# KrishnaswamyLab/MELD

Hardware: AMD Instinct MI355X
Metric: cells/sec through MELD.fit_transform (kNN+Chebyshev) (higher is better)
Workload: dtype f64

## Files before the change

### include/meld_hip.h

```cpp
#ifndef MELD_HIP_H
#define MELD_HIP_H

#include <stddef.h>
#include <stdint.h>

#ifdef __cplusplus
extern "C" {
#endif

#define MELD_OK 0
#define MELD_ERR_INVALID (-1)
#define MELD_ERR_UNSUPPORTED (-2)
#define MELD_ERR_HIP (-3)

typedef void* meld_stream_t;

int meld_abi_version(void);
const char* meld_last_error(void);
int meld_device_count(void);


int meld_knn_padded_dim(int d);
int meld_knn_tile_refs(void);
int meld_knn_block_queries(void);
// ... 45 lines not shown
                            int64_t tile_begin, int64_t tile_count, meld_stream_t stream);
int meld_knn16_sphere_layout(int64_t n_ref, int d, int64_t* rows, int64_t* row_bytes);
int meld_knn16_bounds_from_spheres(const double* X, int64_t N, int d, const double* mean, const float* scale_info,
                      const float* norm2_max, const void* Rt16, int64_t q_begin, int64_t q_count,
                      const float* thr_seed, const float* q_norm2 ,
                      int nprod, void* temp, void* lb2, meld_stream_t stream);
int meld_knn16_prepare_cross(const double* X, int64_t n_refs, int64_t n_total, int d, const double* mean, int64_t q_begin,
                             int64_t q_count, void* Rt16, void* Q16, float* Qn, float* norm2, float* norm2_max,
                             float* scale_info, meld_stream_t stream);
int meld_knn16_prepare_rows(const double* X, int64_t N, int d, const double* mean, const float* scale_info,
                            int64_t q_begin, const int32_t* rows, int64_t n_rows, void* Q16, float* Qn,
                            meld_stream_t stream);
int meld_knn16_research_thresholds(const int32_t* rows, int64_t n_rows, int64_t q_begin, const int32_t* cand_cnt,
                                   const float* cand_d2, int cap, int ksel, const float* norm2, const float* norm2_max,
                                   double err_coef, double err_lin, double err3, const float* scale_info, float* thr,
                                   meld_stream_t stream);
int meld_knn16_seed_thresholds_mfma(const void* Q16, const float* Qn, const void* Rt16, const float* scale_info,
                                    const float* norm2_max, int64_t n_ref, int d, int64_t q_begin, int64_t q_count,
                                    int knn, double radius_factor, int nprod, int side_tiles, float* thr_init,
                                    meld_stream_t stream);
int meld_knn16_topk(const void* Q16, const float* Qn, const void* Rt16, const float* scale_info,
                    int64_t n_ref, int d, int64_t q_count, int ksel, int nprod, int n_slices, const void* lb2,
                    const float* norm2_max, int64_t q_begin, const float* thr_init, int knn, double radius_factor,
                    int32_t* cand_idx, float* cand_d2, int32_t* cand_cnt, float* cand_thr,
                    uint64_t* tiles_done ,
                    const int32_t* block_order ,
                    meld_stream_t stream);
int meld_knn16_block_work(const void* lb2, const float* thr_seed, int64_t n_ref, int d, int64_t q_count, int nprod,
                          const float* norm2_max, const float* scale_info, int32_t* work, meld_stream_t stream);
int meld_knn16_step_lists(const void* lb2, const float* thr_seed, int64_t n_ref, int d, int64_t q_count, int nprod,
                          const float* norm2_max, const float* scale_info, int64_t q_begin, uint32_t* list,
                          int64_t list_stride, int32_t* cnt, meld_stream_t stream);
size_t meld_knn16_list_scratch_bytes(int64_t n_ref);
int meld_knn16_step_lists_direct(const double* X, int64_t N, int d, const double* mean, const float* scale_info, const float* norm2_max,
                                 const void* Rt16, const float* thr_seed, const float* q_norm2, int nprod, void* temp, void* scratch,
                                 uint32_t* list, int64_t list_stride, int32_t* cnt, meld_stream_t stream);
int meld_knn16_step_lists_direct_lead(const double* X, int64_t N, int d, const double* mean, const float* scale_info, const float* norm2_max,
                                 const void* Rt16, const float* thr_seed, const float* q_norm2, int nprod, void* temp, void* scratch,
                                 uint32_t* list, int64_t list_stride, int32_t* cnt, int lead_only, meld_stream_t stream);
int meld_knn16_step_lists_direct_spheres(const double* X, int64_t N, int d, const double* mean, const float* scale_info, const float* norm2_max,
                                 const void* Rt16, const float* thr_seed, const float* q_norm2, int nprod, void* temp, void* scratch,
                                 uint32_t* list, int64_t list_stride, int32_t* cnt, int lead_only, meld_stream_t stream);
int meld_knn16_topk_listed(const void* Q16, const float* Qn, const void* Rt16, const float* scale_info, int64_t n_ref, int d,
                           int64_t q_count, int ksel, const uint32_t* step_list, const int32_t* step_cnt, int64_t list_stride,
                           const float* norm2_max, int64_t q_begin, const float* thr_init, int knn, double radius_factor,
                           int32_t* cand_idx, float* cand_d2, int32_t* cand_cnt, float* cand_thr, uint64_t* tiles_done,
                           const int32_t* block_order, int n_slices , meld_stream_t stream);
int meld_knn16_topk_listed_partial(const void* Q16, const float* Qn, const void* Rt16, const float* scale_info, int64_t n_ref,
                                   int d, int64_t q_count, int ksel, const uint32_t* step_list, const int32_t* step_cnt,
                                   int64_t list_stride, const float* norm2_max, int64_t q_begin, const float* thr_init, int knn,
                                   double radius_factor, int32_t* cand_idx, float* cand_d2, int32_t* cand_cnt, float* cand_thr,
                                   uint64_t* tiles_done, const int32_t* block_order, int n_slices, int partial_test,
                                   meld_stream_t stream);
int meld_knn16_partial_filter(const void* Q16, const float* Qn, const void* Rt16, const float* scale_info, const float* norm2_max, int d,
                              int64_t q_count, const float* thr_init, uint32_t* step_list, const int32_t* step_cnt, int64_t list_stride,
                              int32_t* cnt_out, uint64_t* tested, const int32_t* block_order , meld_stream_t stream);
int meld_knn16_resident_blocks(int d, int nprod);
int meld_knn16_max_slices(int ksel);
int meld_knn16_merge_slices(const int32_t* s_idx, const float* s_d2, const int32_t* s_cnt, int64_t q_count,
                            int ksel, int n_slices, int32_t* out_idx, float* out_d2, int32_t* out_cnt,
                            meld_stream_t stream);


int meld_knn_refine(const double* X, int64_t N, int d, int64_t q_begin, int64_t q_count,
                    const int32_t* cand_idx, const float* cand_d2, const int32_t* cand_cnt,
                    const float* cand_thr ,
                    int ksel, int cap , int knn, double decay, double thresh,
                    const float* norm2_max, double err_coef,
                    const float* norm2 , double err_coef_lin, double* bw,
                    double* cand_val, int32_t* keep_cnt, int32_t* flag_rows, int32_t* n_flag,
                    const int32_t* rows, int out_cap, int32_t* cand_idx_out,
                    double bw_scale ,
                    const double* bw_fixed ,
                    int max_rank ,
                    meld_stream_t stream);

int meld_knn_radius_exact(const double* X, int64_t N, int d, int64_t q_begin, const int32_t* flag_rows,
                          int32_t n_flag, const double* bw, int knn, double decay, double thresh,
                          int mode, int32_t* fb_cnt, const int64_t* fb_off, int32_t* fb_cursor,
                          int32_t* fb_col, double* fb_val, int32_t* err_flag,
                          double bw_scale ,
                          meld_stream_t stream);
int meld_knn_pair_distances(const double* X, int d, const int64_t* rows, const int64_t* cand, int64_t n, int kk, double* out,
                            meld_stream_t stream);

#define MELD_METRIC_L1 1
#define MELD_METRIC_LINF 2
int meld_metric_tile_rows(void);
int meld_metric_tile_boxes(const double* X, int64_t N, int d, double* box_lo, double* box_hi, meld_stream_t stream);
int meld_metric_topk(const double* X, int64_t N, int d, int metric, int ksel, const double* box_lo, const double* box_hi, int prune,
                     double* heap_d, int32_t* heap_i, int32_t* cand_idx, double* cand_d, int32_t* cand_cnt,
                     unsigned long long* tiles_done, meld_stream_t stream);
int meld_metric_refine(const int32_t* cand_idx, const double* cand_d, const int32_t* cand_cnt, int64_t N, int ksel, int knn,
                       double decay, double thresh, double* bw, double* cand_val, int32_t* keep_cnt, int32_t* flag_rows,
                       int32_t* n_flag, meld_stream_t stream);
int meld_metric_radius(const double* X, int64_t N, int d, int metric, const int32_t* flag_rows, int32_t n_flag, const double* bw,
                       double decay, double thresh, int mode, int32_t* fb_cnt, const int64_t* fb_off, int32_t* fb_cursor,
                       int32_t* fb_col, double* fb_val, meld_stream_t stream);

int meld_metric_cross_slices(int64_t M, int64_t N, int n_slices);
int meld_metric_cross_seed(const double* Qt, int64_t M, const double* box_lo, const double* box_hi, int64_t N, int d, int metric,
                           unsigned long long* seed_key, meld_stream_t stream);
int meld_metric_cross_topk(const double* Qt, int64_t M, const double* X, int64_t N, int d, int metric, int ksel, const double* box_lo,
                           const double* box_hi, const int32_t* seed, int prune, int n_slices, double* heap_d, int32_t* heap_i,
                           int32_t* part_idx, double* part_d, int32_t* part_cnt, int32_t* cand_idx, double* cand_d, int32_t* cand_cnt,
                           unsigned long long* tiles_done, meld_stream_t stream);
int meld_metric_cross_refine(const int32_t* cand_idx, const double* cand_d, const int32_t* cand_cnt, int64_t M, int ksel, int knn,
                             double decay, double thresh, double bw_scale, double* bw, double* cand_val, int32_t* keep_cnt,
                             int32_t* flag_rows, int32_t* n_flag, meld_stream_t stream);
int meld_metric_cross_radius(const double* Q, int64_t M, const double* X, int64_t N, int d, int metric, const int32_t* flag_rows,
                             int32_t n_flag, const double* bw, double decay, double thresh, int mode, int32_t* fb_cnt,
                             const int64_t* fb_off, int32_t* fb_cursor, int32_t* fb_col, double* fb_val, meld_stream_t stream);


size_t meld_scan_temp_bytes(int64_t n);
int meld_exclusive_scan_i32_i64(const int32_t* in, int64_t* out, int64_t n, void* temp, size_t temp_bytes,
                                meld_stream_t stream);

int meld_coo_emit(int64_t q_begin, int64_t q_count, const int32_t* cand_idx, const double* cand_val,
                  const int32_t* cand_cnt, int ksel, int cap, const int64_t* keep_off, const int32_t* flag_rows,
                  int32_t n_flag, const int64_t* fb_off, const int32_t* fb_col, const double* fb_val,
                  int64_t fb_base, int64_t M, uint64_t* keys, double* vals, meld_stream_t stream);

size_t meld_sort_temp_bytes(int64_t n);
int meld_sort_pairs_u64_f64(const uint64_t* keys_in, uint64_t* keys_out, const double* vals_in,
                            double* vals_out, int64_t n, int end_bit, void* temp, size_t temp_bytes,
                            meld_stream_t stream);

size_t meld_merge_temp_bytes(int64_t n);
int meld_coo_merge(const uint64_t* keys_sorted, const double* vals_sorted, int64_t n, uint64_t* ukeys,
                   double* uvals, int64_t* n_unique, void* temp, size_t temp_bytes, meld_stream_t stream);

int meld_csr_from_keys(const uint64_t* ukeys, int64_t nnz, int64_t row_begin, int64_t n_rows,
                       int64_t* rowptr, int32_t* col, meld_stream_t stream);

int meld_coo_partition_remote(const uint64_t* keys, const double* vals, int64_t n, int64_t rows_per_rank, int world,
                              int self_rank, int64_t cap, int32_t* counts, int64_t* send, meld_stream_t stream);
int meld_coo_emit_scatter(int64_t q_count, const int32_t* cand_idx, const double* cand_val, int ksel, int cap,
                          const int32_t* keep_cnt, const int32_t* flag_rows, int32_t n_flag, const int64_t* fb_off,
                          const int32_t* fb_col, const double* fb_val, int64_t fb_total, int32_t* cursor, int32_t* tcol,
                          double* tval, meld_stream_t stream);
int meld_csr_bucket_slots(void);
int meld_coo_scatter_rows(const uint64_t* keys, const double* vals, int64_t n, int64_t row_begin, int64_t n_rows,
                          int32_t* cursor, int32_t* tcol, double* tval, meld_stream_t stream);
int meld_csr_rows_sort_merge(const int32_t* cursor, int64_t n_rows, int32_t* tcol, double* tval, int32_t* ucnt,
                             int32_t* flags,
                             int symm ,
                             double theta , meld_stream_t stream);
int meld_csr_rows_sort_merge_sums(const int32_t* cursor, int64_t n_rows, int32_t* tcol, double* tval, int32_t* ucnt, int32_t* flags,
                                  int symm, double theta, double diag, double* sums, meld_stream_t stream);
int meld_csr_compact_rows_anisotropy(const int64_t* rowptr, int64_t n_rows, const int32_t* tcol, const double* tval, int32_t* col,
                                     double* val, const double* ksum, double anisotropy, double* dw, meld_stream_t stream);
int meld_csr_compact_rows(const int64_t* rowptr, int64_t n_rows, const int32_t* tcol, const double* tval,
                          int32_t* col, double* val, meld_stream_t stream);
int meld_csr_compact_rows_sums(const int64_t* rowptr, int64_t n_rows, const int32_t* tcol, const double* tval, int32_t* col,
                               double* val, double diag, double* sums, meld_stream_t stream);

int meld_csr_row_sums(const int64_t* rowptr, const double* val, int64_t n_rows, double diag,
                      double* out, meld_stream_t stream);
int meld_csr_anisotropy(const int64_t* rowptr, const int32_t* col, double* val, int64_t n_rows,
                        const double* ksum_all, int64_t ksum_row_offset, double anisotropy,
                        meld_stream_t stream);
int meld_csr_anisotropy_degrees(const int64_t* rowptr, const int32_t* col, double* val, int64_t n_rows,
                                const double* ksum_all, int64_t ksum_row_offset, double anisotropy, double* dw,
                                meld_stream_t stream);


size_t meld_extend_rows_temp_bytes(int64_t n, int64_t n_rows);
int meld_extend_rows(const uint64_t* keys, const double* half_vals, int64_t n, int64_t row_begin, int64_t n_rows, int64_t n_cols,
                     int64_t* rowptr, int32_t* col, double* val, double* rowsum, void* temp, size_t temp_bytes,
                     meld_stream_t stream);
int meld_extend_apply(const int64_t* rowptr, const int32_t* col, const double* val, const double* rowsum, int64_t n_rows,
                      const double* F, int64_t n_f_rows, int p, const int64_t* colmap, double* out, meld_stream_t stream);


struct meld_pt_layout;
typedef struct meld_laplacian {
  const int64_t* rowptr; const int32_t* col; const double* val; const double* dw;
  int64_t n_rows, nnz;
  const struct meld_pt_layout* layout;
} meld_laplacian_t;

int meld_spmm_dot_slots(void);
int meld_cheby_step(const meld_laplacian_t* L, int p, const double* x_full, int64_t x_row_offset, const double* z, double* y,
                    double* r, double alpha, double beta, double gamma, double coef, double* dots, meld_stream_t stream);

int meld_cheby_step_wide(const meld_laplacian_t* L, int p, const double* x_full, int64_t x_row_offset, const double* z, double* y,
                         double alpha, double beta, double gamma, meld_stream_t stream);

int meld_block_max_blocks(void);
int meld_block_gram_f64(const double* A, int64_t lda, const double* B, int64_t ldb, int64_t n_rows, int m, double* part, int n_blocks,
                        double* C, meld_stream_t stream);
int meld_block_rotate_f64(const double* A, int64_t lda, const double* S, int64_t n_rows, int m, double* out, int64_t ldo,
                          meld_stream_t stream);
// ... 97 lines not shown
```

### meld_amd/_lib.py

```python
from __future__ import annotations

from ._options import is_set, opt

import ctypes as C
import os

_HERE = os.path.dirname(os.path.abspath(__file__))
LIB_NAME = "libmeld_hip.so"
LIB_PATH = os.path.join(_HERE, LIB_NAME)

_i32, _i64, _f64, _sz, _ptr = C.c_int, C.c_int64, C.c_double, C.c_size_t, C.c_void_p

SIGNATURES = {
    "meld_abi_version": (_i32, []),
    "meld_last_error": (C.c_char_p, []),
    "meld_device_count": (_i32, []),
    "meld_knn_padded_dim": (_i32, [_i32]),
    "meld_knn_tile_refs": (_i32, []),
    "meld_knn_block_queries": (_i32, []),
    "meld_knn_row_capacity": (_i32, [_i32]),
    "meld_col_sums_f64": (_i32, [_ptr, _i64, _i32, _ptr, _ptr]),
    "meld_col_stats_temp_bytes": (_sz, [_i32]),
    "meld_col_stats_f64": (_i32, [_ptr, _i64, _i32, _ptr, _ptr, _ptr, _ptr, _sz, _ptr]),
    "meld_knn_prepare_refs": (_i32, [_ptr, _i64, _i32, _ptr, _i32, _ptr, _ptr, _ptr, _ptr]),
    "meld_knn_prepare_queries": (_i32, [_ptr, _i64, _i32, _ptr, _i32, _i64, _i64, _ptr, _ptr]),
    "meld_knn_topk": (_i32, [_ptr, _ptr, _i64, _i32, _i64, _i32, _ptr, _ptr, _ptr, _ptr]),
    "meld_knn_refine": (
        _i32,
        [_ptr, _i64, _i32, _i64, _i64, _ptr, _ptr, _ptr, _ptr, _i32, _i32, _i32, _f64, _f64, _ptr, _f64, _ptr, _f64, _ptr, _ptr, _ptr,
         _ptr, _ptr, _ptr, _i32, _ptr, _f64, _ptr, _i32, _ptr],
    ),
    "meld_knn_error_coef": (_f64, [_i32]),
    "meld_knn16_kblocks": (_i32, [_i32]),
    "meld_knn16_tile_refs": (_i32, []),
    "meld_knn16_split_dims": (_i32, [_i32]),
    "meld_knn16_block_queries": (_i32, []),
    "meld_knn16_row_capacity": (_i32, [_i32]),
    "meld_knn16_error_coef": (_f64, [_i32, _i32]),
    "meld_knn16_error_coef_const": (_f64, [_i32, _i32]),
    "meld_knn16_error_coef_lin": (_f64, [_i32]),
    "meld_knn16_resident_blocks": (_i32, [_i32, _i32]),
    "meld_knn16_tile_bytes": (_sz, [_i32]),
    "meld_knn16_query_bytes": (_sz, [_i32]),
    "meld_knn16_prepare": (_i32, [_ptr, _i64, _i32, _ptr, _i64, _i64, _ptr, _ptr, _ptr, _ptr, _ptr, _ptr, _ptr]),
    "meld_knn16_prepare_scaled": (_i32, [_ptr, _i64, _i32, _ptr, _ptr, _ptr, _i64, _i64, _ptr, _ptr, _ptr, _ptr, _ptr, _ptr, _ptr]),
    "meld_knn16_prepare_cross": (_i32, [_ptr, _i64, _i64, _i32, _ptr, _i64, _i64, _ptr, _ptr, _ptr, _ptr, _ptr, _ptr, _ptr]),
    "meld_knn16_prepare_rows": (_i32, [_ptr, _i64, _i32, _ptr, _ptr, _i64, _ptr, _i64, _ptr, _ptr, _ptr]),
    "meld_knn16_research_thresholds": (_i32, [_ptr, _i64, _i64, _ptr, _ptr, _i32, _i32, _ptr, _ptr, _f64, _f64, _f64, _ptr, _ptr, _ptr]),
    "meld_knn16_bounds_bytes": (_sz, [_i64, _i64]),
    "meld_knn16_bounds_temp_bytes": (_sz, [_i64, _i32, _i64]),
    "meld_knn16_bounds": (_i32, [_ptr, _i64, _i32, _ptr, _ptr, _ptr, _ptr, _i64, _i64, _ptr, _ptr, _i32, _ptr, _ptr, _ptr]),
    "meld_knn16_bounds_from_spheres": (_i32, [_ptr, _i64, _i32, _ptr, _ptr, _ptr, _ptr, _i64, _i64, _ptr, _ptr, _i32, _ptr, _ptr, _ptr]),
    "meld_knn16_tile_spheres": (_i32, [_ptr, _i64, _i32, _ptr, _ptr, _ptr, _i64, _i64, _ptr]),
    "meld_knn16_sphere_layout": (_i32, [_i64, _i32, _ptr, _ptr]),
    "meld_knn16_topk": (_i32, [_ptr, _ptr, _ptr, _ptr, _i64, _i32, _i64, _i32, _i32, _i32, _ptr, _ptr, _i64, _ptr, _i32, _f64, _ptr, _ptr, _ptr, _ptr, _ptr, _ptr, _ptr]),
    "meld_knn16_block_work": (_i32, [_ptr, _ptr, _i64, _i32, _i64, _i32, _ptr, _ptr, _ptr, _ptr]),
    "meld_knn16_step_lists": (_i32, [_ptr, _ptr, _i64, _i32, _i64, _i32, _ptr, _ptr, _i64, _ptr, _i64, _ptr, _ptr]),
    "meld_knn16_list_scratch_bytes": (_sz, [_i64]),
    "meld_knn16_step_lists_direct": (_i32, [_ptr, _i64, _i32, _ptr, _ptr, _ptr, _ptr, _ptr, _ptr, _i32, _ptr, _ptr, _ptr, _i64, _ptr, _ptr]),
    "meld_knn16_prepare_fused": (_i32, [_ptr, _i64, _i32, _ptr, _ptr, _ptr, _ptr, _ptr, _ptr, _ptr, _ptr, _ptr, _ptr, _ptr]),
    "meld_knn16_step_lists_direct_spheres": (_i32, [_ptr, _i64, _i32, _ptr, _ptr, _ptr, _ptr, _ptr, _ptr, _i32, _ptr, _ptr, _ptr, _i64, _ptr, _i32, _ptr]),
    "meld_knn16_step_lists_direct_lead": (_i32, [_ptr, _i64, _i32, _ptr, _ptr, _ptr, _ptr, _ptr, _ptr, _i32, _ptr, _ptr, _ptr, _i64, _ptr, _i32, _ptr]),
    "meld_knn16_topk_listed": (_i32, [_ptr, _ptr, _ptr, _ptr, _i64, _i32, _i64, _i32, _ptr, _ptr, _i64, _ptr, _i64, _ptr, _i32, _f64, _ptr, _ptr, _ptr, _ptr, _ptr, _ptr, _i32, _ptr]),
    "meld_knn16_topk_listed_partial": (_i32, [_ptr, _ptr, _ptr, _ptr, _i64, _i32, _i64, _i32, _ptr, _ptr, _i64, _ptr, _i64, _ptr, _i32, _f64, _ptr, _ptr, _ptr, _ptr, _ptr, _ptr, _i32, _i32, _ptr]),
    "meld_knn16_partial_filter": (_i32, [_ptr, _ptr, _ptr, _ptr, _ptr, _i32, _i64, _ptr, _ptr, _ptr, _i64, _ptr, _ptr, _ptr, _ptr]),
    "meld_knn16_seed_thresholds_mfma": (_i32, [_ptr, _ptr, _ptr, _ptr, _ptr, _i64, _i32, _i64, _i64, _i32, _f64, _i32, _i32, _ptr, _ptr]),
    "meld_knn16_max_slices": (_i32, [_i32]),
    "meld_knn16_merge_slices": (_i32, [_ptr, _ptr, _ptr, _i64, _i32, _i32, _ptr, _ptr, _ptr, _ptr]),
    "meld_knn_radius_exact": (
        _i32,
        [_ptr, _i64, _i32, _i64, _ptr, _i32, _ptr, _i32, _f64, _f64, _i32, _ptr, _ptr, _ptr, _ptr, _ptr, _ptr, _f64, _ptr],
    ),
    "meld_knn_pair_distances": (_i32, [_ptr, _i32, _ptr, _ptr, _i64, _i32, _ptr, _ptr]),
    "meld_metric_tile_rows": (_i32, []),
    "meld_metric_tile_boxes": (_i32, [_ptr, _i64, _i32, _ptr, _ptr, _ptr]),
    "meld_metric_topk": (_i32, [_ptr, _i64, _i32, _i32, _i32, _ptr, _ptr, _i32, _ptr, _ptr, _ptr, _ptr, _ptr, _ptr, _ptr]),
    "meld_metric_refine": (_i32, [_ptr, _ptr, _ptr, _i64, _i32, _i32, _f64, _f64, _ptr, _ptr, _ptr, _ptr, _ptr, _ptr]),
    "meld_metric_radius": (_i32, [_ptr, _i64, _i32, _i32, _ptr, _i32, _ptr, _f64, _f64, _i32, _ptr, _ptr, _ptr, _ptr, _ptr, _ptr]),
    "meld_metric_cross_slices": (_i32, [_i64, _i64, _i32]),
    "meld_metric_cross_seed": (_i32, [_ptr, _i64, _ptr, _ptr, _i64, _i32, _i32, _ptr, _ptr]),
    "meld_metric_cross_topk": (_i32, [_ptr, _i64, _ptr, _i64, _i32, _i32, _i32, _ptr, _ptr, _ptr, _i32, _i32, _ptr, _ptr, _ptr, _ptr, _ptr, _ptr,
                                      _ptr, _ptr, _ptr, _ptr]),
    "meld_metric_cross_refine": (_i32, [_ptr, _ptr, _ptr, _i64, _i32, _i32, _f64, _f64, _f64, _ptr, _ptr, _ptr, _ptr, _ptr, _ptr]),
    "meld_metric_cross_radius": (_i32, [_ptr, _i64, _ptr, _i64, _i32, _i32, _ptr, _i32, _ptr, _f64, _f64, _i32, _ptr, _ptr, _ptr, _ptr, _ptr, _ptr]),
    "meld_scan_temp_bytes": (_sz, [_i64]),
    "meld_exclusive_scan_i32_i64": (_i32, [_ptr, _ptr, _i64, _ptr, _sz, _ptr]),
    "meld_coo_emit": (
        _i32,
        [_i64, _i64, _ptr, _ptr, _ptr, _i32, _i32, _ptr, _ptr, _i32, _ptr, _ptr, _ptr, _i64, _i64, _ptr, _ptr, _ptr],
    ),
    "meld_sort_temp_bytes": (_sz, [_i64]),
    "meld_sort_pairs_u64_f64": (_i32, [_ptr, _ptr, _ptr, _ptr, _i64, _i32, _ptr, _sz, _ptr]),
    "meld_merge_temp_bytes": (_sz, [_i64]),
    "meld_coo_merge": (_i32, [_ptr, _ptr, _i64, _ptr, _ptr, _ptr, _ptr, _sz, _ptr]),
    "meld_csr_from_keys": (_i32, [_ptr, _i64, _i64, _i64, _ptr, _ptr, _ptr]),
    "meld_csr_seg_length": (_i32, []),
    "meld_csr_spmm_f64": (_i32, [_ptr, _ptr, _ptr, _i32, _i64, _ptr, _ptr, _i64, _ptr, _ptr, _i64, _ptr, _ptr, _i64, _i32, _ptr, _i64, _ptr]),
    "meld_csr_transpose_keys": (_i32, [_ptr, _ptr, _ptr, _i32, _i64, _ptr, _ptr, _ptr]),
    "meld_csr_rows_to_dense_f64": (_i32, [_ptr, _ptr, _ptr, _i32, _i64, _i64, _i64, _ptr, _i64, _ptr]),
    "meld_csr_bucket_slots": (_i32, []),
    "meld_coo_scatter_rows": (_i32, [_ptr, _ptr, _i64, _i64, _i64, _ptr, _ptr, _ptr, _ptr]),
    "meld_coo_emit_scatter": (_i32, [_i64, _ptr, _ptr, _i32, _i32, _ptr, _ptr, _i32, _ptr, _ptr, _ptr, _i64, _ptr, _ptr, _ptr, _ptr]),
    "meld_coo_partition_remote": (_i32, [_ptr, _ptr, _i64, _i64, _i32, _i32, _i64, _ptr, _ptr, _ptr]),
    "meld_csr_rows_sort_merge": (_i32, [_ptr, _i64, _ptr, _ptr, _ptr, _ptr, _i32, _f64, _ptr]),
    "meld_csr_compact_rows": (_i32, [_ptr, _i64, _ptr, _ptr, _ptr, _ptr, _ptr]),
    "meld_csr_rows_sort_merge_sums": (_i32, [_ptr, _i64, _ptr, _ptr, _ptr, _ptr, _i32, _f64, _f64, _ptr, _ptr]),
    "meld_csr_compact_rows_anisotropy": (_i32, [_ptr, _i64, _ptr, _ptr, _ptr, _ptr, _ptr, _f64, _ptr, _ptr]),
    "meld_csr_compact_rows_sums": (_i32, [_ptr, _i64, _ptr, _ptr, _ptr, _ptr, _f64, _ptr, _ptr]),
    "meld_csr_row_sums": (_i32, [_ptr, _ptr, _i64, _f64, _ptr, _ptr]),
    "meld_csr_anisotropy": (_i32, [_ptr, _ptr, _ptr, _i64, _ptr, _i64, _f64, _ptr]),
    "meld_csr_anisotropy_degrees": (_i32, [_ptr, _ptr, _ptr, _i64, _ptr, _i64, _f64, _ptr, _ptr]),
    "meld_extend_rows_temp_bytes": (_sz, [_i64, _i64]),
    "meld_extend_rows": (_i32, [_ptr, _ptr, _i64, _i64, _i64, _i64, _ptr, _ptr, _ptr, _ptr, _ptr, _sz, _ptr]),
    "meld_extend_apply": (_i32, [_ptr, _ptr, _ptr, _ptr, _i64, _ptr, _i64, _i32, _ptr, _ptr, _ptr]),
    "meld_spmm_dot_slots": (_i32, []),
    "meld_cheby_step": (_i32, [_ptr, _i32, _ptr, _i64, _ptr, _ptr, _ptr, _f64, _f64, _f64, _f64, _ptr, _ptr]),
    "meld_lanczos_steps": (_i32, [_ptr, _ptr, _ptr, _ptr, _ptr, _ptr, _ptr, _i32, _i32, _ptr, _ptr, _ptr]),
    "meld_lanczos_spmv": (_i32, [_ptr, _ptr, _i64, _ptr, _ptr, _ptr, _ptr, _ptr]),
    "meld_lanczos_alpha": (_i32, [_ptr, _ptr, _ptr, _ptr, _i32, _ptr]),
    "meld_lanczos_axpy": (_i32, [_ptr, _ptr, _i64, _ptr, _ptr, _ptr]),
    "meld_lanczos_beta": (_i32, [_ptr, _ptr, _ptr, _ptr, _i32, _ptr]),
    "meld_lanczos_fold": (_i32, [_ptr, _ptr, _ptr, _ptr, _i32, _ptr]),
    "meld_lanczos_axpy3": (_i32, [_ptr, _ptr, _ptr, _i64, _ptr, _ptr, _ptr]),
    "meld_pt_geometry": (_i32, [_ptr, _ptr, _ptr, _ptr]),
    "meld_pt_num_blocks": (_i32, [_i64]),
    "meld_pt_seg_len": (_i64, [_i32]),
    "meld_pt_stream_len": (_i64, [_i64, _i32]),
    "meld_pt_desc_len": (_i64, [_i32]),
    "meld_pt_build": (_i32, [_ptr, _ptr, _ptr, _i64, _i64, _i64, _i32, _ptr, _ptr, _ptr, _ptr]),
    "meld_cheby_step_wide": (_i32, [_ptr, _i32, _ptr, _i64, _ptr, _ptr, _f64, _f64, _f64, _ptr]),
    "meld_block_max_blocks": (_i32, []),
    "meld_block_gram_f64": (_i32, [_ptr, _i64, _ptr, _i64, _i64, _i32, _ptr, _i32, _ptr, _ptr]),
    "meld_block_rotate_f64": (_i32, [_ptr, _i64, _ptr, _i64, _i32, _ptr, _i64, _ptr]),
    "meld_block_residuals_f64": (_i32, [_ptr, _ptr, _i64, _ptr, _i64, _i32, _ptr, _i32, _ptr, _ptr]),
    "meld_kmeans_max_blocks": (_i32, []),
    "meld_kmeans_assign": (_i32, [_ptr, _i64, _i32, _ptr, _i32, _ptr, _ptr, _ptr, _ptr, _i32, _ptr]),
    "meld_scale_f64": (_i32, [_ptr, _f64, _ptr, _i64, _ptr]),
    "meld_axpby_f64": (_i32, [_f64, _ptr, _f64, _ptr, _i64, _ptr, _ptr]),
    "meld_normalize_rows_l1": (_i32, [_ptr, _ptr, _i64, _i32, _ptr]),
    "meld_assign_nearest": (_i32, [_ptr, _i64, _i32, _ptr, _i32, _ptr, _ptr, _ptr, _ptr]),
    "meld_chain_order": (_i32, [_ptr, _i64, _i32, _i32, _ptr, _ptr]),
    "meld_gather_rows_f64": (_i32, [_ptr, _ptr, _i64, _i32, _ptr, _ptr]),
    "meld_frame_max_dims": (_i32, []),
    "meld_cov_sample_f64": (_i32, [_ptr, _i64, _i32, _ptr, _i64, _ptr, _ptr]),
    "meld_rotate_rows_f64": (_i32, [_ptr, _i64, _i32, _ptr, _ptr, _ptr, _ptr]),
    "meld_argsort_u32_temp_bytes": (_sz, [_i64]),
    "meld_argsort_u32": (_i32, [_ptr, _i64, _i32, _ptr, _ptr, _ptr, _sz, _ptr]),
    "meld_order_starts": (_i32, [_ptr, _i64, _i32, _ptr, _ptr]),
    "meld_order_pick_centroids": (_i32, [_ptr, _i64, _i32, _ptr, _ptr, _i32, _i32, _ptr, _ptr]),
    "meld_order_update_keys": (_i32, [_ptr, _ptr, _ptr, _i64, _i32, _ptr]),
    "meld_rccl_available": (_i32, []),
    "meld_rccl_unique_id": (_i32, [_ptr]),
    "meld_rccl_comm_create": (_i32, [_ptr, _i32, _i32, _ptr]),
    "meld_rccl_comm_destroy": (_i32, [_ptr]),
    "meld_rccl_all_gather": (_i32, [_ptr, _ptr, _ptr, _sz, _ptr]),
# ... 61 lines not shown
```

### meld_amd/build.py

```python
from __future__ import annotations

from ._options import is_set, opt

import os
import shutil
import subprocess
import sys

_HERE = os.path.dirname(os.path.abspath(__file__))
CSRC = os.path.join(_HERE, "csrc")
SOURCES = ["api.hip", "knn.hip", "knn16.hip", "refine.hip", "assemble.hip", "spmm.hip", "spmm_tiled.hip", "reorder.hip", "kmeans.hip", "labels.hip", "sharded.hip", "frame.hip", "csr_dense.hip", "metric_knn.hip", "extend.hip", "subspace.hip"]
OUT = os.path.join(_HERE, "libmeld_hip.so")
FLAGS = ["--offload-arch=gfx950", "-O3", "-std=c++17", "-fPIC", "-Wno-unused-result"]
FILE_FLAGS = {"knn16.hip": ["-fno-honor-nans"]}


def _hipcc():
    exe = shutil.which("hipcc") or "/opt/rocm/bin/hipcc"
    if not os.path.exists(exe):
        raise RuntimeError("hipcc not found (ROCm toolchain required to build meld_amd)")
    return exe


def _stale(out, deps):
# ... 29 lines not shown
                    label = lines[max(i for i in starts if i <= wi)]
                    m2 = re.search(r"Header=(BB\d+_\d+)", label) or (re.match(r"^\.L(BB\d+_\d+):", label) if "Loop Header" in label else None)
                    if m2:
                        votes[m2.group(1)] = votes.get(m2.group(1), 0) + 1
                header = max(votes, key=votes.get)
                assert votes[header] >= 7, votes
                checked = 0
                for bi, i0 in enumerate(starts):
                    i1 = starts[bi + 1] if bi + 1 < len(starts) else len(lines)
                    label = lines[i0]
                    in_loop = re.search(r"(Header=|Loop |^\.L)" + header + r"\b", label) is not None
                    if not in_loop and not any(i in wait_set for i in range(i0, i1)):
                        continue
                    inside = False
                    for l in lines[i0 + 1 : i1]:
                        if "#ASMSTART" in l:
                            inside = True
                        elif "#ASMEND" in l:
                            inside = False
                        elif not inside and not l.lstrip().startswith(";"):
                            assert not slot.search(l.split(";")[0]), (fn, l)
                            checked += 1
                assert checked > 200, (fn, checked)
                kernels += 1
            fn, lines = (m.group(1) if m else None), []
        elif fn:
            lines.append(line)
    assert kernels == 3, kernels
    return kernels


def gate_stream_slots(hipcc=None, verbose=True):
    hipcc = hipcc or _hipcc()
    src = os.path.join(CSRC, "spmm_tiled.hip")
    cmd = [hipcc] + FLAGS + ["--cuda-device-only", "-S", src, "-o", "-"]
    if verbose:
        print("[meld_amd.build] gate:", " ".join(cmd), flush=True)
    run = subprocess.run(cmd, stdout=subprocess.PIPE, stderr=subprocess.PIPE, text=True)
    if run.returncode != 0 or not run.stdout:
        raise RuntimeError("meld_amd.build: `hipcc -S` of spmm_tiled.hip failed (status {}), the register-slot guard of pt_step_kernel "
                           "could not run -- not linking:\n{}".format(run.returncode, run.stderr[-2000:]))
    asm = run.stdout
    try:
        return check_stream_slots(asm)
    except (AssertionError, ValueError, StopIteration) as e:
        raise RuntimeError("meld_amd.build: the register-slot guard of pt_step_kernel failed ({}); the tiled recurrence kernel "
                           "cannot be trusted with this toolchain -- not linking".format(e))


def build(force=False, verbose=True):
    hipcc = _hipcc()
    objdir = os.path.join(_HERE, "build")
    os.makedirs(objdir, exist_ok=True)
    headers = [os.path.join(CSRC, "common.hpp"), os.path.join(_HERE, "..", "include", "meld_hip.h")]
    procs = []
    objs = []
    for src in SOURCES:
        s = os.path.join(CSRC, src)
        o = os.path.join(objdir, src.replace(".hip", ".o"))
        objs.append(o)
        if force or _stale(o, [s] + headers):
            cmd = [hipcc] + FLAGS + FILE_FLAGS.get(src, []) + ["-c", s, "-o", o]
            if verbose:
                print("[meld_amd.build]", " ".join(cmd), flush=True)
            procs.append((src, subprocess.Popen(cmd, stdout=subprocess.PIPE, stderr=subprocess.STDOUT)))
    rebuilt = [src for src, _ in procs]
    for src, p in procs:
        out, _ = p.communicate()
        if p.returncode != 0:
            sys.stderr.write(out.decode(errors="replace"))
            raise RuntimeError("hipcc failed on {}".format(src))
    if "spmm_tiled.hip" in rebuilt or (force and opt("MELD_BUILD_SKIP_GATE") != "1"):
        if opt("MELD_BUILD_SKIP_GATE") != "1":
            gate_stream_slots(hipcc, verbose)
    if force or procs or _stale(OUT, objs):
        cmd = [hipcc, "--offload-arch=gfx950", "-shared", "-fPIC"] + objs + ["-ldl", "-o", OUT]
        if verbose:
            print("[meld_amd.build]", " ".join(cmd), flush=True)
        subprocess.check_call(cmd)
    return OUT


if __name__ == "__main__":
    build(force="--force" in sys.argv)
    print(OUT)
```

### meld_amd/csrc/assemble.hip

```cpp
#include "common.hpp"

#include <rocprim/rocprim.hpp>

namespace meld {

__global__ __launch_bounds__(256) void coo_emit_rows_kernel(int64_t q_begin, int64_t q_count,
                                                            const int* __restrict__ cand_idx,
                                                            const double* __restrict__ cand_val, int ksel, int cap,
                                                            const int64_t* __restrict__ keep_off, int64_t M,
                                                            unsigned long long* __restrict__ keys,
                                                            double* __restrict__ vals) {
  const int lane = threadIdx.x & 63;
  const int64_t q = (int64_t)blockIdx.x * 4 + (threadIdx.x >> 6);
  if (q >= q_count) return;
  const int64_t base = keep_off[q];
  if (keep_off[q + 1] == base) return;
  const unsigned long long gi = (unsigned long long)(q_begin + q);
  int written = 0;
  for (int c0 = 0; c0 < ksel; c0 += 64) {
    const int c = c0 + lane;
    double v = 0.0;
    int j = 0;
    if (c < ksel) {
      v = cand_val[(size_t)q * ksel + c];
// ... 196 lines not shown

extern "C" size_t meld_merge_temp_bytes(int64_t n) {
  size_t bytes = 0;
  uint64_t* k = nullptr;
  double* v = nullptr;
  int64_t* c = nullptr;
  (void)rocprim::reduce_by_key(nullptr, bytes, k, v, (size_t)n, k, v, c, rocprim::plus<double>(),
                               rocprim::equal_to<uint64_t>());
  return bytes + 256;
}

extern "C" int meld_coo_merge(const uint64_t* keys_sorted, const double* vals_sorted, int64_t n, uint64_t* ukeys,
                              double* uvals, int64_t* n_unique, void* temp, size_t temp_bytes,
                              meld_stream_t stream) {
  MELD_CHECK_ARG(keys_sorted && vals_sorted && ukeys && uvals && n_unique && temp && n >= 0,
                 "meld_coo_merge: bad arguments");
  if (n == 0) {
    MELD_HIP_CALL(hipMemsetAsync(n_unique, 0, sizeof(int64_t), S(stream)));
    return MELD_OK;
  }
  size_t bytes = temp_bytes;
  MELD_HIP_CALL(rocprim::reduce_by_key(temp, bytes, keys_sorted, vals_sorted, (size_t)n, ukeys, uvals, n_unique,
                                       rocprim::plus<double>(), rocprim::equal_to<uint64_t>(), S(stream)));
  return MELD_OK;
}

extern "C" int meld_csr_from_keys(const uint64_t* ukeys, int64_t nnz, int64_t row_begin, int64_t n_rows,
                                  int64_t* rowptr, int32_t* col, meld_stream_t stream) {
  MELD_CHECK_ARG(rowptr && n_rows > 0 && nnz >= 0 && (nnz == 0 || (ukeys && col)), "meld_csr_from_keys: bad arguments");
  hipLaunchKernelGGL(csr_rowptr_kernel, dim3((unsigned)ceil_div(n_rows + 1, 256)), dim3(256), 0, S(stream),
                     reinterpret_cast<const unsigned long long*>(ukeys), nnz, row_begin, n_rows, rowptr);
  MELD_LAUNCH_CHECK("csr_rowptr_kernel");
  if (nnz > 0) {
    hipLaunchKernelGGL(csr_cols_kernel, dim3((unsigned)ceil_div(nnz, 256)), dim3(256), 0, S(stream),
                       reinterpret_cast<const unsigned long long*>(ukeys), nnz, col);
    MELD_LAUNCH_CHECK("csr_cols_kernel");
  }
  return MELD_OK;
}

__device__ __forceinline__ void coo_row_run(int64_t r, int lane, bool* leader, int* rank, int* run_len) {
  const int64_t prev = __shfl_up(r, 1, 64);
  const bool head = lane == 0 || prev != r;
  const unsigned long long hb = __ballot(head);
  const unsigned long long below = hb & ((2ull << lane) - 1ull);
  const int lead = 63 - __clzll((long long)below);
  const unsigned long long above = lane == 63 ? 0ull : (hb >> (lane + 1));
  const int next = above ? lane + 1 + (__ffsll((long long)above) - 1) : 64;
  *leader = head;
  *rank = lane - lead;
  *run_len = next - lane;
}

constexpr int CSR_BUCKET = 256;

__global__ __launch_bounds__(256) void coo_scatter_rows_kernel(const unsigned long long* __restrict__ keys,
                                                               const double* __restrict__ vals, int64_t n, int64_t row_begin,
                                                               int64_t n_rows, int* __restrict__ cursor, int* __restrict__ tcol,
                                                               double* __restrict__ tval) {
  const int64_t e = (int64_t)blockIdx.x * blockDim.x + threadIdx.x;
  const int lane = threadIdx.x & 63;
  int64_t r = -1 - lane;
  unsigned long long k = 0;
  if (e < n) {
    k = keys[e];
    const int64_t rr = (int64_t)(k >> 32) - row_begin;
    if (rr >= 0 && rr < n_rows) r = rr;
  }
  bool leader;
  int rank, run_len;
  coo_row_run(r, lane, &leader, &rank, &run_len);
  int first = 0;
  if (leader && r >= 0) first = atomicAdd(cursor + r, run_len);
  const int slot = __shfl(first, lane - rank, 64) + rank;
  if (r >= 0 && slot < CSR_BUCKET) {
    tcol[r * CSR_BUCKET + slot] = (int)(unsigned)k;
    tval[r * CSR_BUCKET + slot] = vals[e];
  }
}

constexpr int PR_PER = 16;
constexpr int PR_WORLD_MAX = 64;
__global__ __launch_bounds__(256) void coo_partition_remote_kernel(const unsigned long long* __restrict__ keys,
                                                                   const double* __restrict__ vals, int64_t n,
                                                                   int64_t rows_per_rank, int world, int self_rank, int64_t cap,
                                                                   int* __restrict__ counts, long long* __restrict__ send) {
  __shared__ int s_cnt[PR_WORLD_MAX];
  __shared__ int s_base[PR_WORLD_MAX];
  if (threadIdx.x < PR_WORLD_MAX) s_cnt[threadIdx.x] = 0;
  __syncthreads();
  const int64_t e0 = (int64_t)blockIdx.x * (256 * PR_PER) + threadIdx.x;
  unsigned long long k[PR_PER];
  int pos[PR_PER];
#pragma unroll
  for (int u = 0; u < PR_PER; ++u) {
    const int64_t e = e0 + (int64_t)u * 256;
    pos[u] = -1;
    k[u] = 0;
    if (e < n) {
      k[u] = keys[e];
      const int o = (int)min((int64_t)(k[u] >> 32) / rows_per_rank, (int64_t)world - 1);
      if (o != self_rank) pos[u] = (o << 24) | atomicAdd(&s_cnt[o], 1);
    }
  }
  __syncthreads();
  if (threadIdx.x < world && s_cnt[threadIdx.x] > 0) s_base[threadIdx.x] = atomicAdd(counts + threadIdx.x, s_cnt[threadIdx.x]);
  __syncthreads();
#pragma unroll
  for (int u = 0; u < PR_PER; ++u) {
    if (pos[u] >= 0) {
      const int o = pos[u] >> 24;
      const int64_t slot = (int64_t)s_base[o] + (pos[u] & 0xFFFFFF);
      if (slot < cap) {
        send[((int64_t)o * 2 + 0) * cap + slot] = (long long)k[u];
        send[((int64_t)o * 2 + 1) * cap + slot] = __double_as_longlong(vals[e0 + (int64_t)u * 256]);
      }
    }
  }
}

__global__ __launch_bounds__(256) void coo_emit_scatter_rows_kernel(int64_t q_count, const int* __restrict__ cand_idx,
                                                                    const double* __restrict__ cand_val, int ksel, int cap,
                                                                    const int* __restrict__ keep_cnt, int* __restrict__ cursor,
                                                                    int* __restrict__ tcol, double* __restrict__ tval) {
  const int lane = threadIdx.x & 63;
  const int64_t q = (int64_t)blockIdx.x * 4 + (threadIdx.x >> 6);
  if (q >= q_count) return;
  if (keep_cnt[q] == 0) return;
  int written = 0;
  for (int c0 = 0; c0 < ksel; c0 += 64) {
    const int c = c0 + lane;
    double v = 0.0;
    int j = 0;
    if (c < ksel) {
      v = cand_val[(size_t)q * ksel + c];
      j = cand_idx[(size_t)q * cap + c];
    }
    const bool keep = v > 0.0;
    const unsigned long long b = __ballot(keep);
    if (keep) {
      const int pos = written + __popcll(b & ((1ull << lane) - 1ull));
      const double hv = 0.5 * v;
      tcol[q * CSR_BUCKET + pos] = j;
      tval[q * CSR_BUCKET + pos] = hv;
      const int slot = atomicAdd(cursor + j, 1);
      if (slot < CSR_BUCKET) {
        tcol[(int64_t)j * CSR_BUCKET + slot] = (int)q;
        tval[(int64_t)j * CSR_BUCKET + slot] = hv;
      }
    }
    written += __popcll(b);
  }
}
__global__ __launch_bounds__(256) void coo_emit_scatter_fallback_kernel(const int* __restrict__ flag_rows, int n_flag,
                                                                        const int64_t* __restrict__ fb_off,
                                                                        const int* __restrict__ fb_col,
                                                                        const double* __restrict__ fb_val, int64_t fb_total,
                                                                        int* __restrict__ cursor, int* __restrict__ tcol,
                                                                        double* __restrict__ tval) {
  const int64_t e = (int64_t)blockIdx.x * blockDim.x + threadIdx.x;
  if (e >= fb_total) return;
  int lo = 0, hi = n_flag - 1;
  while (lo < hi) {
    const int mid = (lo + hi + 1) >> 1;
    if (fb_off[mid] <= e) lo = mid; else hi = mid - 1;
  }
  const int64_t q = flag_rows[lo];
  const int64_t pos = e - fb_off[lo];
  const int j = fb_col[e];
  const double hv = 0.5 * fb_val[e];
  if (pos < CSR_BUCKET) {
    tcol[q * CSR_BUCKET + pos] = j;
    tval[q * CSR_BUCKET + pos] = hv;
  }
  const int slot = atomicAdd(cursor + j, 1);
  if (slot < CSR_BUCKET) {
    tcol[(int64_t)j * CSR_BUCKET + slot] = (int)q;
    tval[(int64_t)j * CSR_BUCKET + slot] = hv;
  }
}

template <int SL, typename K>
__device__ __forceinline__ void csr_bitonic_sort(K (&key)[SL], int lane) {
  constexpr int NE = 64 * SL;
#pragma unroll
  for (int k = 2; k <= NE; k <<= 1) {
#pragma unroll
    for (int j = k >> 1; j > 0; j >>= 1) {
      if (j >= 64) {
        const int je = j >> 6;
#pragma unroll
        for (int e = 0; e < SL; ++e) {
          if ((e & je) == 0) {
            const bool asc = ((64 * e + lane) & k) == 0;
            const K a = key[e], b = key[e | je];
            const bool sw = asc ? (b < a) : (a < b);
            key[e] = sw ? b : a;
            key[e | je] = sw ? a : b;
          }
        }
      } else {
#pragma unroll
        for (int e = 0; e < SL; ++e) {
          const int i = 64 * e + lane;
          const K o = __shfl_xor(key[e], j, 64);
          const bool keep_min = ((i & j) == 0) == ((i & k) == 0);
          key[e] = keep_min ? (o < key[e] ? o : key[e]) : (o < key[e] ? key[e] : o);
        }
      }
    }
  }
}

template <int SL>
__device__ __forceinline__ int csr_row_merge(int* __restrict__ tcol, double* __restrict__ tval, int64_t base, int n, int lane,
                                             bool* bad, int symm, double theta, double* srow) {
  static_assert(CSR_BUCKET <= 256, "the slot shares a 32-bit key with a 24-bit column");
  unsigned cin[SL];
  bool wide = false;
#pragma unroll
  for (int e = 0; e < SL; ++e) {
// ... 200 lines not shown
        if (k < len) {
          const double dd = di * kj[u];
          const double w = (anisotropy == 0.0) ? v[u] : (anisotropy == 1.0) ? v[u] / dd : v[u] / pow(dd, anisotropy);
          col[dst + k] = c[u];
          val[dst + k] = w;
          s += w;
        }
      }
    }
  }
  s += __shfl_xor(s, 1, 64);
  s += __shfl_xor(s, 2, 64);
  s += __shfl_xor(s, 4, 64);
  if (r < n_rows && g == 0) dw[r] = 0.0 + s;
}

extern "C" int meld_csr_bucket_slots(void) { return CSR_BUCKET; }

extern "C" int meld_coo_scatter_rows(const uint64_t* keys, const double* vals, int64_t n, int64_t row_begin, int64_t n_rows,
                                     int32_t* cursor, int32_t* tcol, double* tval, meld_stream_t stream) {
  MELD_CHECK_ARG(cursor && n_rows > 0 && n >= 0 && (n == 0 || (keys && vals && tcol && tval)),
                 "meld_coo_scatter_rows: bad arguments");
  MELD_HIP_CALL(hipMemsetAsync(cursor, 0, sizeof(int32_t) * (size_t)n_rows, S(stream)));
  if (n == 0) return MELD_OK;
  hipLaunchKernelGGL(coo_scatter_rows_kernel, dim3((unsigned)ceil_div(n, 256)), dim3(256), 0, S(stream),
                     reinterpret_cast<const unsigned long long*>(keys), vals, n, row_begin, n_rows, cursor, tcol, tval);
  MELD_LAUNCH_CHECK("coo_scatter_rows_kernel");
  return MELD_OK;
}

extern "C" int meld_coo_partition_remote(const uint64_t* keys, const double* vals, int64_t n, int64_t rows_per_rank, int world,
                                         int self_rank, int64_t cap, int32_t* counts, int64_t* send, meld_stream_t stream) {
  MELD_CHECK_ARG(counts && send && n >= 0 && (n == 0 || (keys && vals)) && rows_per_rank > 0 && world >= 1 && self_rank >= 0 &&
                     self_rank < world && cap >= 0,
                 "meld_coo_partition_remote: bad arguments");
  MELD_HIP_CALL(hipMemsetAsync(counts, 0, sizeof(int32_t) * (size_t)world, S(stream)));
  if (cap > 0) MELD_HIP_CALL(hipMemsetAsync(send, 0xFF, sizeof(int64_t) * 2 * (size_t)world * (size_t)cap, S(stream)));
  if (n == 0) return MELD_OK;
  MELD_CHECK_ARG(world <= PR_WORLD_MAX, "meld_coo_partition_remote: %d ranks (at most %d)", world, PR_WORLD_MAX);
  hipLaunchKernelGGL(coo_partition_remote_kernel, dim3((unsigned)ceil_div(n, 256 * PR_PER)), dim3(256), 0, S(stream),
                     reinterpret_cast<const unsigned long long*>(keys), vals, n, rows_per_rank, world, self_rank, cap, counts,
                     reinterpret_cast<long long*>(send));
  MELD_LAUNCH_CHECK("coo_partition_remote_kernel");
  return MELD_OK;
}

extern "C" int meld_coo_emit_scatter(int64_t q_count, const int32_t* cand_idx, const double* cand_val, int ksel, int cap,
                                     const int32_t* keep_cnt, const int32_t* flag_rows, int32_t n_flag, const int64_t* fb_off,
                                     const int32_t* fb_col, const double* fb_val, int64_t fb_total, int32_t* cursor, int32_t* tcol,
                                     double* tval, meld_stream_t stream) {
  MELD_CHECK_ARG(cand_idx && cand_val && keep_cnt && cursor && tcol && tval && q_count > 0, "meld_coo_emit_scatter: bad arguments");
  MELD_CHECK_ARG(cap >= ksel && ksel <= CSR_BUCKET, "meld_coo_emit_scatter: ksel=%d must fit a row bucket (%d) and the row stride cap=%d",
                 ksel, CSR_BUCKET, cap);
  hipLaunchKernelGGL(coo_emit_scatter_rows_kernel, dim3((unsigned)ceil_div(q_count, 4)), dim3(256), 0, S(stream), q_count, cand_idx,
                     cand_val, ksel, cap, keep_cnt, cursor, tcol, tval);
  MELD_LAUNCH_CHECK("coo_emit_scatter_rows_kernel");
  if (n_flag > 0 && fb_total > 0) {
    MELD_CHECK_ARG(flag_rows && fb_off && fb_col && fb_val, "meld_coo_emit_scatter: missing fallback arrays");
    hipLaunchKernelGGL(coo_emit_scatter_fallback_kernel, dim3((unsigned)ceil_div(fb_total, 256)), dim3(256), 0, S(stream), flag_rows,
                       n_flag, fb_off, fb_col, fb_val, fb_total, cursor, tcol, tval);
    MELD_LAUNCH_CHECK("coo_emit_scatter_fallback_kernel");
  }
  return MELD_OK;
}

extern "C" int meld_csr_rows_sort_merge(const int32_t* cursor, int64_t n_rows, int32_t* tcol, double* tval, int32_t* ucnt,
                                        int32_t* flags, int symm, double theta, meld_stream_t stream) {
  MELD_CHECK_ARG(cursor && tcol && tval && ucnt && flags && n_rows > 0, "meld_csr_rows_sort_merge: bad arguments");
  MELD_CHECK_ARG(symm >= 0 && symm <= 2 && (symm != 2 || (theta >= 0.0 && theta <= 1.0)),
                 "meld_csr_rows_sort_merge: symm must be 0 (+), 1 (*) or 2 (mnn, theta in [0, 1])");
  MELD_HIP_CALL(hipMemsetAsync(flags, 0, sizeof(int32_t), S(stream)));
  hipLaunchKernelGGL(csr_rows_sort_merge_kernel, dim3((unsigned)ceil_div(n_rows, 4)), dim3(256), 0, S(stream), cursor, n_rows,
                     tcol, tval, ucnt, flags, symm, theta, 0.0, (double*)nullptr);
  MELD_LAUNCH_CHECK("csr_rows_sort_merge_kernel");
  return MELD_OK;
}

extern "C" int meld_csr_rows_sort_merge_sums(const int32_t* cursor, int64_t n_rows, int32_t* tcol, double* tval, int32_t* ucnt,
                                             int32_t* flags, int symm, double theta, double diag, double* sums, meld_stream_t stream) {
  MELD_CHECK_ARG(cursor && tcol && tval && ucnt && flags && sums && n_rows > 0, "meld_csr_rows_sort_merge_sums: bad arguments");
  MELD_CHECK_ARG(symm >= 0 && symm <= 2 && (symm != 2 || (theta >= 0.0 && theta <= 1.0)),
                 "meld_csr_rows_sort_merge_sums: symm must be 0 (+), 1 (*) or 2 (mnn, theta in [0, 1])");
  MELD_HIP_CALL(hipMemsetAsync(flags, 0, sizeof(int32_t), S(stream)));
  hipLaunchKernelGGL(csr_rows_sort_merge_kernel, dim3((unsigned)ceil_div(n_rows, 4)), dim3(256), 0, S(stream), cursor, n_rows,
                     tcol, tval, ucnt, flags, symm, theta, diag, sums);
  MELD_LAUNCH_CHECK("csr_rows_sort_merge_kernel");
  return MELD_OK;
}

extern "C" int meld_csr_compact_rows_anisotropy(const int64_t* rowptr, int64_t n_rows, const int32_t* tcol, const double* tval,
                                                int32_t* col, double* val, const double* ksum, double anisotropy, double* dw,
                                                meld_stream_t stream) {
  MELD_CHECK_ARG(rowptr && n_rows > 0 && tcol && tval && col && val && ksum && dw, "meld_csr_compact_rows_anisotropy: bad arguments");
  hipLaunchKernelGGL(csr_compact_rows_anisotropy_kernel, dim3((unsigned)ceil_div(n_rows * 8, 256)), dim3(256), 0, S(stream), rowptr, n_rows,
                     tcol, tval, col, val, ksum, anisotropy, dw);
  MELD_LAUNCH_CHECK("csr_compact_rows_anisotropy_kernel");
  return MELD_OK;
}

extern "C" int meld_csr_compact_rows(const int64_t* rowptr, int64_t n_rows, const int32_t* tcol, const double* tval,
                                     int32_t* col, double* val, meld_stream_t stream) {
  MELD_CHECK_ARG(rowptr && n_rows > 0 && tcol && tval && col && val, "meld_csr_compact_rows: bad arguments");
  hipLaunchKernelGGL(csr_compact_rows_kernel, dim3((unsigned)ceil_div(n_rows * 16, 256)), dim3(256), 0, S(stream), rowptr,
                     n_rows, tcol, tval, col, val);
  MELD_LAUNCH_CHECK("csr_compact_rows_kernel");
  return MELD_OK;
}

extern "C" int meld_csr_compact_rows_sums(const int64_t* rowptr, int64_t n_rows, const int32_t* tcol, const double* tval, int32_t* col,
                                          double* val, double diag, double* sums, meld_stream_t stream) {
  MELD_CHECK_ARG(rowptr && n_rows > 0 && tcol && tval && col && val && sums, "meld_csr_compact_rows_sums: bad arguments");
  hipLaunchKernelGGL(csr_compact_rows_sums_kernel, dim3((unsigned)ceil_div(n_rows * 8, 256)), dim3(256), 0, S(stream), rowptr, n_rows, tcol,
                     tval, col, val, diag, sums);
  MELD_LAUNCH_CHECK("csr_compact_rows_sums_kernel");
// ... 34 lines not shown
```

### meld_amd/csrc/common.hpp

```cpp
#pragma once
#include <hip/hip_runtime.h>
#include <stdint.h>
#include <stdio.h>
#include <stdlib.h>
#include <string.h>

#include "../../include/meld_hip.h"

namespace meld {

char* err_buf();
void set_err(const char* fmt, ...);

static inline hipStream_t S(meld_stream_t s) { return reinterpret_cast<hipStream_t>(s); }

constexpr int WAVE = 64;

#define MELD_CHECK_ARG(cond, ...)        \
  do {                                   \
    if (!(cond)) {                       \
      meld::set_err(__VA_ARGS__);        \
      return MELD_ERR_INVALID;           \
    }                                    \
  } while (0)

#define MELD_LAUNCH_CHECK(name)                                               \
  do {                                                                        \
    hipError_t e__ = hipGetLastError();                                       \
    if (e__ != hipSuccess) {                                                  \
      meld::set_err("%s: launch failed: %s", name, hipGetErrorString(e__));   \
      return MELD_ERR_HIP;                                                    \
    }                                                                         \
  } while (0)

#define MELD_HIP_CALL(expr)                                                   \
  do {                                                                        \
    hipError_t e__ = (expr);                                                  \
    if (e__ != hipSuccess) {                                                  \
      meld::set_err("%s failed: %s", #expr, hipGetErrorString(e__));          \
      return MELD_ERR_HIP;                                                    \
    }                                                                         \
  } while (0)

__device__ __forceinline__ double wave_sum(double v) {
#pragma unroll
  for (int off = 32; off > 0; off >>= 1) v += __shfl_xor(v, off, 64);
  return v;
}

__device__ __forceinline__ int lane_id() { return threadIdx.x & 63; }

static inline int64_t ceil_div(int64_t a, int64_t b) { return (a + b - 1) / b; }

static inline const char* meld_dev_getenv(const char* name) {
  const char* dev = getenv("MELD_DEV");
  return (dev && dev[0] == '1' && dev[1] == 0) ? getenv(name) : nullptr;
}

struct PtLanczos {
  const double* nrm2_prev;
  double* nrm2_zero;
  const double* state_prev;
  double* state_cur;
  double* betas;
  int it;
  const int* stop;
};

static inline bool laplacian_ok(const meld_laplacian_t* L) {
  if (!L || !L->rowptr || !L->dw) return false;
  if (const meld_pt_layout_t* t = L->layout)
    return t->blk_row && t->blk_ntile && t->blk_ndist && t->seg && t->list_cols && t->pval && t->pidx;
  return L->nnz == 0 || (L->col && L->val);
}

int pt_step(const meld_pt_layout_t* L, const int64_t* rowptr, const double* dw, int p, const double* x_full,
            int64_t x_row_offset, const double* z, double* y, double* r, double alpha, double beta, double gamma,
            double coef, double* dots, const double* coef_dev, hipStream_t st, double coef_x = 0.0, const PtLanczos* lz = nullptr);

}
```

### meld_amd/csrc/knn16.hip

```cpp
#include "common.hpp"

#include <hip/hip_fp16.h>

#include <algorithm>

namespace meld {

constexpr int K16_TS = 64;
constexpr int K16_BQ = 256;
constexpr int K16_THREADS = 256;
constexpr int K16_NWAVE = K16_THREADS / 64;
constexpr int K16_SLACK = 128;
constexpr int K16_CAPMAX = 256;
constexpr int K16_BOUNDS_THREADS = 1024;
constexpr int K16_SLOTS = K16_CAPMAX / 64;
constexpr int K16_DMAX = 16 * 9 - 3;

constexpr int K16_SPLIT_DA = 13;
__host__ __device__ inline void k16_slot(int c, int d, int dA, int* coord, int* piece) {
  *coord = -1;
  *piece = -1;
  if (dA == 0) {
    if (c < d) *coord = c;
    else if (c < d + 3) *piece = 3 + (c - d);
    return;
  }
  const int nb = d - dA;
  if (c < dA) *coord = c;
  else if (c < dA + 3) *piece = c - dA;
  else if (c < 16) return;
  else if (c < 16 + nb) *coord = dA + (c - 16);
  else if (c < 16 + nb + 3) *piece = 3 + (c - 16 - nb);
}

typedef float f32x16 __attribute__((ext_vector_type(16)));
typedef _Float16 f16x8 __attribute__((ext_vector_type(8)));

__device__ __forceinline__ float min3f(float a, float b, float c) { return __builtin_fminf(__builtin_fminf(a, b), c); }
__device__ __forceinline__ float min16(const f32x16& v) {
  const float a = min3f(v[0], v[1], v[2]);
  const float b = min3f(v[3], v[4], v[5]);
  const float c = min3f(v[6], v[7], v[8]);
  const float d = min3f(v[9], v[10], v[11]);
  const float e = min3f(v[12], v[13], v[14]);
  return __builtin_fminf(min3f(a, b, v[15]), min3f(c, d, e));
}

__device__ __forceinline__ unsigned ordered_bits(float f) {
  const unsigned b = __float_as_uint(f);
  return (b & 0x80000000u) ? ~b : (b | 0x80000000u);
}

__device__ __forceinline__ float ld_sc1_f(const float* p) {
  return __hip_atomic_load(p, __ATOMIC_RELAXED, __HIP_MEMORY_SCOPE_AGENT);
}
__device__ __forceinline__ int ld_sc1_i(const int* p) {
  return __hip_atomic_load(p, __ATOMIC_RELAXED, __HIP_MEMORY_SCOPE_AGENT);
}

#define K16_COLD_REGION_END() __builtin_amdgcn_s_waitcnt(0x0F70)

__device__ __forceinline__ bool knn16_row_slot(int p, int n0, int n1, int half, int* q) {
  if (p < half) {
    *q = p;
    return p < n0;
  }
  *q = n0 + (p - half);
  return (p - half) < n1;
}
__device__ __forceinline__ int knn16_split_pos(int pos, int m0, int half) { return pos < m0 ? pos : half + (pos - m0); }

__device__ __forceinline__ float from_ordered_bits(unsigned k) {
  return __uint_as_float((k & 0x80000000u) ? (k & 0x7fffffffu) : ~k);
}

__device__ float knn16_squeeze_row(int n0, int n1, int half, int ksel, int knn1, float rf2, float err, float nq_row,
                                   float* __restrict__ d2row, int* __restrict__ idxrow, int lane, int* n0_out,
                                   int* n1_out, float* r_out) {
  asm volatile("s_waitcnt vmcnt(0)" ::: "memory");
  float d[K16_SLOTS];
  int ix[K16_SLOTS];
  unsigned key[K16_SLOTS];
  bool valid[K16_SLOTS];
#pragma unroll
  for (int e = 0; e < K16_SLOTS; ++e) {
    const int p = lane + 64 * e;
    int q;
    valid[e] = p < 2 * half && knn16_row_slot(p, n0, n1, half, &q);
    if (valid[e]) {
      d[e] = ld_sc1_f(d2row + p);
      ix[e] = ld_sc1_i(idxrow + p);
      key[e] = ordered_bits(d[e]);
    } else {
      d[e] = INFINITY;
      ix[e] = 0x7fffffff;
      key[e] = 0xffffffffu;
    }
  }
  unsigned T = 0;
#pragma unroll 1
  for (int bit = 31; bit >= 0; --bit) {
    const unsigned trial = T | (1u << bit);
    int c = 0;
#pragma unroll
    for (int e = 0; e < K16_SLOTS; ++e) c += __popcll(__ballot(key[e] < trial));
    if (c < ksel) T = trial;
  }
  float R = INFINITY;
  if (knn1 > 0 && n0 + n1 >= knn1) {
    unsigned A = 0;
#pragma unroll 1
    for (int bit = 31; bit >= 0; --bit) {
      const unsigned trial = A | (1u << bit);
      int c = 0;
#pragma unroll
      for (int e = 0; e < K16_SLOTS; ++e) c += __popcll(__ballot(key[e] < trial));
      if (c < knn1) A = trial;
    }
    R = (rf2 * ((from_ordered_bits(A) + nq_row) + err) + err) * 1.00001f + 1e-30f - nq_row;
  }
  *r_out = R;
  const unsigned Tc = min(T, ordered_bits(R));
  int total = 0;
#pragma unroll
  for (int e = 0; e < K16_SLOTS; ++e) total += __popcll(__ballot(valid[e] && key[e] <= Tc));
  const int m0 = (total + 1) >> 1;
  int base = 0;
// ... 798 lines not shown
  auto emit = [&](unsigned ev, int par) __attribute__((always_inline)) {
    unsigned nm = 0u;
#pragma unroll
    for (int w = 0; w < 4; ++w) nm |= ((wmask[par][w] >> lane) & 1u) << w;
    nm &= (ev >> 24);
    const bool keep = nm != 0u;
    const unsigned long long b = __ballot(keep);
    if (keep) my_list_w[out_n + __popcll(b & ((1ull << lane) - 1ull))] = (ev & 0xFFFFFFu) | (nm << 24);
    out_n += __popcll(b);
  };
  unsigned ev_prev = 0u, ev_cur = load_entries(0), ev_nxt = load_entries(1);
  if (n_steps > 0) stage(ev_cur, 0);
  __builtin_amdgcn_s_waitcnt(0x0F70);
  asm volatile("s_waitcnt lgkmcnt(0)\n\ts_barrier" ::: "memory");
  for (int s = 0; s < n_steps; ++s) {
    const int buf = s & 1;
    const unsigned ev_nn = load_entries(s + 2);
    if (s + 1 < n_steps) stage(ev_nxt, buf ^ 1);
    if (wave == 0 && s > 0) emit(ev_prev, buf ^ 1);
    unsigned mybits = 0u;
#pragma unroll
    for (int j = 0; j < TPS; ++j) {
      const unsigned e = (unsigned)__builtin_amdgcn_readlane((int)ev_cur, j);
      if ((e >> (24 + wave)) & 1u) {
        const f16x8* a8 = reinterpret_cast<const f16x8*>(&ring[buf][j][0]) + jq;
        const f16x8 aA = a8[h * K16_TS], aB = a8[h * K16_TS + 32];
        f32x16 c00, c01, c10, c11;
#pragma unroll
        for (int r = 0; r < 16; ++r) c00[r] = c01[r] = c10[r] = c11[r] = 0.0f;
        c00 = __builtin_amdgcn_mfma_f32_32x32x16_f16(aA, b0[0], c00, 0, 0, 0);
        c01 = __builtin_amdgcn_mfma_f32_32x32x16_f16(aA, b0[1], c01, 0, 0, 0);
        c10 = __builtin_amdgcn_mfma_f32_32x32x16_f16(aB, b0[0], c10, 0, 0, 0);
        c11 = __builtin_amdgcn_mfma_f32_32x32x16_f16(aB, b0[1], c11, 0, 0, 0);
        const bool hit = __builtin_fminf(min16(c00), min16(c10)) < tA[0] || __builtin_fminf(min16(c01), min16(c11)) < tA[1];
        if (__any(hit)) mybits |= 1u << j;
        ++n_tested;
      }
    }
    if (lane == 0) wmask[buf][wave] = mybits;
    __builtin_amdgcn_s_waitcnt(0x0F70);
    asm volatile("s_waitcnt lgkmcnt(0)\n\ts_barrier" ::: "memory");
    ev_prev = ev_cur;
    ev_cur = ev_nxt;
    ev_nxt = ev_nn;
  }
  if (wave == 0) {
    if (n_steps > 0) emit(ev_prev, (n_steps - 1) & 1);
    if (lane == 0) cnt_out[bx] = out_n;
  }
  if (tested && lane == 0) atomicAdd(tested, n_tested);
}

template <int SL>
__device__ __forceinline__ void k16_bitonic_sort(unsigned long long (&key)[SL], int lane) {
  constexpr int NE = 64 * SL;
#pragma unroll
  for (int k = 2; k <= NE; k <<= 1) {
#pragma unroll
    for (int j = k >> 1; j > 0; j >>= 1) {
      if (j >= 64) {
        const int je = j >> 6;
#pragma unroll
        for (int e = 0; e < SL; ++e) {
          if ((e & je) == 0) {
            const int i = 64 * e + lane;
            const bool asc = (i & k) == 0;
            const unsigned long long a = key[e], b = key[e | je];
            const bool sw = asc ? (b < a) : (a < b);
            key[e] = sw ? b : a;
            key[e | je] = sw ? a : b;
          }
        }
      } else {
#pragma unroll
        for (int e = 0; e < SL; ++e) {
          const int i = 64 * e + lane;
          const unsigned long long o = __shfl_xor(key[e], j, 64);
          const bool keep_min = ((i & j) == 0) == ((i & k) == 0);
          key[e] = keep_min ? (o < key[e] ? o : key[e]) : (o < key[e] ? key[e] : o);
        }
      }
    }
  }
}
template <int SL>
__device__ __forceinline__ void k16_finish_row(float* __restrict__ drow, int* __restrict__ irow, int n0, int half, int n_all, int n,
                                               float add, float out_scale, int lane) {
  unsigned long long key[SL];
#pragma unroll
  for (int e = 0; e < SL; ++e) {
    const int i = lane + 64 * e;
    const int p = i < n0 ? i : half + (i - n0);
    key[e] = ~0ull;
    if (i < n_all) key[e] = ((unsigned long long)ordered_bits(drow[p] + 0.0f) << 32) | (unsigned)irow[p];
  }
  k16_bitonic_sort<SL>(key, lane);
#pragma unroll
  for (int e = 0; e < SL; ++e) {
    const int i = 64 * e + lane;
    if (i < n) {
      drow[i] = (from_ordered_bits((unsigned)(key[e] >> 32)) + add) * out_scale;
      irow[i] = (int)(unsigned)key[e];
    }
  }
}
__global__ __launch_bounds__(256) void knn16_finish_rows_kernel(float* __restrict__ d2, int* __restrict__ idx,
                                                                int* __restrict__ cnt, const float* __restrict__ Qn,
                                                                const float* __restrict__ scale_info, int64_t n_rows,
                                                                int64_t q_pad, int cap, int ksel) {
  const int lane = threadIdx.x & 63;
  const int64_t row = (int64_t)blockIdx.x * 4 + (threadIdx.x >> 6);
  if (row >= n_rows) return;
  const int packed = cnt[row];
  const int n0 = packed & 0xffff, n1 = (packed >> 16) & 0xffff, half = cap >> 1;
  float* drow = d2 + (size_t)row * cap;
  int* irow = idx + (size_t)row * cap;
  const int n_all = n0 + n1, n = min(n_all, ksel);
  const float add = Qn[row % q_pad], out_scale = scale_info[1];
  if (n_all <= 64)
    k16_finish_row<1>(drow, irow, n0, half, n_all, n, add, out_scale, lane);
  else if (n_all <= 128)
    k16_finish_row<2>(drow, irow, n0, half, n_all, n, add, out_scale, lane);
  else
    k16_finish_row<K16_SLOTS>(drow, irow, n0, half, n_all, n, add, out_scale, lane);
  if (lane == 0) cnt[row] = n;
}

constexpr int K16_MERGE_MAX = 4096;
constexpr int K16_MERGE_SLOTS = K16_MERGE_MAX / 64;

__global__ __launch_bounds__(64) void knn16_merge_slices_kernel(const int* __restrict__ s_idx,
                                                                const float* __restrict__ s_d2,
                                                                const int* __restrict__ s_cnt, int q_count, int q_pad,
                                                                int ksel, int cap, int n_slices,
                                                                int* __restrict__ out_idx, float* __restrict__ out_d2,
                                                                int* __restrict__ out_cnt) {
  extern __shared__ __attribute__((aligned(16))) unsigned char merge_lds[];
  float* sd = reinterpret_cast<float*>(merge_lds);
// ... 1315 lines not shown
                     dim3(64 * SEED_WAVES), 0, st, reinterpret_cast<const _Float16*>(Q16), Qn,                            \
                     reinterpret_cast<const _Float16*>(Rt16), scale_info, norm2_max, n_tiles, (int)(q_begin / K16_TS),   \
                     side, n_b * K16_NWAVE, knn + 1, rf2, ec, el, thr_init)
#define K16_SEEDM_CASE(KBV)          \
  case KBV:                          \
    if (knn + 1 <= 16)               \
      K16_SEEDM_LAUNCH(KBV, 16);     \
    else                             \
      K16_SEEDM_LAUNCH(KBV, 64);     \
    break;
  switch (KB) {
    K16_SEEDM_CASE(1)
    K16_SEEDM_CASE(2)
    K16_SEEDM_CASE(3)
    K16_SEEDM_CASE(4)
    K16_SEEDM_CASE(5)
    K16_SEEDM_CASE(6)
    K16_SEEDM_CASE(7)
    K16_SEEDM_CASE(8)
    K16_SEEDM_CASE(9)
    default:
      set_err("meld_knn16_seed_thresholds_mfma: no kernel for %d K blocks", KB);
      return MELD_ERR_UNSUPPORTED;
  }
#undef K16_SEEDM_CASE
#undef K16_SEEDM_LAUNCH
  MELD_LAUNCH_CHECK("knn16_seed_mfma_kernel");
  return MELD_OK;
}

template <int KB, int STATS>
static void k16_launch_topk(dim3 grid, hipStream_t st, const K16Args& ka, bool listed, bool ee, int nprod) {
  if (listed) {
    if constexpr (KB >= 2 && KB <= 7) {
      if (ee) {
        hipLaunchKernelGGL((knn16_topk_kernel<KB, STATS, 1, true, true>), grid, dim3(K16_THREADS), 0, st, ka);
        return;
      }
    }
    hipLaunchKernelGGL((knn16_topk_kernel<KB, STATS, 1, true>), grid, dim3(K16_THREADS), 0, st, ka);
  } else if (nprod == 1) {
    hipLaunchKernelGGL((knn16_topk_kernel<KB, STATS, 1>), grid, dim3(K16_THREADS), 0, st, ka);
  } else {
    hipLaunchKernelGGL((knn16_topk_kernel<KB, STATS, 3>), grid, dim3(K16_THREADS), 0, st, ka);
  }
}

static int k16_topk_impl(const void* Q16, const float* Qn, const void* Rt16, const float* scale_info,
                         int64_t n_ref, int d,
                         int64_t q_count, int ksel, int nprod, int n_slices, const void* lb2,
                         const float* norm2_max, int64_t q_begin, const float* thr_init, int knn,
                         double radius_factor, int32_t* cand_idx, float* cand_d2, int32_t* cand_cnt,
                         float* cand_thr, uint64_t* tiles_done, const int32_t* block_order, const uint32_t* step_list,
                         const int32_t* step_cnt, int64_t list_stride, meld_stream_t stream, int partial_test = 0, int two_counters = 0) {
  MELD_CHECK_ARG(nprod == 1 || nprod == 3, "meld_knn16_topk: nprod must be 1 or 3");
  MELD_CHECK_ARG(step_list == nullptr || (step_cnt != nullptr && nprod == 1 && lb2 == nullptr && thr_init != nullptr),
                 "meld_knn16_topk_listed: step lists go with the hi-only pass, start thresholds and no table");
  MELD_CHECK_ARG(n_slices >= 1 && n_slices * ksel <= K16_MERGE_MAX, "meld_knn16_topk: n_slices=%d must satisfy n_slices * ksel <= %d",
                 n_slices, K16_MERGE_MAX);
  MELD_CHECK_ARG(Q16 && Qn && Rt16 && scale_info && cand_idx && cand_d2 && cand_cnt, "meld_knn16_topk: null pointer");
  MELD_CHECK_ARG(lb2 == nullptr || norm2_max != nullptr, "meld_knn16_topk: pruning needs norm2_max");
  MELD_CHECK_ARG(cand_thr == nullptr || (norm2_max != nullptr && knn >= 0 && knn < ksel && radius_factor >= 1.0),
                 "meld_knn16_topk: the radius cut needs norm2_max, 0 <= knn < ksel, radius_factor >= 1");
  const int knn1 = (cand_thr && knn >= 1) ? knn + 1 : 0;
  const float rf2 = knn1 > 0 ? (float)(radius_factor * radius_factor * (1.0 + 1e-6)) : 0.0f;
  const float err_c = (float)meld_knn16_error_coef_const(nprod, d), err_l = (float)meld_knn16_error_coef_lin(nprod);
  MELD_CHECK_ARG(n_ref > 0 && n_ref < (int64_t)1 << 31 && q_count > 0, "meld_knn16_topk: bad sizes");
  const int cap = meld_knn16_row_capacity(ksel);
  if (cap < 0) return cap;
  const int KB = meld_knn16_kblocks(d);
  if (KB < 0) return KB;
  const int n_tiles = (int)ceil_div(n_ref, K16_TS);
  const dim3 grid((unsigned)n_slices, (unsigned)ceil_div(q_count, K16_BQ));
  MELD_CHECK_ARG(grid.y <= 65535u, "meld_knn16_topk: more than 65535 query blocks in one launch");
  MELD_CHECK_ARG(n_slices <= ceil_div(n_ref, K16_TS), "meld_knn16_topk: more slices than reference tiles");
  const int tile_origin = (int)((q_begin / K16_TS) % n_tiles);
  const _Float16* q = reinterpret_cast<const _Float16*>(Q16);
  const _Float16* r = reinterpret_cast<const _Float16*>(Rt16);
  unsigned long long* stats = nullptr;
  if (meld_dev_getenv("MELD_KNN16_STATS")) {
    static unsigned long long* counters[64] = {nullptr};
    int dev = 0;
    MELD_HIP_CALL(hipGetDevice(&dev));
    MELD_CHECK_ARG(dev >= 0 && dev < 64, "meld_knn16_topk: device index out of range");
    if (counters[dev] == nullptr) MELD_HIP_CALL(hipMalloc(reinterpret_cast<void**>(&counters[dev]), 256));
    MELD_HIP_CALL(hipMemsetAsync(counters[dev], 0, 256, S(stream)));
    stats = counters[dev];
  }
  K16Args ka;
  ka.Q16 = q;
  ka.Qn = Qn;
  ka.Rt16 = r;
  ka.scale_info = scale_info;
  ka.n_ref = (int)n_ref;
  ka.n_tiles = n_tiles;
  ka.ksel = ksel;
  ka.cap = cap;
  ka.lb2 = reinterpret_cast<const __half*>(lb2);
  ka.norm2_max = norm2_max;
  ka.err_coef = (float)meld_knn16_error_coef(nprod, d);
  ka.tile_origin = tile_origin;
  ka.batch_every = 64;
  ka.batch_slack = 64;
  ka.two_sided = 1;
  ka.stats = stats;
  ka.thr_init = thr_init;
  ka.knn1 = knn1;
  ka.rf2 = rf2;
  ka.err_c = err_c;
  ka.err_l = err_l;
  ka.cand_idx = cand_idx;
  ka.cand_d2 = cand_d2;
  ka.cand_cnt = cand_cnt;
  ka.cand_thr = cand_thr;
  ka.tiles_done = reinterpret_cast<unsigned long long*>(tiles_done);
  ka.block_order = block_order;
  ka.step_list = step_list;
  ka.step_cnt = step_cnt;
  ka.list_stride = (long long)list_stride;
  const int dA = k16_dA(d, KB);
  const bool ee = step_list != nullptr && dA > 0 && KB >= 2 && KB <= 7 && partial_test != 0;
  ka.ee_hi = 16 + d - dA;
  ka.count_go = two_counters;
  ka.planes_used = ((dA > 0 ? 16 + (d - dA) + 3 : d + 3) + 7) / 8;
#define K16_CASE(KBV)                                                                                                      \
  case KBV:                                                                                                                \
    (stats ? k16_launch_topk<KBV, 1> : k16_launch_topk<KBV, 0>)(grid, S(stream), ka, step_list != nullptr, ee, nprod); \
    break;
  switch (KB) {
    K16_CASE(1)
    K16_CASE(2)
    K16_CASE(3)
    K16_CASE(4)
    K16_CASE(5)
    K16_CASE(6)
    K16_CASE(7)
    K16_CASE(8)
    K16_CASE(9)
    default:
      set_err("meld_knn16_topk: KB=%d is not an instantiated size", KB);
      return MELD_ERR_UNSUPPORTED;
  }
#undef K16_CASE
  MELD_LAUNCH_CHECK("knn16_topk_kernel");
  const int64_t n_rows = (int64_t)grid.x * K16_BQ * grid.y;
  hipLaunchKernelGGL(knn16_finish_rows_kernel, dim3((unsigned)ceil_div(n_rows, 4)), dim3(256), 0, S(stream), cand_d2, cand_idx, cand_cnt, Qn,
                     scale_info, n_rows, (int64_t)grid.y * K16_BQ, cap, ksel);
  MELD_LAUNCH_CHECK("knn16_finish_rows_kernel");
  if (stats) {
    unsigned long long st[13] = {0, 0, 0, 0, 0, 0, 0, 0, 0, 0, 0, 0, 0};
    MELD_HIP_CALL(hipStreamSynchronize(S(stream)));
    MELD_HIP_CALL(hipMemcpy(st, stats, sizeof(st), hipMemcpyDeviceToHost));
    fprintf(stderr, "[knn16 stats] wave-blocks %llu  slow-path entries %llu (%.1f %%)  appends %llu (%.1f per query)  compactions %llu  tiles staged %llu (%.1f %% of workgroups x tiles)\n",
            st[0], st[1], st[0] ? 100.0 * (double)st[1] / (double)st[0] : 0.0, st[2], (double)st[2] / (double)q_count, st[3], st[4],
            100.0 * (double)st[4] / ((double)grid.y * (double)n_tiles));
    if (ee)
      fprintf(stderr, "[knn16 stats] blocks of 32 references that went on past K block 0: %llu of %llu (%.1f %%)\n", st[12], st[0],
              st[0] ? 100.0 * (double)st[12] / (double)st[0] : 0.0);
    {
      const double tot = (double)(st[5] + st[6] + st[7] + st[8] + st[9] + st[10]);
      fprintf(stderr, "[knn16 stats] wave cycles (s_memtime units, summed over waves; %% of the scan loop): MFMA segments of live steps %.1f  slow path %.1f  "
                      "control tail %.1f  tile wait %.1f  barrier %.1f  steps sat out %.1f   -- per wave and staged tile: %.0f units; live wave-steps %.1f %%\n",
              100.0 * st[5] / tot, 100.0 * st[6] / tot, 100.0 * st[7] / tot, 100.0 * st[8] / tot, 100.0 * st[9] / tot, 100.0 * st[10] / tot,
              tot / (double)st[11], st[11] ? 50.0 * (double)st[0] / (double)st[11] : 0.0);
    }
  }
  return MELD_OK;
}

extern "C" int meld_knn16_topk(const void* Q16, const float* Qn, const void* Rt16, const float* scale_info,
                               int64_t n_ref, int d,
                               int64_t q_count, int ksel, int nprod, int n_slices, const void* lb2,
                               const float* norm2_max, int64_t q_begin, const float* thr_init, int knn,
                               double radius_factor, int32_t* cand_idx, float* cand_d2, int32_t* cand_cnt,
                               float* cand_thr, uint64_t* tiles_done, const int32_t* block_order, meld_stream_t stream) {
  return k16_topk_impl(Q16, Qn, Rt16, scale_info, n_ref, d, q_count, ksel, nprod, n_slices, lb2, norm2_max, q_begin, thr_init, knn,
                       radius_factor, cand_idx, cand_d2, cand_cnt, cand_thr, tiles_done, block_order, nullptr, nullptr, 0, stream);
}

extern "C" int meld_knn16_topk_listed(const void* Q16, const float* Qn, const void* Rt16, const float* scale_info, int64_t n_ref,
                                      int d, int64_t q_count, int ksel, const uint32_t* step_list, const int32_t* step_cnt,
                                      int64_t list_stride, const float* norm2_max, int64_t q_begin, const float* thr_init, int knn,
                                      double radius_factor, int32_t* cand_idx, float* cand_d2, int32_t* cand_cnt, float* cand_thr,
                                      uint64_t* tiles_done, const int32_t* block_order, int n_slices, meld_stream_t stream) {
  MELD_CHECK_ARG(step_list && step_cnt && list_stride > 0, "meld_knn16_topk_listed: null step lists");
  return k16_topk_impl(Q16, Qn, Rt16, scale_info, n_ref, d, q_count, ksel, 1, n_slices, nullptr, norm2_max, q_begin, thr_init, knn,
                       radius_factor, cand_idx, cand_d2, cand_cnt, cand_thr, tiles_done, block_order, step_list, step_cnt, list_stride,
                       stream);
}

extern "C" int meld_knn16_topk_listed_partial(const void* Q16, const float* Qn, const void* Rt16, const float* scale_info, int64_t n_ref,
                                              int d, int64_t q_count, int ksel, const uint32_t* step_list, const int32_t* step_cnt,
                                              int64_t list_stride, const float* norm2_max, int64_t q_begin, const float* thr_init, int knn,
                                              double radius_factor, int32_t* cand_idx, float* cand_d2, int32_t* cand_cnt, float* cand_thr,
                                              uint64_t* tiles_done, const int32_t* block_order, int n_slices, int partial_test,
                                              meld_stream_t stream) {
  MELD_CHECK_ARG(step_list && step_cnt && list_stride > 0, "meld_knn16_topk_listed_partial: null step lists");
  return k16_topk_impl(Q16, Qn, Rt16, scale_info, n_ref, d, q_count, ksel, 1, n_slices, nullptr, norm2_max, q_begin, thr_init, knn,
                       radius_factor, cand_idx, cand_d2, cand_cnt, cand_thr, tiles_done, block_order, step_list, step_cnt, list_stride,
                       stream, partial_test, 1);
}

extern "C" int meld_knn16_partial_filter(const void* Q16, const float* Qn, const void* Rt16, const float* scale_info, const float* norm2_max,
                                         int d, int64_t q_count, const float* thr_init, uint32_t* step_list, const int32_t* step_cnt,
                                         int64_t list_stride, int32_t* cnt_out, uint64_t* tested, const int32_t* block_order,
                                         meld_stream_t stream) {
  MELD_CHECK_ARG(Q16 && Qn && Rt16 && scale_info && norm2_max && thr_init && step_list && step_cnt && cnt_out && list_stride > 0 && q_count > 0,
                 "meld_knn16_partial_filter: null pointer or bad sizes");
  const int KB = meld_knn16_kblocks(d);
  if (KB < 0) return KB;
  const int dA = k16_dA(d, KB);
  MELD_CHECK_ARG(dA > 0 && KB >= 2, "meld_knn16_partial_filter: d = %d has no split operand layout", d);
  const unsigned n_blocks = (unsigned)ceil_div(q_count, K16_BQ);
  hipLaunchKernelGGL((knn16_partial_filter_kernel<8, 4>), dim3(n_blocks), dim3(256), 0, S(stream), reinterpret_cast<const _Float16*>(Q16), Qn,
                     reinterpret_cast<const _Float16*>(Rt16), scale_info, norm2_max, thr_init, step_list, step_cnt, (long long)list_stride, cnt_out,
                     reinterpret_cast<unsigned long long*>(tested), block_order, KB, 16 + d - dA);
  MELD_LAUNCH_CHECK("knn16_partial_filter_kernel");
  return MELD_OK;
}

extern "C" int meld_knn16_resident_blocks(int d, int nprod) {
  MELD_CHECK_ARG(nprod == 1 || nprod == 3, "meld_knn16_resident_blocks: nprod must be 1 or 3");
  const int KB = meld_knn16_kblocks(d);
  if (KB < 0) return KB;
  int per_cu = 0;
#define K16_OCC(KBV)                                                                                              \
  case KBV:                                                                                                       \
    if (nprod == 1) {                                                                                             \
      MELD_HIP_CALL(hipOccupancyMaxActiveBlocksPerMultiprocessor(&per_cu, knn16_topk_kernel<KBV, 0, 1>, K16_THREADS, 0)); \
    } else {                                                                                                      \
      MELD_HIP_CALL(hipOccupancyMaxActiveBlocksPerMultiprocessor(&per_cu, knn16_topk_kernel<KBV, 0, 3>, K16_THREADS, 0)); \
    }                                                                                                             \
    break;
  switch (KB) {
    K16_OCC(1)
    K16_OCC(2)
    K16_OCC(3)
    K16_OCC(4)
    K16_OCC(5)
    K16_OCC(6)
    K16_OCC(7)
    K16_OCC(8)
    K16_OCC(9)
    default:
      return MELD_ERR_UNSUPPORTED;
  }
#undef K16_OCC
  int dev = 0, cus = 0;
  MELD_HIP_CALL(hipGetDevice(&dev));
  MELD_HIP_CALL(hipDeviceGetAttribute(&cus, hipDeviceAttributeMultiprocessorCount, dev));
  return per_cu * cus;
}

// ... 16 lines not shown
```

### meld_amd/csrc/refine.hip

```cpp
#include "common.hpp"

#include <algorithm>
#include <cfloat>

namespace meld {

constexpr int RB_FALL = 8;
#ifndef RF_U
#define RF_UC 7
#define RF_U 5
#endif

constexpr int RF_DMAX = 256;
__host__ __device__ __forceinline__ bool rf_four_chains(int d) { return (d & 1) == 0 && d <= RF_DMAX; }

__device__ __forceinline__ double dist2_four_chains(const double* __restrict__ xa, const double* __restrict__ xb, int d) {
  const double2* a2 = reinterpret_cast<const double2*>(xa);
  const double2* b2 = reinterpret_cast<const double2*>(xb);
  const int nk = d >> 1;
  double s[4] = {0.0, 0.0, 0.0, 0.0}, s1[4] = {0.0, 0.0, 0.0, 0.0};
  int kk = 0;
  for (; kk + 4 <= nk; kk += 4) {
#pragma unroll
    for (int j = 0; j < 4; ++j) {
      const double2 a = a2[kk + j], b = b2[kk + j];
      const double t0 = a.x - b.x, t1 = a.y - b.y;
      s[j] = fma(t0, t0, s[j]);
      s1[j] = fma(t1, t1, s1[j]);
    }
  }
#pragma unroll
  for (int j = 0; j < 3; ++j) {
    if (kk + j < nk) {
      const double2 a = a2[kk + j], b = b2[kk + j];
      const double t0 = a.x - b.x, t1 = a.y - b.y;
      s[j] = fma(t0, t0, s[j]);
      s1[j] = fma(t1, t1, s1[j]);
    }
  }
  return ((s[0] + s1[0]) + (s[1] + s1[1])) + ((s[2] + s1[2]) + (s[3] + s1[3]));
}

__device__ __forceinline__ double decay_kernel(double dist, double bw, double decay) {
  if (isinf(decay)) return dist <= bw ? 1.0 : 0.0;
  double v = exp(-pow(dist / bw, decay));
  if (v != v) v = 1.0;
  return v;
}

template <bool COOP>
__global__ __launch_bounds__(256) void refine_kernel(
    const double* __restrict__ X, int d, int64_t q_begin, int64_t q_count, const int* __restrict__ cand_idx,
    const float* __restrict__ cand_d2, const int* __restrict__ cand_cnt, const float* __restrict__ cand_thr, int ksel,
    int cap, int knn, double decay, double thresh, double radius_factor, const float* __restrict__ norm2_max, double err_coef,
    const float* __restrict__ norm2, double err_coef_lin, double bw_scale, const double* __restrict__ bw_fixed, int max_rank,
    double* __restrict__ bw_out, double* __restrict__ cand_val, int* __restrict__ keep_cnt,
    int* __restrict__ flag_rows, int* __restrict__ n_flag, const int* __restrict__ rows, int out_cap,
    int* __restrict__ cand_idx_out) {
  const int lane = threadIdx.x & 63;
  const int64_t q = (int64_t)blockIdx.x * 4 + (threadIdx.x >> 6);
  if (q >= q_count) return;
  const int64_t orow = rows ? (int64_t)rows[q] : q;
  const int64_t gi = q_begin + orow;
  const double* xi = X + gi * d;
  const size_t ro = (size_t)q * cap;
  int idx_raw[2] = {0, 0};
  float d2_raw[2] = {0.0f, 0.0f}, d2_knn = 0.0f;
  if constexpr (COOP) {
#pragma unroll
    for (int e = 0; e < 2; ++e) {
      const int cc = min(lane + 64 * e, cap - 1);
      idx_raw[e] = cand_idx[ro + cc];
      d2_raw[e] = cand_d2[ro + cc];
    }
    d2_knn = cand_d2[ro + min(knn, cap - 1)];
  }
  const int n = min(cand_cnt[q], ksel);

  double E = err_coef * (double)norm2_max[0];
  if (norm2 != nullptr && err_coef_lin > 0.0) E += err_coef_lin * sqrt((double)norm2[gi] * (double)norm2_max[0]);
  double skip_above = INFINITY;
  const double skip_factor = fmax(radius_factor * bw_scale, 1.0);
  if (bw_fixed != nullptr) {
    const double rfix = fmax(bw_fixed[gi] * bw_scale, DBL_EPSILON) * radius_factor;
    skip_above = rfix * rfix * (1.0 + 1e-12) + E;
  } else if (n > knn) {
    skip_above = skip_factor * skip_factor * ((double)(COOP ? d2_knn : cand_d2[ro + knn]) + E) + E;
  }

  double dist[2];
  int idx[2];
  if constexpr (COOP) {
    __shared__ __attribute__((aligned(16))) double xis[4][RF_DMAX];
    __shared__ double dls[4][128];
    const int w = threadIdx.x >> 6;
    for (int k = lane; k < d; k += 64) xis[w][k] = xi[k];
    bool gth[2];
#pragma unroll
    for (int e = 0; e < 2; ++e) {
      const int c = lane + 64 * e;
      idx[e] = c < n ? idx_raw[e] : 0x7fffffff;
      gth[e] = c < n && (double)d2_raw[e] <= skip_above;
    }
    const int n_g = __popcll(__ballot(gth[0])) + __popcll(__ballot(gth[1]));
    const int grp = lane >> 2, j = lane & 3, nk = d >> 1;
    const double2* X2 = reinterpret_cast<const double2*>(X);
    const double2* xi2 = reinterpret_cast<const double2*>(&xis[w][0]);
    for (int c0 = 0; c0 < n_g; c0 += 16) {
      const int c = c0 + grp;
      const int i_lo = __shfl(idx[0], c & 63, 64), i_hi = __shfl(idx[1], c & 63, 64);
      const bool ok = c < n_g;
      const double2* xj2 = X2 + (int64_t)(ok ? (c < 64 ? i_lo : i_hi) : 0) * nk;
      double s = 0.0, s1 = 0.0;
      for (int k0 = 0; k0 < nk; k0 += 4 * RF_UC) {
        double2 b[RF_UC];
#pragma unroll
        for (int u = 0; u < RF_UC; ++u) {
          const int k = k0 + 4 * u + j;
          if (ok && k < nk) b[u] = xj2[k];
        }
#pragma unroll
        for (int u = 0; u < RF_UC; ++u) {
          const int k = k0 + 4 * u + j;
          if (ok && k < nk) {
            const double2 a = xi2[k];
            const double t0 = a.x - b[u].x, t1 = a.y - b[u].y;
            s = fma(t0, t0, s);
            s1 = fma(t1, t1, s1);
          }
        }
// ... 49 lines not shown
        s = fma(t, t, s);
        s += s1;
      }
      dist[e] = sqrt(s);
    } else {
      if (c >= n) idx[e] = 0x7fffffff;
      dist[e] = INFINITY;
    }
  }
  }

  const unsigned long long g0 = __ballot(dist[0] < INFINITY), g1 = __ballot(dist[1] < INFINITY);
  const int n_fin = g1 ? 64 + (64 - __clzll((long long)g1)) : (g0 ? 64 - __clzll((long long)g0) : 0);
  int rk[2] = {0, 0};
  const int ne = (n_fin > 64) ? 2 : 1;
  bool ranked = false;
  if (ne == 1 && n <= 64) {
    int r0 = 0;
    for (int l2 = 0; l2 < n_fin; ++l2) {
      const double de = __hiloint2double(__builtin_amdgcn_readlane(__double2hiint(dist[0]), l2), __builtin_amdgcn_readlane(__double2loint(dist[0]), l2));
      r0 += (de < dist[0]) ? 1 : 0;
    }
    int sum = dist[0] < INFINITY ? r0 : 0;
#pragma unroll
    for (int o = 32; o > 0; o >>= 1) sum += __shfl_xor(sum, o, 64);
    if (sum == n_fin * (n_fin - 1) / 2) {
      rk[0] = r0;
      ranked = true;
    }
  }
  for (int e2 = 0; e2 < (ranked ? 0 : ne); ++e2) {
    const int lim = min(64, n_fin - 64 * e2);
    for (int l2 = 0; l2 < lim; ++l2) {
      const double de = __hiloint2double(__builtin_amdgcn_readlane(__double2hiint(dist[e2]), l2), __builtin_amdgcn_readlane(__double2loint(dist[e2]), l2));
      const int ie = __builtin_amdgcn_readlane(idx[e2], l2);
      rk[0] += (de < dist[0] || (de == dist[0] && ie < idx[0])) ? 1 : 0;
      if (n > 64) rk[1] += (de < dist[1] || (de == dist[1] && ie < idx[1])) ? 1 : 0;
    }
  }
  double bw = 0.0;
#pragma unroll
  for (int e = 0; e < 2; ++e) {
    const unsigned long long b = __ballot((lane + 64 * e) < n && rk[e] == knn);
    if (b) bw = __shfl(dist[e], __ffsll((long long)b) - 1, 64);
  }
  if (bw_fixed != nullptr) bw = bw_fixed[gi];
  bw = fmax(bw, DBL_EPSILON);
  const double bw_raw = bw;
  bw = fmax(bw * bw_scale, DBL_EPSILON);

  const double radius = bw * radius_factor;
  const double reach = bw_fixed != nullptr ? radius : fmax(radius, bw_raw);
  double tau = INFINITY;
  if (cand_cnt[q] >= ksel) tau = (double)cand_d2[ro + ksel - 1];
  if (cand_thr != nullptr) tau = fmin(tau, (double)cand_thr[q]);
  bool complete = (reach * reach + E <= tau);
  if (max_rank > 0) {
    double d_m = INFINITY;
#pragma unroll
    for (int e = 0; e < 2; ++e) {
      const unsigned long long b = __ballot((lane + 64 * e) < n && rk[e] == max_rank - 1 && dist[e] < INFINITY);
      if (b) d_m = __shfl(dist[e], __ffsll((long long)b) - 1, 64);
    }
    if (d_m < INFINITY && d_m * d_m + E <= tau && d_m >= bw_raw) complete = true;
  }
  if (bw_fixed == nullptr && n <= knn) complete = false;

  int kept = 0;
#pragma unroll
  for (int e = 0; e < 2; ++e) {
    const int c = lane + 64 * e;
    double v = 0.0;
    if (c < n && complete) {
      v = decay_kernel(dist[e], bw, decay);
      if (v < thresh || (int64_t)idx[e] == gi) v = 0.0;
      if (max_rank > 0 && rk[e] >= max_rank) v = 0.0;
    }
    if (c < ksel) {
      cand_val[(size_t)orow * ksel + c] = v;
      if (cand_idx_out) cand_idx_out[(size_t)orow * out_cap + c] = (c < n) ? idx[e] : 0;
    }
    kept += __popcll(__ballot(v > 0.0));
  }
  if (lane == 0) {
    bw_out[orow] = bw_raw;
    keep_cnt[orow] = complete ? kept : 0;
    if (!complete) {
      const int pos = atomicAdd(n_flag, 1);
      flag_rows[pos] = (int)orow;
    }
  }
}

__global__ __launch_bounds__(256) void radius_exact_kernel(
    const double* __restrict__ X, int64_t N, int d, int64_t q_begin, const int* __restrict__ flag_rows,
    int n_flag, const double* __restrict__ bw_all, int knn, double decay, double thresh, int mode,
    int* __restrict__ fb_cnt, const int64_t* __restrict__ fb_off, int* __restrict__ fb_cursor,
    int* __restrict__ fb_col, double* __restrict__ fb_val, int* __restrict__ err_flag, int64_t ref_chunk,
    double radius_factor, double bw_scale) {
  extern __shared__ __attribute__((aligned(16))) double xq[];
  __shared__ int s_cnt[RB_FALL];
  __shared__ int s_lt[RB_FALL];
  const int f0 = blockIdx.x * RB_FALL;
  const int nf = min(RB_FALL, n_flag - f0);
  const int64_t ref_lo = (int64_t)blockIdx.y * ref_chunk;
  const int64_t ref_hi = min(N, ref_lo + ref_chunk);
  int64_t gi[RB_FALL];
  double bw[RB_FALL], rad[RB_FALL], bw_chk[RB_FALL];
#pragma unroll
  for (int f = 0; f < RB_FALL; ++f) {
    const int q = flag_rows[f0 + (f < nf ? f : 0)];
    gi[f] = q_begin + q;
    bw_chk[f] = bw_all[q];
    bw[f] = fmax(bw_all[q] * bw_scale, DBL_EPSILON);
    rad[f] = bw[f] * radius_factor * (1.0 + 1e-9);
  }
  for (int u = threadIdx.x; u < RB_FALL * d; u += blockDim.x) {
    const int f = u / d, k = u % d;
    xq[u] = X[gi[f] * d + k];
  }
  if (threadIdx.x < RB_FALL) {
    s_cnt[threadIdx.x] = 0;
    s_lt[threadIdx.x] = 0;
  }
  __syncthreads();

  int cnt[RB_FALL], lt[RB_FALL];
#pragma unroll
  for (int f = 0; f < RB_FALL; ++f) cnt[f] = lt[f] = 0;

  const bool four = rf_four_chains(d);
  const int tpr = four ? 4 : 1;
  const int jq = four ? (threadIdx.x & 3) : 0;
  const int nk = d >> 1;
  const double2* xq2 = reinterpret_cast<const double2*>(xq);
// ... 84 lines not shown
                                    int* __restrict__ fb_cnt) {
  const int f = blockIdx.x * blockDim.x + threadIdx.x;
  if (f >= n_flag) return;
  if (lt_then_cursor[f] > knn && bw_all[flag_rows[f]] > DBL_EPSILON) {
    atomicOr(err_flag, 1);
    fb_cnt[f] = -1;
  }
  lt_then_cursor[f] = 0;
}

__global__ __launch_bounds__(256) void pair_distances_kernel(const double* __restrict__ X, int d, const int64_t* __restrict__ rows,
                                                             const int64_t* __restrict__ cand, int64_t n, int kk,
                                                             double* __restrict__ out) {
  const int64_t e = (int64_t)blockIdx.x * blockDim.x + threadIdx.x;
  if (e >= n * kk) return;
  const double* xq = X + rows[e / kk] * d;
  const double* xr = X + cand[e] * d;
  if (rf_four_chains(d)) {
    out[e] = sqrt(dist2_four_chains(xq, xr, d));
    return;
  }
  double s = 0.0, s1 = 0.0;
  for (int k = 0; k < d; ++k) {
    const double t = xq[k] - xr[k];
    if ((k & 1) == 0) s = fma(t, t, s); else s1 = fma(t, t, s1);
  }
  out[e] = sqrt(s + s1);
}

}

using namespace meld;

extern "C" int meld_knn_refine(const double* X, int64_t N, int d, int64_t q_begin, int64_t q_count,
                               const int32_t* cand_idx, const float* cand_d2, const int32_t* cand_cnt,
                               const float* cand_thr, int ksel,
                               int cap, int knn, double decay, double thresh, const float* norm2_max, double err_coef,
                               const float* norm2, double err_coef_lin, double* bw,
                               double* cand_val, int32_t* keep_cnt, int32_t* flag_rows, int32_t* n_flag,
                               const int32_t* rows, int out_cap, int32_t* cand_idx_out, double bw_scale, const double* bw_fixed,
                               int max_rank, meld_stream_t stream) {
  MELD_CHECK_ARG(X && cand_idx && cand_d2 && cand_cnt && norm2_max && bw && cand_val && keep_cnt && flag_rows && n_flag,
                 "meld_knn_refine: null pointer");
  MELD_CHECK_ARG(q_count > 0 && q_begin >= 0 && d > 0 && (rows != nullptr || q_begin + q_count <= N),
                 "meld_knn_refine: bad sizes");
  MELD_CHECK_ARG(rows == nullptr || (cand_idx_out != nullptr && out_cap >= ksel),
                 "meld_knn_refine: a row list needs cand_idx_out with row stride >= ksel");
  MELD_CHECK_ARG(ksel >= 1 && ksel <= 128, "meld_knn_refine: ksel=%d outside [1,128]", ksel);
  MELD_CHECK_ARG(knn >= 0 && decay > 0 && thresh > 0 && thresh <= 1, "meld_knn_refine: bad kernel parameters");
  MELD_CHECK_ARG(cap >= ksel, "meld_knn_refine: row stride cap=%d smaller than ksel=%d", cap, ksel);
  MELD_CHECK_ARG(err_coef >= 0 && err_coef_lin >= 0, "meld_knn_refine: error coefficients must be non-negative");
  MELD_CHECK_ARG(bw_scale > 0 && bw_scale < INFINITY, "meld_knn_refine: bandwidth_scale must be positive and finite");
  MELD_CHECK_ARG(max_rank == 0 || max_rank > knn, "meld_knn_refine: max_rank=%d must exceed knn=%d (or be 0)", max_rank, knn);
  const double radius_factor = pow(-log(thresh), 1.0 / decay);
#define RF_LAUNCH(COOPV)                                                                                                          \
  hipLaunchKernelGGL(refine_kernel<COOPV>, dim3((unsigned)ceil_div(q_count, 4)), dim3(256), 0, S(stream), X, d, q_begin, q_count,  \
                     cand_idx, cand_d2, cand_cnt, cand_thr, ksel, cap, knn, decay, thresh, radius_factor, norm2_max, err_coef,     \
                     norm2, err_coef_lin, bw_scale, bw_fixed, max_rank, bw, cand_val, keep_cnt, flag_rows, n_flag, rows, out_cap, \
                     cand_idx_out)
  if (rf_four_chains(d))
    RF_LAUNCH(true);
  else
    RF_LAUNCH(false);
#undef RF_LAUNCH
  MELD_LAUNCH_CHECK("refine_kernel");
  return MELD_OK;
}

extern "C" int meld_knn_radius_exact(const double* X, int64_t N, int d, int64_t q_begin, const int32_t* flag_rows,
                                     int32_t n_flag, const double* bw, int knn, double decay, double thresh, int mode,
                                     int32_t* fb_cnt, const int64_t* fb_off, int32_t* fb_cursor, int32_t* fb_col,
                                     double* fb_val, int32_t* err_flag, double bw_scale, meld_stream_t stream) {
  if (n_flag == 0) return MELD_OK;
  MELD_CHECK_ARG(bw_scale > 0 && bw_scale < INFINITY, "meld_knn_radius_exact: bandwidth_scale must be positive and finite");
  MELD_CHECK_ARG(X && flag_rows && bw && n_flag > 0 && N > 0 && d > 0, "meld_knn_radius_exact: bad arguments");
  MELD_CHECK_ARG(mode == 0 ? (fb_cnt && err_flag && fb_cursor) : (fb_off && fb_cursor && fb_col && fb_val),
                 "meld_knn_radius_exact: missing output for mode %d", mode);
  const size_t lds = sizeof(double) * RB_FALL * (size_t)d;
  constexpr size_t lds_default = 64 * 1024 - 2 * RB_FALL * sizeof(int), lds_max = 160 * 1024 - 2 * RB_FALL * sizeof(int);
  MELD_CHECK_ARG(lds <= lds_max, "meld_knn_radius_exact: d=%d needs %zu bytes of LDS for the %d rows of a workgroup, more than the %zu it has",
                 d, lds, RB_FALL, lds_max);
  if (lds > lds_default) {
    static bool configured[64] = {};
    int dev = 0;
    if (hipGetDevice(&dev) != hipSuccess || dev < 0 || dev >= 64) dev = 0;
    if (!configured[dev]) {
      MELD_HIP_CALL(hipFuncSetAttribute(reinterpret_cast<const void*>(&radius_exact_kernel), hipFuncAttributeMaxDynamicSharedMemorySize,
                                        (int)lds_max));
      configured[dev] = true;
    }
  }
  const int64_t n_groups = ceil_div(n_flag, RB_FALL);
  const int64_t want_chunks = std::max<int64_t>(1, 1024 / n_groups);
  const int64_t ref_chunk = std::max<int64_t>(1024, ceil_div(ceil_div(N, want_chunks), 256) * 256);
  const int64_t n_chunks = ceil_div(N, ref_chunk);
  hipStream_t st = S(stream);
  if (mode == 0) {
    MELD_HIP_CALL(hipMemsetAsync(fb_cnt, 0, sizeof(int32_t) * n_flag, st));
    MELD_HIP_CALL(hipMemsetAsync(fb_cursor, 0, sizeof(int32_t) * n_flag, st));
  }
  hipLaunchKernelGGL(radius_exact_kernel, dim3((unsigned)n_groups, (unsigned)n_chunks), dim3(256), lds, st, X, N, d, q_begin,
                     flag_rows, n_flag, bw, knn, decay, thresh, mode, fb_cnt, fb_off, fb_cursor, fb_col, fb_val, err_flag,
                     ref_chunk, pow(-log(thresh), 1.0 / decay), bw_scale);
  if (mode == 0)
    hipLaunchKernelGGL(radius_check_kernel, dim3((unsigned)ceil_div(n_flag, 256)), dim3(256), 0, st, fb_cursor, n_flag, knn,
                       err_flag, flag_rows, bw, fb_cnt);
  MELD_LAUNCH_CHECK("radius_exact_kernel");
  return MELD_OK;
}

extern "C" int meld_knn_pair_distances(const double* X, int d, const int64_t* rows, const int64_t* cand, int64_t n, int kk, double* out,
                                       meld_stream_t stream) {
  MELD_CHECK_ARG(X && rows && cand && out && d > 0 && n >= 0 && kk > 0, "meld_knn_pair_distances: bad arguments");
  if (n == 0) return MELD_OK;
  hipLaunchKernelGGL(pair_distances_kernel, dim3((unsigned)ceil_div(n * kk, 256)), dim3(256), 0, S(stream), X, d, rows, cand, n, kk, out);
  MELD_LAUNCH_CHECK("pair_distances_kernel");
  return MELD_OK;
}
```

### meld_amd/graph.py

```python
from __future__ import annotations

from ._options import opt

import math
import time

from types import SimpleNamespace

import numpy as np
import torch

from ._lib import check, get_lib, ptr
from .knn_plan import SearchOptions, plan_knn_search, search_nprod, sphere_layout

__all__ = ["DeviceGraph", "build_knn_graph", "default_ksel", "EVENTS", "record_events"]

EVENTS = {"enabled": False, "pairs": []}


def record_events(enabled=True):
    EVENTS["enabled"] = bool(enabled)
    EVENTS["pairs"] = []


class _EventSpan:
    def __init__(self, name, **meta):
        self.name, self.meta = name, meta

    def __enter__(self):
        if EVENTS["enabled"]:
            self.a = torch.cuda.Event(enable_timing=True)
            self.b = torch.cuda.Event(enable_timing=True)
            self.a.record()
        return self

    def __exit__(self, *exc):
        if EVENTS["enabled"]:
            self.b.record()
            EVENTS["pairs"].append((self.name, self.a, self.b, self.meta))
        return False


def event_times_ms():
    out = {}
    for name, a, b, meta in EVENTS["pairs"]:
        out.setdefault(name, []).append(a.elapsed_time(b))
    return out


def _stream():
    return torch.cuda.current_stream().cuda_stream


def default_ksel(knn):
    k = 4 * (knn + 1)
    k = ((k + 31) // 32) * 32
    return int(min(128, max(32, k)))


class _Timer:

    def __init__(self, enabled):
        self.enabled = enabled
        self.t = {}
        self._t0 = None

# ... 412 lines not shown
                return False
            At = np.zeros((d, int(lib.meld_frame_max_dims())))
            At[:, :d] = evecs[:, ::-1].T
            return torch.from_numpy(At).to(X.device, non_blocking=True)

        return finish

    def principal_frame(self, X, mean, lead, comm=None, axes=None):
        lib, st = self.lib, _stream()
        N, d = int(X.shape[0]), int(X.shape[1])
        if axes is not None and (comm is None or getattr(comm, "world", 1) == 1):
            At = axes(lead)
            if At is False:
                return None
            out = torch.empty_like(X)
            check(lib.meld_rotate_rows_f64(ptr(X), N, d, ptr(mean), ptr(At), ptr(out), st), "meld_rotate_rows_f64")
            return out
        wide = d > int(lib.meld_frame_max_dims())
        stride = max(1, N // 32768)
        if wide:
            Xs = X[::stride] - mean
            cov = torch.triu(Xs.T @ Xs)
            del Xs
        else:
            cov = torch.zeros(d, d, dtype=torch.float64, device=X.device)
            check(lib.meld_cov_sample_f64(ptr(X), N, d, ptr(mean), stride, ptr(cov), st), "meld_cov_sample_f64")
        if comm is not None and getattr(comm, "world", 1) > 1:
            if comm.rank != 0:
                cov.zero_()
            comm.all_reduce_sum(cov)
        evals, evecs = _eigh_one_thread(cov.cpu().numpy())
        tot = float(evals.sum())
        if not np.isfinite(tot) or tot <= 0.0 or float(evals[-lead:].sum()) < 0.5 * tot:
            return None
        if wide:
            V = torch.from_numpy(np.ascontiguousarray(evecs[:, ::-1])).to(X.device)
            return torch.addmm(-(mean @ V), X, V)
        At = np.zeros((d, int(lib.meld_frame_max_dims())))
        At[:, :d] = evecs[:, ::-1].T
        At = torch.from_numpy(At).to(X.device)
        out = torch.empty_like(X)
        check(lib.meld_rotate_rows_f64(ptr(X), N, d, ptr(mean), ptr(At), ptr(out), st), "meld_rotate_rows_f64")
        return out

    def directed_kernel_coo(self, X, q_begin, q_count, knn, decay, thresh, ksel, tm=None, force_fallback=False, n_refs=None, assemble=False, comm=None,
                            bw_scale=1.0, bw_fixed=None, col_stats=None, knn_max=None, symm=(0, 0.0), count_rows_ge=None, frame_axes=None,
                            anisotropy=None):
        N = int(X.shape[0])
        NR = int(n_refs) if n_refs is not None else N
        if n_refs is not None and not (0 < NR <= q_begin and q_begin + q_count <= N):
            raise ValueError("cross search: the queries must lie behind the n_refs references")
        a = SimpleNamespace(X=X, N=N, d=int(X.shape[1]), NR=NR, cross=n_refs is not None, q_begin=q_begin, q_count=q_count, knn=knn, decay=decay,
                            thresh=thresh, bw_scale=bw_scale, bw_fixed=bw_fixed, knn_max=knn_max, force_fallback=force_fallback,
                            col_stats=col_stats, frame_axes=frame_axes, tm=tm or _Timer(False))
        r = self._search_and_refine(a, ksel, comm)
        retry_from = None
        if r.n_flag > max(1024, q_count // 100) and ksel < 128 and r.plan.search == "f16x3" and not force_fallback:
            retry_from, ksel = (ksel, r.n_flag), 128
            r = self._search_and_refine(a, ksel, None)
        s = self._exact_sweep(a, r, count_rows_ge)
        keys, vals, assembled = self._emit(a, r, s, ksel, assemble, symm, anisotropy)
        p, c = r.plan, r.cands
        info = dict(ksel=int(ksel), KP=int(c.KP), search=p.search, nprod=p.nprod, n_flagged_rows=r.n_flag,
                    prune=p.prune, radius_cut=p.radius_cut, seed=p.seed != "none", seeded_bounds=p.seeded_bounds, block_order=p.block_order != "none",
                    step_lists=p.lists != "none", principal_frame=p.frame, two_phase=p.two_pass, n_rows_bandwidth_recomputed=s.n_rebandwidth,
                    n_researched_rows=r.n_flag_stage1 if p.stage2 else 0, nnz_directed=r.m_main + s.fb_total,
                    wave_tiles_done=r.tiles_done_h, blocks_past_partial_test=r.blocks_on_h, pairs_past_filter=r.pairs_kept_h)
        if s.rows_at_least is not None:
            info["rows_with_at_least"] = s.rows_at_least
        if assembled is not None:
            info["assembled"] = assembled
        if retry_from is not None:
            info["ksel_retry_from"], info["n_flagged_rows_first_try"] = int(retry_from[0]), int(retry_from[1])
        return keys, vals, r.bw, info

    def _search_and_refine(self, a, ksel, comm):
        lib, dev = self.lib, a.X.device
        nprod = search_nprod(self.nprod, a.d)
        resident = lib.meld_knn16_resident_blocks(a.d, nprod) if lib.meld_knn16_kblocks(a.d) > 0 and nprod in (1, 3) else 0
        plan = plan_knn_search(lib, a.N, a.d, a.q_begin, a.q_count, a.knn, ksel, options=self, cross=a.cross, bandwidth=a.bw_fixed is not None,
                               world=getattr(comm, "world", 1) if comm is not None else 1, resident=resident)
        a.tm.start()
        col_min = col_max = None
        if a.col_stats is not None:
            sums, col_min, col_max = a.col_stats
            mean = sums / a.N
        elif a.d <= 256:
            sums, col_min, col_max = self.col_stats(a.X)
            mean = sums / a.N
        else:
            mean = a.X.mean(dim=0)
        norm2 = torch.empty(a.N, dtype=torch.float32, device=dev)
        nmax = torch.zeros(1, dtype=torch.float32, device=dev)
        if plan.search == "wide":
            c = self._candidates_wide(a, plan, ksel, mean, norm2, nmax)
        elif plan.search == "f32":
            c = self._candidates_f32(a, plan, ksel, mean, norm2, nmax)
        else:
            c = self._candidates_f16x3(a, plan, ksel, comm, mean, col_min, col_max, norm2, nmax)
        a.tm.stop("knn_topk")
        return self._refine(a, c, ksel)

    def _candidates_wide(self, a, plan, ksel, mean, norm2, nmax):
        dev, N, q_begin, q_count = a.X.device, a.N, a.q_begin, a.q_count
        cap = int(ksel)
        Xc = a.X - mean
        n2 = (Xc * Xc).sum(dim=1)
        norm2.copy_(n2.to(torch.float32))
        nmax.copy_(n2.max().to(torch.float32).reshape(1))
        a.tm.stop("prepare")
        kk = min(int(ksel), N)
        cand_idx = torch.zeros(q_count * cap, dtype=torch.int32, device=dev)
        cand_d2 = torch.full((q_count * cap,), float("inf"), dtype=torch.float32, device=dev)
        cand_cnt = torch.full((q_count,), kk, dtype=torch.int32, device=dev)
        QC, RC = 4096, 32768
        with _EventSpan("knn_topk", N=N, d=a.d, q=q_count):
            for q0 in range(0, q_count, QC):
                q1 = min(q_count, q0 + QC)
                Xq = Xc[q_begin + q0 : q_begin + q1]
                nq = n2[q_begin + q0 : q_begin + q1]
                best_d = torch.full((q1 - q0, 0), 0.0, dtype=torch.float64, device=dev)
                best_i = torch.zeros((q1 - q0, 0), dtype=torch.int64, device=dev)
                for r0 in range(0, N, RC):
                    r1 = min(N, r0 + RC)
                    D = nq[:, None] + n2[None, r0:r1] - 2.0 * (Xq @ Xc[r0:r1].T)
                    ids = torch.arange(r0, r1, device=dev, dtype=torch.int64)[None, :].expand(q1 - q0, -1)
                    D = torch.cat([best_d, D], dim=1)
                    ids = torch.cat([best_i, ids], dim=1)
                    best_d, sel = torch.topk(D, min(kk, D.shape[1]), dim=1, largest=False, sorted=True)
                    best_i = torch.gather(ids, 1, sel)
                rows = torch.arange(q0, q1, device=dev, dtype=torch.int64)[:, None] * cap + torch.arange(kk, device=dev)[None, :]
                cand_d2[rows.reshape(-1)] = best_d.clamp_(min=0.0).to(torch.float32).reshape(-1)
                cand_idx[rows.reshape(-1)] = best_i.to(torch.int32).reshape(-1)
        return SimpleNamespace(plan=plan, idx=cand_idx, d2=cand_d2, cnt=cand_cnt, thr=None, cap=cap, err_coef=1e-6, err_lin=0.0, KP=a.d,
# ... 108 lines not shown
            check(lib.meld_knn16_tile_spheres(ptr(X_s), N, d, ptr(mean_s), ptr(o.scale_info), ptr(tmpb), t0s, max(t1s - t0s, 0), st), "meld_knn16_tile_spheres")
            parts = (tmpb[: rows_c * row_b], tmpb[rows_c * row_b : rows_c * (row_b + 4)], tmpb[rows_c * (row_b + 4) : rows_c * (row_b + 8)])
            for arr, width in zip(parts, (row_b, 4, 4)):
                mine = arr[comm.rank * per * width : (comm.rank + 1) * per * width].clone()
                comm.all_gather_rows(arr, mine)
        lb2 = step_list = step_cnt = None
        if plan.lists == "direct":
            step_list = torch.empty(n_blocks * n_tiles, dtype=torch.int32, device=dev)
            step_cnt = torch.empty(n_blocks, dtype=torch.int32, device=dev)
            scratch = torch.empty(lib.meld_knn16_list_scratch_bytes(N), dtype=torch.uint8, device=dev)
            check((lib.meld_knn16_step_lists_direct_spheres if spheres_ready else lib.meld_knn16_step_lists_direct_lead)(ptr(X_s), N, d, ptr(mean_s), ptr(o.scale_info), ptr(nmax), ptr(o.Rt), ptr(seeds), ptr(o.Qn), plan.nprod,
                ptr(tmpb), ptr(scratch), ptr(step_list), n_tiles, ptr(step_cnt), int(plan.lead_bounds), st),
                  "meld_knn16_step_lists_direct")
            del scratch
        else:
            sb = plan.seeded_bounds
            lb2 = torch.empty(lib.meld_knn16_bounds_bytes(N, a.q_count), dtype=torch.uint8, device=dev)
            check((lib.meld_knn16_bounds_from_spheres if plan.bounds == "bounds_from_spheres" or spheres_ready else lib.meld_knn16_bounds)(
                ptr(X_s), N, d, ptr(mean_s), ptr(o.scale_info), ptr(nmax), ptr(o.Rt), a.q_begin, a.q_count, ptr(seeds) if sb else None,
                ptr(o.Qn) if sb else None, plan.nprod, ptr(tmpb), ptr(lb2), st), "meld_knn16_bounds")
            if plan.lists == "table":
                step_list = torch.empty(n_blocks * n_tiles, dtype=torch.int32, device=dev)
                step_cnt = torch.empty(n_blocks, dtype=torch.int32, device=dev)
                check(lib.meld_knn16_step_lists(ptr(lb2), ptr(seeds), N, d, a.q_count, plan.nprod, ptr(nmax), ptr(o.scale_info), a.q_begin,
                                                ptr(step_list), n_tiles, ptr(step_cnt), st), "meld_knn16_step_lists")
        work = step_cnt
        if plan.block_order == "work":
            work = torch.empty(n_blocks, dtype=torch.int32, device=dev)
            check(lib.meld_knn16_block_work(ptr(lb2), ptr(seeds), N, d, a.q_count, plan.nprod, ptr(nmax), ptr(o.scale_info), ptr(work), st), "meld_knn16_block_work")
        block_order = torch.argsort(work, descending=True, stable=True).to(torch.int32) if plan.block_order != "none" else None
        a.tm.stop("bounds")
        return lb2, step_list, step_cnt, block_order

    def _search16(self, a, plan, o, c, ksel, seeds, rfac, lists):
        lib, st, dev, d, q_count, q_pad, cap = self.lib, _stream(), a.X.device, a.d, a.q_count, o.q_pad, c.cap
        lb2, step_list, step_cnt, block_order = lists
        q0 = 0 if a.cross else a.q_begin
        tiles_b = c.tiles_done
        if plan.two_pass:
            with _EventSpan("knn_filter", N=a.N, d=d, q=q_count):
                check(lib.meld_knn16_partial_filter(ptr(o.Q), ptr(o.Qn), ptr(o.Rt), ptr(o.scale_info), ptr(c.nmax), d, q_count, ptr(seeds), ptr(step_list),
                                                    ptr(step_cnt), o.n_tiles, ptr(step_cnt), ptr(c.tiles_done), ptr(block_order), st), "meld_knn16_partial_filter")
                if block_order is not None:
                    block_order = torch.argsort(step_cnt, descending=True, stable=True).to(torch.int32)
            tiles_b = c.tiles_done[1:]
            a.tm.stop("knn_filter")
        S = plan.main_slices
        with _EventSpan("knn_topk", N=a.N, d=d, q=q_count):
            if S > 1:
                out = (torch.empty(S * q_pad * cap, dtype=torch.int32, device=dev), torch.empty(S * q_pad * cap, dtype=torch.float32, device=dev),
                       torch.empty(S * q_pad, dtype=torch.int32, device=dev), torch.full((S, q_pad), float("inf"), dtype=torch.float32, device=dev))
            else:
                out = (c.idx, c.d2, c.cnt, c.thr)
            if step_list is not None:
                check(lib.meld_knn16_topk_listed_partial(ptr(o.Q), ptr(o.Qn), ptr(o.Rt), ptr(o.scale_info), a.NR, d, q_count, ksel, ptr(step_list), ptr(step_cnt),
                                                         o.n_tiles, ptr(c.nmax), q0, ptr(seeds), plan.knn_cut, rfac, *map(ptr, out), ptr(tiles_b), ptr(block_order),
                                                         S, int(plan.partial_in_search), st), "meld_knn16_topk_listed")
            else:
                check(lib.meld_knn16_topk(ptr(o.Q), ptr(o.Qn), ptr(o.Rt), ptr(o.scale_info), a.NR, d, q_count, ksel, plan.nprod, S, ptr(lb2), ptr(c.nmax), q0,
                                          ptr(seeds), plan.knn_cut, rfac, *map(ptr, out), ptr(c.tiles_done), ptr(block_order), st), "meld_knn16_topk")
            if S > 1:
                check(lib.meld_knn16_merge_slices(*map(ptr, out[:3]), q_count, ksel, S, ptr(c.idx), ptr(c.d2), ptr(c.cnt), st), "meld_knn16_merge_slices")
                c.thr.copy_(out[3].amin(0))
            del out
            while _WHILE_SEARCHING:
                _WHILE_SEARCHING.pop()()
        del o.Q

    def _refine(self, a, c, ksel):
        lib, st, dev, q_count = self.lib, _stream(), a.X.device, a.q_count
        r = SimpleNamespace(plan=c.plan, cands=c)
        max_rank = 0 if a.knn_max is None else int(a.knn_max) + 1
        r.bw = torch.empty(q_count, dtype=torch.float64, device=dev)
        r.cand_val = torch.empty(q_count * ksel, dtype=torch.float64, device=dev)
        r.keep_cnt = torch.empty(q_count, dtype=torch.int32, device=dev)
        r.flag_rows = torch.empty(q_count, dtype=torch.int32, device=dev)
        n_flag = torch.zeros(1, dtype=torch.int32, device=dev)
        nmax_used = c.nmax
        if a.force_fallback:
            nmax_used = torch.full((1,), float("inf"), dtype=torch.float32, device=dev)
        check(
            lib.meld_knn_refine(
                ptr(a.X), a.N, a.d, a.q_begin, q_count, ptr(c.idx), ptr(c.d2), ptr(c.cnt), ptr(c.thr), ksel, c.cap, a.knn, float(a.decay),
                float(a.thresh), ptr(nmax_used), float(c.err_coef), ptr(c.norm2), float(c.err_lin), ptr(r.bw), ptr(r.cand_val), ptr(r.keep_cnt),
                ptr(r.flag_rows), ptr(n_flag), None, 0, None, float(a.bw_scale), ptr(a.bw_fixed), max_rank, st,
            ),
            "meld_knn_refine",
        )
        r.n_flag = r.n_flag_stage1 = int(n_flag.item())
        a.tm.stop("refine")
        stage2 = c.research is not None and r.n_flag > 0 and not a.force_fallback
        if stage2:
            self._stage2(a, c, r, ksel, n_flag, max_rank)
        c.research = None
        r.keep_off = _scan_i32(lib, r.keep_cnt, st)
        td, p = c.tiles_done, c.plan
        heads = [n_flag[0].to(torch.int64), r.keep_off[q_count]] + ([td[0], td[2] if p.two_pass else td[1], td[1]] if td is not None else [])
        heads_h = torch.stack(heads).tolist()
        if stage2:
            r.n_flag = int(heads_h[0])
        r.m_main = int(heads_h[1])
        r.tiles_done_h = int(heads_h[2]) if td is not None else None
        r.blocks_on_h = int(heads_h[3]) if td is not None and p.frame else None
        r.pairs_kept_h = int(heads_h[4]) if td is not None and p.two_pass else None
        if r.pairs_kept_h is not None and lib.meld_knn16_kblocks(a.d) > 7:
            r.blocks_on_h = 2 * r.pairs_kept_h
        return r

    def _stage2(self, a, c, r, ksel, n_flag, max_rank):
        lib, st, dev, d, cap, o = self.lib, _stream(), a.X.device, a.d, c.cap, c.research
        n_flag_h = r.n_flag
        rows2 = torch.sort(r.flag_rows[:n_flag_h]).values.contiguous()
        q2_pad = ((n_flag_h + o.BQ - 1) // o.BQ) * o.BQ
        Q2 = torch.empty(q2_pad * lib.meld_knn16_query_bytes(d), dtype=torch.uint8, device=dev)
        Qn2 = torch.empty(q2_pad, dtype=torch.float32, device=dev)
        check(lib.meld_knn16_prepare_rows(ptr(o.X_s), a.N, d, ptr(o.mean_s), ptr(o.scale_info), a.q_begin, ptr(rows2), n_flag_h, ptr(Q2), ptr(Qn2), st), "meld_knn16_prepare_rows")
        n_blocks2 = q2_pad // o.BQ
        resident = lib.meld_knn16_resident_blocks(d, 3)
        if resident < 0:
            check(resident, "meld_knn16_resident_blocks")
        n_slices = int(max(1, min(lib.meld_knn16_max_slices(ksel), 2 * resident // max(n_blocks2, 1), o.n_tiles)))
        thr2 = torch.empty(q2_pad, dtype=torch.float32, device=dev)
        check(lib.meld_knn16_research_thresholds(ptr(rows2), n_flag_h, a.q_begin, ptr(c.cnt), ptr(c.d2), cap, ksel, ptr(c.norm2), ptr(c.nmax),
                                                 float(c.err_coef), float(c.err_lin), float(lib.meld_knn16_error_coef(3, d)),
                                                 ptr(o.scale_info), ptr(thr2), st), "meld_knn16_research_thresholds")
        c2_idx = torch.empty(n_slices * q2_pad * cap, dtype=torch.int32, device=dev)
        c2_d2 = torch.empty(n_slices * q2_pad * cap, dtype=torch.float32, device=dev)
        c2_cnt = torch.empty(n_slices * q2_pad, dtype=torch.int32, device=dev)
        with _EventSpan("knn_topk_stage2", N=a.N, d=d, q=n_flag_h):
            check(lib.meld_knn16_topk(ptr(Q2), ptr(Qn2), ptr(o.Rt), ptr(o.scale_info), a.NR, d, n_flag_h, ksel, 3, n_slices, None, ptr(c.nmax), 0, ptr(thr2), 0, 1.0,
                                      ptr(c2_idx), ptr(c2_d2), ptr(c2_cnt), None, None, None, st), "meld_knn16_topk(stage 2)")
            if n_slices > 1:
                m_idx = torch.empty(q2_pad * cap, dtype=torch.int32, device=dev)
                m_d2 = torch.empty(q2_pad * cap, dtype=torch.float32, device=dev)
                m_cnt = torch.empty(q2_pad, dtype=torch.int32, device=dev)
                check(lib.meld_knn16_merge_slices(ptr(c2_idx), ptr(c2_d2), ptr(c2_cnt), n_flag_h, ksel, n_slices, ptr(m_idx), ptr(m_d2), ptr(m_cnt), st), "meld_knn16_merge_slices")
                c2_idx, c2_d2, c2_cnt = m_idx, m_d2, m_cnt
        n_flag.zero_()
        check(
            lib.meld_knn_refine(
                ptr(a.X), a.N, d, a.q_begin, n_flag_h, ptr(c2_idx), ptr(c2_d2), ptr(c2_cnt), None, ksel, cap, a.knn, float(a.decay),
                float(a.thresh), ptr(c.nmax), float(lib.meld_knn16_error_coef(3, d)), None, 0.0, ptr(r.bw), ptr(r.cand_val), ptr(r.keep_cnt),
                ptr(r.flag_rows), ptr(n_flag), ptr(rows2), cap, ptr(c.idx), float(a.bw_scale), ptr(a.bw_fixed), max_rank, st,
            ),
            "meld_knn_refine(stage 2)",
        )
        a.tm.stop("knn_stage2")

    def _exact_sweep(self, a, r, count_rows_ge):
        lib, st, dev, q_count, n_flag_h = self.lib, _stream(), a.X.device, a.q_count, r.n_flag
        knn_chk = a.knn if a.bw_fixed is None else 2**31 - 1
        s = SimpleNamespace(n_rebandwidth=0, fb_total=0, fb_off=None, fb_col=None, fb_val=None, fb_cnt=None, rows_at_least=None)
        if n_flag_h > 0:
            r.flag_rows = flag_rows = torch.sort(r.flag_rows[:n_flag_h]).values.contiguous()
            fb_cnt = torch.empty(n_flag_h, dtype=torch.int32, device=dev)
            err = torch.zeros(1, dtype=torch.int32, device=dev)
            cursor = torch.zeros(n_flag_h, dtype=torch.int32, device=dev)

            def sweep(fill, what, fb_cnt=None, fb_off=None, fb_col=None, fb_val=None, err=None):
                check(lib.meld_knn_radius_exact(ptr(a.X), a.NR, a.d, a.q_begin, ptr(flag_rows), n_flag_h, ptr(r.bw), knn_chk, float(a.decay), float(a.thresh), fill,
                                                ptr(fb_cnt), ptr(fb_off), ptr(cursor), ptr(fb_col), ptr(fb_val), ptr(err), float(a.bw_scale), st), what)

            sweep(0, "meld_knn_radius_exact(count)", fb_cnt=fb_cnt, err=err)
            if int(err.item()) != 0:
                bad = torch.nonzero(fb_cnt < 0).reshape(-1)
                rows_bad = flag_rows[bad].to(torch.int64)
                r.bw[rows_bad] = _exact_bandwidth(a.X, a.q_begin + rows_bad, a.knn, n_refs=a.NR)
                fb_cnt.zero_()
                cursor.zero_()
                err.zero_()
                sweep(0, "meld_knn_radius_exact(recount)", fb_cnt=fb_cnt, err=err)
                if int(err.item()) != 0:
                    raise NotImplementedError(
                        "degenerate neighbourhoods: the exact sweep could not settle the bandwidth of {} rows".format(int((fb_cnt < 0).sum())))
                s.n_rebandwidth = int(bad.shape[0])
            fb_off = _scan_i32(lib, fb_cnt, st)
            fb_total = int(fb_off[n_flag_h].item())
            need = 12 * fb_total + 32 * (r.m_main + fb_total)
            if need > torch.cuda.get_device_properties(dev).total_memory:
                raise MemoryError(
                    "the kernel radius covers {:.3g} neighbours per cell on average: the graph would hold {:.3g} entries ({:.0f} GB to "
                    "assemble) -- raise decay or thresh".format((r.m_main + fb_total) / max(q_count, 1), float(r.m_main + fb_total), need / 1e9))
            fb_col = torch.empty(max(fb_total, 1), dtype=torch.int32, device=dev)
            fb_val = torch.empty(max(fb_total, 1), dtype=torch.float64, device=dev)
            sweep(1, "meld_knn_radius_exact(fill)", fb_off=fb_off, fb_col=fb_col, fb_val=fb_val)
            if a.knn_max is not None and fb_total > 0 and int(fb_cnt.max()) > int(a.knn_max):
                rows_e = torch.repeat_interleave(torch.arange(n_flag_h, device=dev), fb_cnt.to(torch.int64))
                o = torch.argsort(fb_col[:fb_total].to(torch.int64), stable=True)
                o = o[torch.argsort(-fb_val[:fb_total][o], stable=True)]
                o = o[torch.argsort(rows_e[o], stable=True)]
                rank = torch.arange(fb_total, device=dev) - fb_off[:n_flag_h][rows_e[o]]
                keep = o[rank < int(a.knn_max)]
                keep = keep[torch.argsort(rows_e[keep], stable=True)]
                fb_col, fb_val = fb_col[keep].contiguous(), fb_val[keep].contiguous()
                fb_cnt = torch.clamp(fb_cnt, max=int(a.knn_max))
                fb_off = _scan_i32(lib, fb_cnt, st)
                fb_total = int(fb_off[n_flag_h].item())
            s.fb_total, s.fb_off, s.fb_col, s.fb_val, s.fb_cnt = fb_total, fb_off, fb_col, fb_val, fb_cnt
        a.tm.stop("radius_exact")
        if count_rows_ge is not None:
            tot = r.keep_cnt.to(torch.int64)
            if n_flag_h > 0 and s.fb_total > 0:
                tot = tot.clone()
                tot[r.flag_rows[:n_flag_h].to(torch.int64)] = s.fb_cnt.to(torch.int64)
            s.rows_at_least = int(((tot + 1) >= int(count_rows_ge)).sum())
        return s

    def _emit(self, a, r, s, ksel, assemble, symm, anisotropy=None):
        lib, st, dev, q_count, n_flag_h, c = self.lib, _stream(), a.X.device, a.q_count, r.n_flag, r.cands
        M = r.m_main + s.fb_total
        assembled = None
        if assemble and M > 0 and a.q_begin == 0 and q_count == a.NR and not a.cross and opt("MELD_ASSEMBLE", "bucket") == "bucket" \
                and opt("MELD_ASSEMBLE_FUSED", "1") != "0":
            B = int(lib.meld_csr_bucket_slots())
            if ksel <= B and q_count * B * 12 <= torch.cuda.mem_get_info(dev)[0] // 4:
                cursor = r.keep_cnt.clone()
                if n_flag_h > 0 and s.fb_total > 0:
                    cursor[r.flag_rows[:n_flag_h].to(torch.int64)] = s.fb_cnt
                tcol = torch.empty(q_count * B, dtype=torch.int32, device=dev)
                tval = torch.empty(q_count * B, dtype=torch.float64, device=dev)
                check(lib.meld_coo_emit_scatter(q_count, ptr(c.idx), ptr(r.cand_val), ksel, c.cap, ptr(r.keep_cnt), ptr(r.flag_rows), n_flag_h,
                                                ptr(s.fb_off), ptr(s.fb_col), ptr(s.fb_val), s.fb_total, ptr(cursor), ptr(tcol), ptr(tval), st),
                      "meld_coo_emit_scatter")
                a.tm.stop("coo_emit")
                aniso = anisotropy if opt("MELD_ASSEMBLE_FUSED_ANISO", "1") != "0" else None
                assembled = self._finish_buckets(cursor, tcol, tval, q_count, sums_diag=1.0, symm=symm, anisotropy=aniso)
                if assembled is not None and self.last_row_sums is not None:
                    assembled = assembled + (self.last_row_sums[1],)
                    if self.last_degrees is not None:
                        assembled = assembled + (self.last_degrees,)
                a.tm.stop("symmetrize")
                del cursor, tcol, tval
        keys = vals = None
        if assembled is None:
            keys = torch.empty(2 * M, dtype=torch.int64, device=dev)
            vals = torch.empty(2 * M, dtype=torch.float64, device=dev)
            if M > 0:
                check(
                    lib.meld_coo_emit(
                        a.q_begin, q_count, ptr(c.idx), ptr(r.cand_val), ptr(c.cnt), ksel, c.cap, ptr(r.keep_off), ptr(r.flag_rows),
                        n_flag_h, ptr(s.fb_off), ptr(s.fb_col), ptr(s.fb_val), r.m_main, M, ptr(keys), ptr(vals), st,
                    ),
                    "meld_coo_emit",
                )
        a.tm.stop("coo_emit")
        return keys, vals, assembled

    def sort_pairs(self, keys, vals, N):
        lib, st = self.lib, _stream()
        n = int(keys.shape[0])
        keys2 = torch.empty_like(keys)
        vals2 = torch.empty_like(vals)
        if n == 0:
            return keys2, vals2
        tb = lib.meld_sort_temp_bytes(n)
        tmp = torch.empty(tb, dtype=torch.uint8, device=keys.device)
        end_bit = 32 + max(1, int(N - 1).bit_length())
        check(lib.meld_sort_pairs_u64_f64(ptr(keys), ptr(keys2), ptr(vals), ptr(vals2), n, end_bit, ptr(tmp), tb, st), "meld_sort_pairs_u64_f64")
        return keys2, vals2

    def partition_remote(self, keys, vals, rows_per_rank, world, rank, cap):
        dev = keys.device
        counts = torch.empty(world, dtype=torch.int32, device=dev)
        send = torch.empty(world * 2 * cap, dtype=torch.int64, device=dev)
        check(self.lib.meld_coo_partition_remote(ptr(keys), ptr(vals), int(keys.shape[0]), int(rows_per_rank), int(world), int(rank),
                                                 int(cap), ptr(counts), ptr(send), _stream()), "meld_coo_partition_remote")
        return send, counts

    def _finish_buckets(self, cursor, tcol, tval, n_rows, sums_diag=None, symm=(0, 0.0), anisotropy=None):
        lib, st, dev = self.lib, _stream(), cursor.device
        i32 = dict(dtype=torch.int32, device=dev)
        ucnt = torch.empty(n_rows, **i32)
        flags = torch.empty(1, **i32)
        fused = anisotropy is not None and sums_diag is not None
        if fused:
            sums = torch.empty(n_rows, dtype=torch.float64, device=dev)
            check(lib.meld_csr_rows_sort_merge_sums(ptr(cursor), n_rows, ptr(tcol), ptr(tval), ptr(ucnt), ptr(flags), int(symm[0]), float(symm[1]),
                                                    float(sums_diag), ptr(sums), st), "meld_csr_rows_sort_merge_sums")
        else:
            check(lib.meld_csr_rows_sort_merge(ptr(cursor), n_rows, ptr(tcol), ptr(tval), ptr(ucnt), ptr(flags), int(symm[0]), float(symm[1]), st), "meld_csr_rows_sort_merge")
        rowptr = _scan_i32(lib, ucnt, st)
        nnz, flag = (int(v) for v in torch.stack([rowptr[n_rows], flags[0].to(torch.int64)]).tolist())
        if flag != 0:
            return None
        col = torch.empty(nnz, **i32)
# ... 474 lines not shown
```

### meld_amd/knn_plan.py

```python
from __future__ import annotations

import ctypes
import dataclasses
from dataclasses import dataclass
from typing import Optional

from ._lib import check
from ._options import opt


@dataclass(frozen=True)
class SearchOptions:

    search: str = "f16x3"
    nprod: int = 1
    prune: bool = True
    radius_cut: bool = True
    seed: bool = True
    seeded_bounds: bool = True
    block_order: bool = True
    rotate: bool = True
    rotate_min_cells: int = 262144

    @classmethod
    def from_env(cls, search=None, prune=None, nprod=None):
        out = cls(search=search or opt("MELD_KNN_SEARCH", "f16x3"), nprod=1 if nprod is None else int(nprod),
                  prune=(opt("MELD_KNN_PRUNE", "1") != "0") if prune is None else bool(prune),
                  rotate=opt("MELD_KNN_ROTATE", "1") != "0", rotate_min_cells=int(opt("MELD_KNN_ROTATE_MIN", "262144")))
        if out.search not in ("f16x3", "f32"):
            raise ValueError("unknown search kernel {!r}".format(out.search))
        return out


@dataclass(frozen=True)
class KnnPlan:
    search: str
    nprod: int
    frame: bool
    radius_cut: bool
    prune: bool
    seed: str
    knn_cut: int
    bounds: str
    seeded_bounds: bool
    lists: str
    block_order: str
    main_slices: int
    two_pass: bool
    partial_in_search: bool
    stage2: bool
    lead_bounds: Optional[bool] = None
    partial_forced: bool = False
    fused_operands: bool = dataclasses.field(default=False, compare=False)

    def __post_init__(self):
        if self.lead_bounds is None:
            object.__setattr__(self, "lead_bounds", self.lists == "direct" and self.frame)

    def without_frame(self):
        return dataclasses.replace(self, frame=False, two_pass=False, lead_bounds=False,
                                   partial_in_search=self.partial_in_search and self.partial_forced)


def search_nprod(nprod, d):
    return 3 if (nprod == 1 and d <= 6) else nprod


def sphere_layout(lib, N, d):
    rows, row_bytes = ctypes.c_int64(0), ctypes.c_int64(0)
    check(lib.meld_knn16_sphere_layout(N, d, ctypes.byref(rows), ctypes.byref(row_bytes)), "meld_knn16_sphere_layout")
    return int(rows.value), int(row_bytes.value)


def plan_knn_search(lib, N, d, q_begin, q_count, knn, ksel, *, options, cross=False, bandwidth=False, world=1, resident=0):
    search = options.search
    if search == "f16x3" and lib.meld_knn16_kblocks(d) < 0:
        search = "wide"
    if cross and search != "f16x3":
        raise NotImplementedError("the search between two point sets runs on the split-fp16 MFMA kernel only (d <= 141)")
    if search != "f16x3":
        return KnnPlan(search, options.nprod, False, False, False, "none", knn, "none", False, "none", "none", 1, False, False, False)
    nprod = search_nprod(options.nprod, d)
    TS, BQ = lib.meld_knn16_tile_refs(), lib.meld_knn16_block_queries()
    n_blocks, n_tiles = -(-q_count // BQ), -(-N // TS)
    radius_cut = bool(options.radius_cut) and knn < ksel
    frame = bool(options.rotate and lib.meld_knn16_split_dims(d) > 0 and nprod == 1 and not cross and options.prune and options.seed
                 and N >= max(16384, options.rotate_min_cells) and q_begin % BQ == 0 and not bandwidth)
    prune = bool(options.prune) and q_begin % TS == 0 and N >= 16384 and not cross
    seed = "none"
    if bandwidth and radius_cut:
        seed = "bandwidth"
    elif options.seed and radius_cut and q_begin % BQ == 0 and not cross:
        seed = "mfma"
    bounds, lists, block_order, seeded_bounds, main_slices = "none", "none", "none", False, 1
    if prune:
        seeded_bounds = seed != "none" and bool(options.seeded_bounds)
        shared = world > 1 and sphere_layout(lib, N, d)[0] % world == 0
        want_lists = seed != "none" and radius_cut and nprod == 1
        if want_lists and seeded_bounds and not shared and q_begin == 0 and q_count == N and opt("MELD_KNN_LIST_DIRECT", "1") != "0":
            lists = "direct"
        else:
            bounds = "bounds_from_spheres" if shared else "bounds"
            lists = "table" if want_lists else "none"
        if options.block_order and n_blocks > 1:
            block_order = "lists" if lists != "none" else "work"
        if radius_cut and resident > 0 and n_blocks < 2 * resident:
            main_slices = int(max(1, min(4, lib.meld_knn16_max_slices(ksel), -(-2 * resident // n_blocks), n_tiles // 64)))
    ee = opt("MELD_KNN16_EE")
    partial = frame if ee is None else ee != "0"
    two = opt("MELD_KNN_TWO_PHASE", "1")
    two_pass = lists != "none" and frame and (main_slices == 1 or two == "2") and two != "0" and ee is None
    lead_bounds = lists == "direct" and frame and opt("MELD_KNN16_LEAD_BOUNDS", "1") != "0"
    fused = prune and bounds != "bounds_from_spheres" and q_begin == 0 and q_count == N and opt("MELD_KNN_FUSED_OPERANDS", "1") != "0"
    return KnnPlan(search, nprod, frame, radius_cut, prune, seed, 0 if seed == "bandwidth" else knn, bounds, seeded_bounds, lists,
                   block_order, main_slices, two_pass, partial, nprod == 1, lead_bounds, ee is not None, fused)
```

Baseline: 28.44 million.

## Fuse kNN row finishing, refine and COO bucket emission into per-row kernels

Adds a raw listed top-k variant that skips the in-kernel row finish, plus a fused refine kernel that sorts each row's candidates with a register bitonic sort, computes kernel values and scatters them straight into CSR row buckets. Stage-2 re-searched rows are then emitted through a listed scatter that claims bucket slots atomically. This removes the intermediate cand_val array and separate finish and emit passes, cutting global memory traffic and kernel launches. In exchange, bucket writes become atomic and depend on claim ordering, and the path is gated on even d, ksel <= 128 and a single device.

Result: faster. 29.32 million (median of 6 runs) (+3.1%).

```diff
diff --git a/include/meld_hip.h b/include/meld_hip.h
--- a/include/meld_hip.h
+++ b/include/meld_hip.h
@@ -121,6 +121,13 @@
                                    double radius_factor, int32_t* cand_idx, float* cand_d2, int32_t* cand_cnt, float* cand_thr,
                                    uint64_t* tiles_done, const int32_t* block_order, int n_slices, int partial_test,
                                    meld_stream_t stream);
+int meld_knn16_topk_listed_raw(const void* Q16, const float* Qn, const void* Rt16, const float* scale_info, int64_t n_ref, int d,
+                               int64_t q_count, int ksel, const uint32_t* step_list, const int32_t* step_cnt, int64_t list_stride,
+                               const float* norm2_max, int64_t q_begin, const float* thr_init, int knn, double radius_factor,
+                               int32_t* cand_idx, float* cand_d2, int32_t* cand_cnt, float* cand_thr, uint64_t* tiles_done,
+                               const int32_t* block_order, int partial_test, meld_stream_t stream);
+int meld_knn16_finish_rows(float* cand_d2, int32_t* cand_idx, int32_t* cand_cnt, const float* Qn, const float* scale_info, int64_t n_rows,
+                           int ksel, meld_stream_t stream);
 int meld_knn16_partial_filter(const void* Q16, const float* Qn, const void* Rt16, const float* scale_info, const float* norm2_max, int d,
                               int64_t q_count, const float* thr_init, uint32_t* step_list, const int32_t* step_cnt, int64_t list_stride,
                               int32_t* cnt_out, uint64_t* tested, const int32_t* block_order , meld_stream_t stream);
@@ -143,6 +150,17 @@
                     const double* bw_fixed ,
                     int max_rank ,
                     meld_stream_t stream);
+
+int meld_knn_refine_emit(const double* X, int64_t N, int d, const int32_t* cand_idx, const float* cand_d2, const int32_t* cand_cnt,
+                         const float* cand_thr, int ksel, int cap, int knn, double decay, double thresh, const float* norm2_max,
+                         double err_coef, const float* norm2, double err_coef_lin, double* bw, int32_t* keep_cnt,
+                         int32_t* flag_rows, int32_t* n_flag, double bw_scale, const double* bw_fixed, int max_rank,
+                         int32_t* cursor, int32_t* tcol, double* tval, meld_stream_t stream);
+int meld_knn_refine_sort_emit(const double* X, int64_t N, int d, int32_t* cand_idx, float* cand_d2, int32_t* cand_cnt, const float* Qn,
+                              const float* scale_info, const float* cand_thr, int ksel, int cap, int knn, double decay, double thresh,
+                              const float* norm2_max, double err_coef, const float* norm2, double err_coef_lin, double* bw,
+                              int32_t* keep_cnt, int32_t* flag_rows, int32_t* n_flag, double bw_scale, const double* bw_fixed, int max_rank,
+                              int32_t* cursor, int32_t* tcol, double* tval, meld_stream_t stream);
 
 int meld_knn_radius_exact(const double* X, int64_t N, int d, int64_t q_begin, const int32_t* flag_rows,
                           int32_t n_flag, const double* bw, int knn, double decay, double thresh,
@@ -209,6 +227,10 @@
                           const int32_t* keep_cnt, const int32_t* flag_rows, int32_t n_flag, const int64_t* fb_off,
                           const int32_t* fb_col, const double* fb_val, int64_t fb_total, int32_t* cursor, int32_t* tcol,
                           double* tval, meld_stream_t stream);
+int meld_coo_emit_scatter_listed(const int32_t* rows, int32_t n_rows, const int32_t* cand_idx, const double* cand_val, int ksel,
+                                 int cap, const int32_t* keep_cnt, const int32_t* flag_rows, int32_t n_flag, const int64_t* fb_off,
+                                 const int32_t* fb_col, const double* fb_val, int64_t fb_total, int32_t* cursor, int32_t* tcol,
+                                 double* tval, meld_stream_t stream);
 int meld_csr_bucket_slots(void);
 int meld_coo_scatter_rows(const uint64_t* keys, const double* vals, int64_t n, int64_t row_begin, int64_t n_rows,
                           int32_t* cursor, int32_t* tcol, double* tval, meld_stream_t stream);
diff --git a/meld_amd/_lib.py b/meld_amd/_lib.py
--- a/meld_amd/_lib.py
+++ b/meld_amd/_lib.py
@@ -29,6 +29,16 @@
         _i32,
         [_ptr, _i64, _i32, _i64, _i64, _ptr, _ptr, _ptr, _ptr, _i32, _i32, _i32, _f64, _f64, _ptr, _f64, _ptr, _f64, _ptr, _ptr, _ptr,
          _ptr, _ptr, _ptr, _i32, _ptr, _f64, _ptr, _i32, _ptr],
+    ),
+    "meld_knn_refine_emit": (
+        _i32,
+        [_ptr, _i64, _i32, _ptr, _ptr, _ptr, _ptr, _i32, _i32, _i32, _f64, _f64, _ptr, _f64, _ptr, _f64, _ptr, _ptr, _ptr, _ptr, _f64, _ptr,
+         _i32, _ptr, _ptr, _ptr, _ptr],
+    ),
+    "meld_knn_refine_sort_emit": (
+        _i32,
+        [_ptr, _i64, _i32, _ptr, _ptr, _ptr, _ptr, _ptr, _ptr, _i32, _i32, _i32, _f64, _f64, _ptr, _f64, _ptr, _f64, _ptr, _ptr, _ptr, _ptr, _f64,
+         _ptr, _i32, _ptr, _ptr, _ptr, _ptr],
     ),
     "meld_knn_error_coef": (_f64, [_i32]),
     "meld_knn16_kblocks": (_i32, [_i32]),
@@ -63,6 +73,8 @@
     "meld_knn16_step_lists_direct_lead": (_i32, [_ptr, _i64, _i32, _ptr, _ptr, _ptr, _ptr, _ptr, _ptr, _i32, _ptr, _ptr, _ptr, _i64, _ptr, _i32, _ptr]),
     "meld_knn16_topk_listed": (_i32, [_ptr, _ptr, _ptr, _ptr, _i64, _i32, _i64, _i32, _ptr, _ptr, _i64, _ptr, _i64, _ptr, _i32, _f64, _ptr, _ptr, _ptr, _ptr, _ptr, _ptr, _i32, _ptr]),
     "meld_knn16_topk_listed_partial": (_i32, [_ptr, _ptr, _ptr, _ptr, _i64, _i32, _i64, _i32, _ptr, _ptr, _i64, _ptr, _i64, _ptr, _i32, _f64, _ptr, _ptr, _ptr, _ptr, _ptr, _ptr, _i32, _i32, _ptr]),
+    "meld_knn16_topk_listed_raw": (_i32, [_ptr, _ptr, _ptr, _ptr, _i64, _i32, _i64, _i32, _ptr, _ptr, _i64, _ptr, _i64, _ptr, _i32, _f64, _ptr, _ptr, _ptr, _ptr, _ptr, _ptr, _i32, _ptr]),
+    "meld_knn16_finish_rows": (_i32, [_ptr, _ptr, _ptr, _ptr, _ptr, _i64, _i32, _ptr]),
     "meld_knn16_partial_filter": (_i32, [_ptr, _ptr, _ptr, _ptr, _ptr, _i32, _i64, _ptr, _ptr, _ptr, _i64, _ptr, _ptr, _ptr, _ptr]),
     "meld_knn16_seed_thresholds_mfma": (_i32, [_ptr, _ptr, _ptr, _ptr, _ptr, _i64, _i32, _i64, _i64, _i32, _f64, _i32, _i32, _ptr, _ptr]),
     "meld_knn16_max_slices": (_i32, [_i32]),
@@ -101,6 +113,7 @@
     "meld_csr_bucket_slots": (_i32, []),
     "meld_coo_scatter_rows": (_i32, [_ptr, _ptr, _i64, _i64, _i64, _ptr, _ptr, _ptr, _ptr]),
     "meld_coo_emit_scatter": (_i32, [_i64, _ptr, _ptr, _i32, _i32, _ptr, _ptr, _i32, _ptr, _ptr, _ptr, _i64, _ptr, _ptr, _ptr, _ptr]),
+    "meld_coo_emit_scatter_listed": (_i32, [_ptr, _i32, _ptr, _ptr, _i32, _i32, _ptr, _ptr, _i32, _ptr, _ptr, _ptr, _i64, _ptr, _ptr, _ptr, _ptr]),
     "meld_coo_partition_remote": (_i32, [_ptr, _ptr, _i64, _i64, _i32, _i32, _i64, _ptr, _ptr, _ptr]),
     "meld_csr_rows_sort_merge": (_i32, [_ptr, _i64, _ptr, _ptr, _ptr, _ptr, _i32, _f64, _ptr]),
     "meld_csr_compact_rows": (_i32, [_ptr, _i64, _ptr, _ptr, _ptr, _ptr, _ptr]),
diff --git a/meld_amd/build.py b/meld_amd/build.py
--- a/meld_amd/build.py
+++ b/meld_amd/build.py
@@ -105,7 +105,7 @@
     hipcc = _hipcc()
     objdir = os.path.join(_HERE, "build")
     os.makedirs(objdir, exist_ok=True)
-    headers = [os.path.join(CSRC, "common.hpp"), os.path.join(_HERE, "..", "include", "meld_hip.h")]
+    headers = [os.path.join(CSRC, "common.hpp"), os.path.join(CSRC, "k16_rows.hpp"), os.path.join(_HERE, "..", "include", "meld_hip.h")]
     procs = []
     objs = []
     for src in SOURCES:
diff --git a/meld_amd/csrc/assemble.hip b/meld_amd/csrc/assemble.hip
--- a/meld_amd/csrc/assemble.hip
+++ b/meld_amd/csrc/assemble.hip
@@ -272,7 +272,6 @@
   *run_len = next - lane;
 }
 
-constexpr int CSR_BUCKET = 256;
 
 __global__ __launch_bounds__(256) void coo_scatter_rows_kernel(const unsigned long long* __restrict__ keys,
                                                                const double* __restrict__ vals, int64_t n, int64_t row_begin,
@@ -339,15 +338,22 @@
   }
 }
 
+template <bool CLAIM>
 __global__ __launch_bounds__(256) void coo_emit_scatter_rows_kernel(int64_t q_count, const int* __restrict__ cand_idx,
                                                                     const double* __restrict__ cand_val, int ksel, int cap,
                                                                     const int* __restrict__ keep_cnt, int* __restrict__ cursor,
-                                                                    int* __restrict__ tcol, double* __restrict__ tval) {
+                                                                    int* __restrict__ tcol, double* __restrict__ tval,
+                                                                    const int* __restrict__ rows) {
   const int lane = threadIdx.x & 63;
-  const int64_t q = (int64_t)blockIdx.x * 4 + (threadIdx.x >> 6);
-  if (q >= q_count) return;
+  const int64_t qi = (int64_t)blockIdx.x * 4 + (threadIdx.x >> 6);
+  if (qi >= q_count) return;
+  const int64_t q = CLAIM ? (int64_t)rows[qi] : qi;
   if (keep_cnt[q] == 0) return;
   int written = 0;
+  if constexpr (CLAIM) {
+    if (lane == 0) written = atomicAdd(cursor + q, keep_cnt[q]);
+    written = __builtin_amdgcn_readfirstlane(written);
+  }
   for (int c0 = 0; c0 < ksel; c0 += 64) {
     const int c = c0 + lane;
     double v = 0.0;
@@ -361,8 +367,10 @@
     if (keep) {
       const int pos = written + __popcll(b & ((1ull << lane) - 1ull));
       const double hv = 0.5 * v;
-      tcol[q * CSR_BUCKET + pos] = j;
-      tval[q * CSR_BUCKET + pos] = hv;
+      if (!CLAIM || pos < CSR_BUCKET) {
+        tcol[q * CSR_BUCKET + pos] = j;
+        tval[q * CSR_BUCKET + pos] = hv;
+      }
       const int slot = atomicAdd(cursor + j, 1);
       if (slot < CSR_BUCKET) {
         tcol[(int64_t)j * CSR_BUCKET + slot] = (int)q;
@@ -372,6 +380,7 @@
     written += __popcll(b);
   }
 }
+template <bool CLAIM>
 __global__ __launch_bounds__(256) void coo_emit_scatter_fallback_kernel(const int* __restrict__ flag_rows, int n_flag,
                                                                         const int64_t* __restrict__ fb_off,
                                                                         const int* __restrict__ fb_col,
@@ -386,7 +395,7 @@
     if (fb_off[mid] <= e) lo = mid; else hi = mid - 1;
   }
   const int64_t q = flag_rows[lo];
-  const int64_t pos = e - fb_off[lo];
+  const int64_t pos = CLAIM ? (int64_t)atomicAdd(cursor + q, 1) : e - fb_off[lo];
   const int j = fb_col[e];
   const double hv = 0.5 * fb_val[e];
   if (pos < CSR_BUCKET) {
@@ -693,14 +702,36 @@
   MELD_CHECK_ARG(cand_idx && cand_val && keep_cnt && cursor && tcol && tval && q_count > 0, "meld_coo_emit_scatter: bad arguments");
   MELD_CHECK_ARG(cap >= ksel && ksel <= CSR_BUCKET, "meld_coo_emit_scatter: ksel=%d must fit a row bucket (%d) and the row stride cap=%d",
                  ksel, CSR_BUCKET, cap);
-  hipLaunchKernelGGL(coo_emit_scatter_rows_kernel, dim3((unsigned)ceil_div(q_count, 4)), dim3(256), 0, S(stream), q_count, cand_idx,
-                     cand_val, ksel, cap, keep_cnt, cursor, tcol, tval);
+  hipLaunchKernelGGL(coo_emit_scatter_rows_kernel<false>, dim3((unsigned)ceil_div(q_count, 4)), dim3(256), 0, S(stream), q_count, cand_idx,
+                     cand_val, ksel, cap, keep_cnt, cursor, tcol, tval, (const int*)nullptr);
   MELD_LAUNCH_CHECK("coo_emit_scatter_rows_kernel");
   if (n_flag > 0 && fb_total > 0) {
     MELD_CHECK_ARG(flag_rows && fb_off && fb_col && fb_val, "meld_coo_emit_scatter: missing fallback arrays");
-    hipLaunchKernelGGL(coo_emit_scatter_fallback_kernel, dim3((unsigned)ceil_div(fb_total, 256)), dim3(256), 0, S(stream), flag_rows,
+    hipLaunchKernelGGL(coo_emit_scatter_fallback_kernel<false>, dim3((unsigned)ceil_div(fb_total, 256)), dim3(256), 0, S(stream), flag_rows,
                        n_flag, fb_off, fb_col, fb_val, fb_total, cursor, tcol, tval);
     MELD_LAUNCH_CHECK("coo_emit_scatter_fallback_kernel");
+  }
+  return MELD_OK;
+}
+
+extern "C" int meld_coo_emit_scatter_listed(const int32_t* rows, int32_t n_rows, const int32_t* cand_idx, const double* cand_val, int ksel,
+                                            int cap, const int32_t* keep_cnt, const int32_t* flag_rows, int32_t n_flag,
+                                            const int64_t* fb_off, const int32_t* fb_col, const double* fb_val, int64_t fb_total,
+                                            int32_t* cursor, int32_t* tcol, double* tval, meld_stream_t stream) {
+  MELD_CHECK_ARG(cursor && tcol && tval && n_rows >= 0 && n_flag >= 0 && fb_total >= 0, "meld_coo_emit_scatter_listed: bad arguments");
+  if (n_rows > 0) {
+    MELD_CHECK_ARG(rows && cand_idx && cand_val && keep_cnt, "meld_coo_emit_scatter_listed: missing candidate arrays");
+    MELD_CHECK_ARG(cap >= ksel && ksel >= 1 && ksel <= CSR_BUCKET, "meld_coo_emit_scatter_listed: ksel=%d must fit a row bucket (%d) and the row stride cap=%d",
+                   ksel, CSR_BUCKET, cap);
+    hipLaunchKernelGGL(coo_emit_scatter_rows_kernel<true>, dim3((unsigned)ceil_div(n_rows, 4)), dim3(256), 0, S(stream), (int64_t)n_rows,
+                       cand_idx, cand_val, ksel, cap, keep_cnt, cursor, tcol, tval, rows);
+    MELD_LAUNCH_CHECK("coo_emit_scatter_rows_kernel<listed>");
+  }
+  if (n_flag > 0 && fb_total > 0) {
+    MELD_CHECK_ARG(flag_rows && fb_off && fb_col && fb_val, "meld_coo_emit_scatter_listed: missing fallback arrays");
+    hipLaunchKernelGGL(coo_emit_scatter_fallback_kernel<true>, dim3((unsigned)ceil_div(fb_total, 256)), dim3(256), 0, S(stream), flag_rows,
+                       n_flag, fb_off, fb_col, fb_val, fb_total, cursor, tcol, tval);
+    MELD_LAUNCH_CHECK("coo_emit_scatter_fallback_kernel<claim>");
   }
   return MELD_OK;
 }
diff --git a/meld_amd/csrc/common.hpp b/meld_amd/csrc/common.hpp
--- a/meld_amd/csrc/common.hpp
+++ b/meld_amd/csrc/common.hpp
@@ -52,6 +52,8 @@
 
 static inline int64_t ceil_div(int64_t a, int64_t b) { return (a + b - 1) / b; }
 
+constexpr int CSR_BUCKET = 256;
+
 static inline const char* meld_dev_getenv(const char* name) {
   const char* dev = getenv("MELD_DEV");
   return (dev && dev[0] == '1' && dev[1] == 0) ? getenv(name) : nullptr;
diff --git a/meld_amd/csrc/k16_rows.hpp b/meld_amd/csrc/k16_rows.hpp
--- /dev/null
+++ b/meld_amd/csrc/k16_rows.hpp
@@ -0,0 +1,50 @@
+#pragma once
+#include "common.hpp"
+
+namespace meld {
+
+constexpr int K16_ROW_CAPMAX = 256;
+constexpr int K16_ROW_SLOTS = K16_ROW_CAPMAX / 64;
+
+__device__ __forceinline__ unsigned ordered_bits(float f) {
+  const unsigned b = __float_as_uint(f);
+  return (b & 0x80000000u) ? ~b : (b | 0x80000000u);
+}
+__device__ __forceinline__ float from_ordered_bits(unsigned k) {
+  return __uint_as_float((k & 0x80000000u) ? (k & 0x7fffffffu) : ~k);
+}
+
+template <int SL>
+__device__ __forceinline__ void k16_bitonic_sort(unsigned long long (&key)[SL], int lane) {
+  constexpr int NE = 64 * SL;
+#pragma unroll
+  for (int k = 2; k <= NE; k <<= 1) {
+#pragma unroll
+    for (int j = k >> 1; j > 0; j >>= 1) {
+      if (j >= 64) {
+        const int je = j >> 6;
+#pragma unroll
+        for (int e = 0; e < SL; ++e) {
+          if ((e & je) == 0) {
+            const int i = 64 * e + lane;
+            const bool asc = (i & k) == 0;
+            const unsigned long long a = key[e], b = key[e | je];
+            const bool sw = asc ? (b < a) : (a < b);
+            key[e] = sw ? b : a;
+            key[e | je] = sw ? a : b;
+          }
+        }
+      } else {
+#pragma unroll
+        for (int e = 0; e < SL; ++e) {
+          const int i = 64 * e + lane;
+          const unsigned long long o = __shfl_xor(key[e], j, 64);
+          const bool keep_min = ((i & j) == 0) == ((i & k) == 0);
+          key[e] = keep_min ? (o < key[e] ? o : key[e]) : (o < key[e] ? key[e] : o);
+        }
+      }
+    }
+  }
+}
+
+}
diff --git a/meld_amd/csrc/knn16.hip b/meld_amd/csrc/knn16.hip
--- a/meld_amd/csrc/knn16.hip
+++ b/meld_amd/csrc/knn16.hip
@@ -1,4 +1,5 @@
 #include "common.hpp"
+#include "k16_rows.hpp"
 
 #include <hip/hip_fp16.h>
 
@@ -11,7 +12,7 @@
 constexpr int K16_THREADS = 256;
 constexpr int K16_NWAVE = K16_THREADS / 64;
 constexpr int K16_SLACK = 128;
-constexpr int K16_CAPMAX = 256;
+constexpr int K16_CAPMAX = K16_ROW_CAPMAX;
 constexpr int K16_BOUNDS_THREADS = 1024;
 constexpr int K16_SLOTS = K16_CAPMAX / 64;
 constexpr int K16_DMAX = 16 * 9 - 3;
@@ -46,10 +47,6 @@
   return __builtin_fminf(min3f(a, b, v[15]), min3f(c, d, e));
 }
 
-__device__ __forceinline__ unsigned ordered_bits(float f) {
-  const unsigned b = __float_as_uint(f);
-  return (b & 0x80000000u) ? ~b : (b | 0x80000000u);
-}
 
 __device__ __forceinline__ float ld_sc1_f(const float* p) {
   return __hip_atomic_load(p, __ATOMIC_RELAXED, __HIP_MEMORY_SCOPE_AGENT);
@@ -70,9 +67,6 @@
 }
 __device__ __forceinline__ int knn16_split_pos(int pos, int m0, int half) { return pos < m0 ? pos : half + (pos - m0); }
 
-__device__ __forceinline__ float from_ordered_bits(unsigned k) {
-  return __uint_as_float((k & 0x80000000u) ? (k & 0x7fffffffu) : ~k);
-}
 
 __device__ float knn16_squeeze_row(int n0, int n1, int half, int ksel, int knn1, float rf2, float err, float nq_row,
                                    float* __restrict__ d2row, int* __restrict__ idxrow, int lane, int* n0_out,
@@ -977,38 +971,6 @@
 }
 
 template <int SL>
-__device__ __forceinline__ void k16_bitonic_sort(unsigned long long (&key)[SL], int lane) {
-  constexpr int NE = 64 * SL;
-#pragma unroll
-  for (int k = 2; k <= NE; k <<= 1) {
-#pragma unroll
-    for (int j = k >> 1; j > 0; j >>= 1) {
-      if (j >= 64) {
-        const int je = j >> 6;
-#pragma unroll
-        for (int e = 0; e < SL; ++e) {
-          if ((e & je) == 0) {
-            const int i = 64 * e + lane;
-            const bool asc = (i & k) == 0;
-            const unsigned long long a = key[e], b = key[e | je];
-            const bool sw = asc ? (b < a) : (a < b);
-            key[e] = sw ? b : a;
-            key[e | je] = sw ? a : b;
-          }
-        }
-      } else {
-#pragma unroll
-        for (int e = 0; e < SL; ++e) {
-          const int i = 64 * e + lane;
-          const unsigned long long o = __shfl_xor(key[e], j, 64);
-          const bool keep_min = ((i & j) == 0) == ((i & k) == 0);
-          key[e] = keep_min ? (o < key[e] ? o : key[e]) : (o < key[e] ? key[e] : o);
-        }
-      }
-    }
-  }
-}
-template <int SL>
 __device__ __forceinline__ void k16_finish_row(float* __restrict__ drow, int* __restrict__ irow, int n0, int half, int n_all, int n,
                                                float add, float out_scale, int lane) {
   unsigned long long key[SL];
@@ -2430,8 +2392,10 @@
                          const float* norm2_max, int64_t q_begin, const float* thr_init, int knn,
                          double radius_factor, int32_t* cand_idx, float* cand_d2, int32_t* cand_cnt,
                          float* cand_thr, uint64_t* tiles_done, const int32_t* block_order, const uint32_t* step_list,
-                         const int32_t* step_cnt, int64_t list_stride, meld_stream_t stream, int partial_test = 0, int two_counters = 0) {
+                         const int32_t* step_cnt, int64_t list_stride, meld_stream_t stream, int partial_test = 0, int two_counters = 0,
+                         bool finish = true) {
   MELD_CHECK_ARG(nprod == 1 || nprod == 3, "meld_knn16_topk: nprod must be 1 or 3");
+  MELD_CHECK_ARG(finish || n_slices == 1, "meld_knn16_topk_listed_raw: raw rows go with one slice (the merge of slices takes finished rows)");
   MELD_CHECK_ARG(step_list == nullptr || (step_cnt != nullptr && nprod == 1 && lb2 == nullptr && thr_init != nullptr),
                  "meld_knn16_topk_listed: step lists go with the hi-only pass, start thresholds and no table");
   MELD_CHECK_ARG(n_slices >= 1 && n_slices * ksel <= K16_MERGE_MAX, "meld_knn16_topk: n_slices=%d must satisfy n_slices * ksel <= %d",
@@ -2521,10 +2485,12 @@
   }
 #undef K16_CASE
   MELD_LAUNCH_CHECK("knn16_topk_kernel");
-  const int64_t n_rows = (int64_t)grid.x * K16_BQ * grid.y;
-  hipLaunchKernelGGL(knn16_finish_rows_kernel, dim3((unsigned)ceil_div(n_rows, 4)), dim3(256), 0, S(stream), cand_d2, cand_idx, cand_cnt, Qn,
-                     scale_info, n_rows, (int64_t)grid.y * K16_BQ, cap, ksel);
-  MELD_LAUNCH_CHECK("knn16_finish_rows_kernel");
+  if (finish) {
+    const int64_t n_rows = (int64_t)grid.x * K16_BQ * grid.y;
+    hipLaunchKernelGGL(knn16_finish_rows_kernel, dim3((unsigned)ceil_div(n_rows, 4)), dim3(256), 0, S(stream), cand_d2, cand_idx, cand_cnt, Qn,
+                       scale_info, n_rows, (int64_t)grid.y * K16_BQ, cap, ksel);
+    MELD_LAUNCH_CHECK("knn16_finish_rows_kernel");
+  }
   if (stats) {
     unsigned long long st[13] = {0, 0, 0, 0, 0, 0, 0, 0, 0, 0, 0, 0, 0};
     MELD_HIP_CALL(hipStreamSynchronize(S(stream)));
@@ -2577,6 +2543,28 @@
   return k16_topk_impl(Q16, Qn, Rt16, scale_info, n_ref, d, q_count, ksel, 1, n_slices, nullptr, norm2_max, q_begin, thr_init, knn,
                        radius_factor, cand_idx, cand_d2, cand_cnt, cand_thr, tiles_done, block_order, step_list, step_cnt, list_stride,
                        stream, partial_test, 1);
+}
+
+extern "C" int meld_knn16_topk_listed_raw(const void* Q16, const float* Qn, const void* Rt16, const float* scale_info, int64_t n_ref,
+                                          int d, int64_t q_count, int ksel, const uint32_t* step_list, const int32_t* step_cnt,
+                                          int64_t list_stride, const float* norm2_max, int64_t q_begin, const float* thr_init, int knn,
+                                          double radius_factor, int32_t* cand_idx, float* cand_d2, int32_t* cand_cnt, float* cand_thr,
+                                          uint64_t* tiles_done, const int32_t* block_order, int partial_test, meld_stream_t stream) {
+  MELD_CHECK_ARG(step_list && step_cnt && list_stride > 0, "meld_knn16_topk_listed_raw: null step lists");
+  return k16_topk_impl(Q16, Qn, Rt16, scale_info, n_ref, d, q_count, ksel, 1, 1, nullptr, norm2_max, q_begin, thr_init, knn,
+                       radius_factor, cand_idx, cand_d2, cand_cnt, cand_thr, tiles_done, block_order, step_list, step_cnt, list_stride,
+                       stream, partial_test, 1, false);
+}
+
+extern "C" int meld_knn16_finish_rows(float* cand_d2, int32_t* cand_idx, int32_t* cand_cnt, const float* Qn, const float* scale_info,
+                                      int64_t n_rows, int ksel, meld_stream_t stream) {
+  MELD_CHECK_ARG(cand_d2 && cand_idx && cand_cnt && Qn && scale_info && n_rows > 0, "meld_knn16_finish_rows: bad arguments");
+  const int cap = meld_knn16_row_capacity(ksel);
+  if (cap < 0) return cap;
+  hipLaunchKernelGGL(knn16_finish_rows_kernel, dim3((unsigned)ceil_div(n_rows, 4)), dim3(256), 0, S(stream), cand_d2, cand_idx, cand_cnt, Qn,
+                     scale_info, n_rows, n_rows, cap, ksel);
+  MELD_LAUNCH_CHECK("knn16_finish_rows_kernel");
+  return MELD_OK;
 }
 
 extern "C" int meld_knn16_partial_filter(const void* Q16, const float* Qn, const void* Rt16, const float* scale_info, const float* norm2_max,
diff --git a/meld_amd/csrc/refine.hip b/meld_amd/csrc/refine.hip
--- a/meld_amd/csrc/refine.hip
+++ b/meld_amd/csrc/refine.hip
@@ -1,7 +1,9 @@
 #include "common.hpp"
+#include "k16_rows.hpp"
 
 #include <algorithm>
 #include <cfloat>
+#include <cstdint>
 
 namespace meld {
 
@@ -48,7 +50,23 @@
   return v;
 }
 
-template <bool COOP>
+template <int SL>
+__device__ __forceinline__ void rf_rank_raw_row(const float* drow, const int* irow, int n0, int half, int n_all, int lane,
+                                                unsigned long long (&out)[2]) {
+  unsigned long long key[SL];
+#pragma unroll
+  for (int e = 0; e < SL; ++e) {
+    const int i = lane + 64 * e;
+    const int p = i < n0 ? i : half + (i - n0);
+    key[e] = ~0ull;
+    if (i < n_all) key[e] = ((unsigned long long)ordered_bits(drow[p] + 0.0f) << 32) | (unsigned)irow[p];
+  }
+  k16_bitonic_sort<SL>(key, lane);
+  out[0] = key[0];
+  out[1] = SL > 1 ? key[SL > 1 ? 1 : 0] : ~0ull;
+}
+
+template <bool COOP, bool EMIT = false, bool RAW = false>
 __global__ __launch_bounds__(256) void refine_kernel(
     const double* __restrict__ X, int d, int64_t q_begin, int64_t q_count, const int* __restrict__ cand_idx,
     const float* __restrict__ cand_d2, const int* __restrict__ cand_cnt, const float* __restrict__ cand_thr, int ksel,
@@ -56,7 +74,10 @@
     const float* __restrict__ norm2, double err_coef_lin, double bw_scale, const double* __restrict__ bw_fixed, int max_rank,
     double* __restrict__ bw_out, double* __restrict__ cand_val, int* __restrict__ keep_cnt,
     int* __restrict__ flag_rows, int* __restrict__ n_flag, const int* __restrict__ rows, int out_cap,
-    int* __restrict__ cand_idx_out) {
+    int* __restrict__ cand_idx_out, int* __restrict__ cursor = nullptr, int* __restrict__ tcol = nullptr,
+    double* __restrict__ tval = nullptr, int* raw_idx = nullptr, float* raw_d2 = nullptr, int* raw_cnt = nullptr,
+    const float* __restrict__ Qn = nullptr, const float* __restrict__ scale_info = nullptr) {
+  static_assert((COOP || !EMIT) && (EMIT || !RAW), "the emitting forms exist for the four-chain kernel only");
   const int lane = threadIdx.x & 63;
   const int64_t q = (int64_t)blockIdx.x * 4 + (threadIdx.x >> 6);
   if (q >= q_count) return;
@@ -66,7 +87,27 @@
   const size_t ro = (size_t)q * cap;
   int idx_raw[2] = {0, 0};
   float d2_raw[2] = {0.0f, 0.0f}, d2_knn = 0.0f;
-  if constexpr (COOP) {
+  int n_raw = 0;
+  if constexpr (RAW) {
+    const int packed = raw_cnt[q];
+    const int n0 = packed & 0xffff, n_all = n0 + ((packed >> 16) & 0xffff);
+    const float add = Qn[q], out_scale = scale_info[1];
+    unsigned long long key[2];
+    if (n_all <= 64)
+      rf_rank_raw_row<1>(raw_d2 + ro, raw_idx + ro, n0, cap >> 1, n_all, lane, key);
+    else if (n_all <= 128)
+      rf_rank_raw_row<2>(raw_d2 + ro, raw_idx + ro, n0, cap >> 1, n_all, lane, key);
+    else
+      rf_rank_raw_row<K16_ROW_SLOTS>(raw_d2 + ro, raw_idx + ro, n0, cap >> 1, n_all, lane, key);
+#pragma unroll
+    for (int e = 0; e < 2; ++e) {
+      idx_raw[e] = (int)(unsigned)key[e];
+      d2_raw[e] = (from_ordered_bits((unsigned)(key[e] >> 32)) + add) * out_scale;
+    }
+    const float k_lo = __shfl(d2_raw[0], knn & 63, 64), k_hi = __shfl(d2_raw[1], knn & 63, 64);
+    d2_knn = knn < 64 ? k_lo : k_hi;
+    n_raw = min(n_all, ksel);
+  } else if constexpr (COOP) {
 #pragma unroll
     for (int e = 0; e < 2; ++e) {
       const int cc = min(lane + 64 * e, cap - 1);
@@ -75,7 +116,9 @@
     }
     d2_knn = cand_d2[ro + min(knn, cap - 1)];
   }
-  const int n = min(cand_cnt[q], ksel);
+  int n_list;
+  if constexpr (RAW) n_list = n_raw; else n_list = min(cand_cnt[q], ksel);
+  const int n = n_list;
 
   double E = err_coef * (double)norm2_max[0];
   if (norm2 != nullptr && err_coef_lin > 0.0) E += err_coef_lin * sqrt((double)norm2[gi] * (double)norm2_max[0]);
@@ -231,7 +274,12 @@
   const double radius = bw * radius_factor;
   const double reach = bw_fixed != nullptr ? radius : fmax(radius, bw_raw);
   double tau = INFINITY;
-  if (cand_cnt[q] >= ksel) tau = (double)cand_d2[ro + ksel - 1];
+  if constexpr (RAW) {
+    const float t_lo = __shfl(d2_raw[0], (ksel - 1) & 63, 64), t_hi = __shfl(d2_raw[1], (ksel - 1) & 63, 64);
+    if (n >= ksel) tau = (double)(ksel <= 64 ? t_lo : t_hi);
+  } else {
+    if (cand_cnt[q] >= ksel) tau = (double)cand_d2[ro + ksel - 1];
+  }
   if (cand_thr != nullptr) tau = fmin(tau, (double)cand_thr[q]);
   bool complete = (reach * reach + E <= tau);
   if (max_rank > 0) {
@@ -246,6 +294,8 @@
   if (bw_fixed == nullptr && n <= knn) complete = false;
 
   int kept = 0;
+  double vk[2];
+  unsigned long long kb[2];
 #pragma unroll
   for (int e = 0; e < 2; ++e) {
     const int c = lane + 64 * e;
@@ -255,11 +305,52 @@
       if (v < thresh || (int64_t)idx[e] == gi) v = 0.0;
       if (max_rank > 0 && rk[e] >= max_rank) v = 0.0;
     }
-    if (c < ksel) {
-      cand_val[(size_t)orow * ksel + c] = v;
-      if (cand_idx_out) cand_idx_out[(size_t)orow * out_cap + c] = (c < n) ? idx[e] : 0;
-    }
-    kept += __popcll(__ballot(v > 0.0));
+    if constexpr (!EMIT) {
+      if (c < ksel) {
+        cand_val[(size_t)orow * ksel + c] = v;
+        if (cand_idx_out) cand_idx_out[(size_t)orow * out_cap + c] = (c < n) ? idx[e] : 0;
+      }
+    }
+    vk[e] = v;
+    kb[e] = __ballot(v > 0.0);
+    kept += __popcll(kb[e]);
+  }
+  if constexpr (EMIT) {
+    if (kept > 0) {
+      int base = 0;
+      if (lane == 0) base = atomicAdd(cursor + gi, kept);
+      base = __builtin_amdgcn_readfirstlane(base);
+#pragma unroll
+      for (int e = 0; e < 2; ++e) {
+        if (vk[e] > 0.0) {
+          const int pos = base + (e ? __popcll(kb[0]) : 0) + __popcll(kb[e] & ((1ull << lane) - 1ull));
+          const int j = idx[e];
+          const double hv = 0.5 * vk[e];
+          if (pos < CSR_BUCKET) {
+            tcol[gi * CSR_BUCKET + pos] = j;
+            tval[gi * CSR_BUCKET + pos] = hv;
+          }
+          const int slot = atomicAdd(cursor + j, 1);
+          if (slot < CSR_BUCKET) {
+            tcol[(int64_t)j * CSR_BUCKET + slot] = (int)gi;
+            tval[(int64_t)j * CSR_BUCKET + slot] = hv;
+          }
+        }
+      }
+    }
+  }
+  if constexpr (RAW) {
+    if (!complete) {
+#pragma unroll
+      for (int e = 0; e < 2; ++e) {
+        const int c = lane + 64 * e;
+        if (c < n) {
+          raw_d2[ro + c] = d2_raw[e];
+          raw_idx[ro + c] = idx_raw[e];
+        }
+      }
+      if (lane == 0) raw_cnt[q] = n;
+    }
   }
   if (lane == 0) {
     bw_out[orow] = bw_raw;
@@ -450,6 +541,7 @@
   MELD_CHECK_ARG(err_coef >= 0 && err_coef_lin >= 0, "meld_knn_refine: error coefficients must be non-negative");
   MELD_CHECK_ARG(bw_scale > 0 && bw_scale < INFINITY, "meld_knn_refine: bandwidth_scale must be positive and finite");
   MELD_CHECK_ARG(max_rank == 0 || max_rank > knn, "meld_knn_refine: max_rank=%d must exceed knn=%d (or be 0)", max_rank, knn);
+  MELD_CHECK_ARG(!rf_four_chains(d) || ((uintptr_t)X & 15) == 0, "meld_knn_refine: X must be 16-byte aligned (even d <= %d)", RF_DMAX);
   const double radius_factor = pow(-log(thresh), 1.0 / decay);
 #define RF_LAUNCH(COOPV)                                                                                                          \
   hipLaunchKernelGGL(refine_kernel<COOPV>, dim3((unsigned)ceil_div(q_count, 4)), dim3(256), 0, S(stream), X, d, q_begin, q_count,  \
@@ -465,6 +557,62 @@
   return MELD_OK;
 }
 
+static int refine_emit_impl(const char* who, const double* X, int64_t N, int d, int32_t* cand_idx, float* cand_d2, int32_t* cand_cnt,
+                            const float* Qn, const float* scale_info, const float* cand_thr, int ksel, int cap, int knn, double decay,
+                            double thresh, const float* norm2_max, double err_coef, const float* norm2, double err_coef_lin, double* bw,
+                            int32_t* keep_cnt, int32_t* flag_rows, int32_t* n_flag, double bw_scale, const double* bw_fixed, int max_rank,
+                            int32_t* cursor, int32_t* tcol, double* tval, meld_stream_t stream) {
+  MELD_CHECK_ARG(X && cand_idx && cand_d2 && cand_cnt && norm2_max && bw && keep_cnt && flag_rows && n_flag && cursor && tcol && tval,
+                 "%s: null pointer", who);
+  MELD_CHECK_ARG(N > 0 && N < (int64_t)1 << 31 && rf_four_chains(d), "%s: needs 0 < N < 2^31 and an even d <= %d (d=%d)", who, RF_DMAX, d);
+  MELD_CHECK_ARG(((uintptr_t)X & 15) == 0, "%s: X must be 16-byte aligned", who);
+  MELD_CHECK_ARG(ksel >= 1 && ksel <= 128 && ksel <= CSR_BUCKET, "%s: ksel=%d outside [1,128]", who, ksel);
+  MELD_CHECK_ARG(knn >= 0 && decay > 0 && thresh > 0 && thresh <= 1, "%s: bad kernel parameters", who);
+  MELD_CHECK_ARG(cap >= ksel, "%s: row stride cap=%d smaller than ksel=%d", who, cap, ksel);
+  MELD_CHECK_ARG(Qn == nullptr || (cap <= K16_ROW_CAPMAX && (cap & 1) == 0), "%s: raw rows have an even stride of at most %d (cap=%d)", who,
+                 K16_ROW_CAPMAX, cap);
+  MELD_CHECK_ARG(err_coef >= 0 && err_coef_lin >= 0, "%s: error coefficients must be non-negative", who);
+  MELD_CHECK_ARG(bw_scale > 0 && bw_scale < INFINITY, "%s: bandwidth_scale must be positive and finite", who);
+  MELD_CHECK_ARG(max_rank == 0 || max_rank > knn, "%s: max_rank=%d must exceed knn=%d (or be 0)", who, max_rank, knn);
+  MELD_HIP_CALL(hipMemsetAsync(cursor, 0, sizeof(int32_t) * (size_t)N, S(stream)));
+  const double rf = pow(-log(thresh), 1.0 / decay);
+  const dim3 grid((unsigned)ceil_div(N, 4));
+  if (Qn == nullptr)
+    hipLaunchKernelGGL((refine_kernel<true, true, false>), grid, dim3(256), 0, S(stream), X, d, (int64_t)0, N, cand_idx, cand_d2, cand_cnt, cand_thr,
+                       ksel, cap, knn, decay, thresh, rf, norm2_max, err_coef, norm2, err_coef_lin, bw_scale, bw_fixed, max_rank, bw,
+                       (double*)nullptr, keep_cnt, flag_rows, n_flag, (const int*)nullptr, 0, (int*)nullptr, cursor, tcol, tval, (int*)nullptr,
+                       (float*)nullptr, (int*)nullptr, (const float*)nullptr, (const float*)nullptr);
+  else
+    hipLaunchKernelGGL((refine_kernel<true, true, true>), grid, dim3(256), 0, S(stream), X, d, (int64_t)0, N, (const int*)nullptr,
+                       (const float*)nullptr, (const int*)nullptr, cand_thr, ksel, cap, knn, decay, thresh, rf, norm2_max, err_coef, norm2,
+                       err_coef_lin, bw_scale, bw_fixed, max_rank, bw, (double*)nullptr, keep_cnt, flag_rows, n_flag, (const int*)nullptr, 0,
+                       (int*)nullptr, cursor, tcol, tval, cand_idx, cand_d2, cand_cnt, Qn, scale_info);
+  MELD_LAUNCH_CHECK("refine_kernel<emit>");
+  return MELD_OK;
+}
+
+extern "C" int meld_knn_refine_emit(const double* X, int64_t N, int d, const int32_t* cand_idx, const float* cand_d2, const int32_t* cand_cnt,
+                                    const float* cand_thr, int ksel, int cap, int knn, double decay, double thresh, const float* norm2_max,
+                                    double err_coef, const float* norm2, double err_coef_lin, double* bw, int32_t* keep_cnt,
+                                    int32_t* flag_rows, int32_t* n_flag, double bw_scale, const double* bw_fixed, int max_rank,
+                                    int32_t* cursor, int32_t* tcol, double* tval, meld_stream_t stream) {
+  return refine_emit_impl("meld_knn_refine_emit", X, N, d, const_cast<int32_t*>(cand_idx), const_cast<float*>(cand_d2),
+                          const_cast<int32_t*>(cand_cnt), nullptr, nullptr, cand_thr, ksel, cap, knn, decay, thresh, norm2_max, err_coef, norm2,
+                          err_coef_lin, bw, keep_cnt, flag_rows, n_flag, bw_scale, bw_fixed, max_rank, cursor, tcol, tval, stream);
+}
+
+extern "C" int meld_knn_refine_sort_emit(const double* X, int64_t N, int d, int32_t* cand_idx, float* cand_d2, int32_t* cand_cnt, const float* Qn,
+                                         const float* scale_info, const float* cand_thr, int ksel, int cap, int knn, double decay,
+                                         double thresh, const float* norm2_max, double err_coef, const float* norm2, double err_coef_lin,
+                                         double* bw, int32_t* keep_cnt, int32_t* flag_rows, int32_t* n_flag, double bw_scale,
+                                         const double* bw_fixed, int max_rank, int32_t* cursor, int32_t* tcol, double* tval,
+                                         meld_stream_t stream) {
+  MELD_CHECK_ARG(Qn && scale_info, "meld_knn_refine_sort_emit: null pointer");
+  return refine_emit_impl("meld_knn_refine_sort_emit", X, N, d, cand_idx, cand_d2, cand_cnt, Qn, scale_info, cand_thr, ksel, cap, knn, decay,
+                          thresh, norm2_max, err_coef, norm2, err_coef_lin, bw, keep_cnt, flag_rows, n_flag, bw_scale, bw_fixed, max_rank, cursor,
+                          tcol, tval, stream);
+}
+
 extern "C" int meld_knn_radius_exact(const double* X, int64_t N, int d, int64_t q_begin, const int32_t* flag_rows,
                                      int32_t n_flag, const double* bw, int knn, double decay, double thresh, int mode,
                                      int32_t* fb_cnt, const int64_t* fb_off, int32_t* fb_cursor, int32_t* fb_col,
@@ -472,6 +620,7 @@
   if (n_flag == 0) return MELD_OK;
   MELD_CHECK_ARG(bw_scale > 0 && bw_scale < INFINITY, "meld_knn_radius_exact: bandwidth_scale must be positive and finite");
   MELD_CHECK_ARG(X && flag_rows && bw && n_flag > 0 && N > 0 && d > 0, "meld_knn_radius_exact: bad arguments");
+  MELD_CHECK_ARG(!rf_four_chains(d) || ((uintptr_t)X & 15) == 0, "meld_knn_radius_exact: X must be 16-byte aligned (even d <= %d)", RF_DMAX);
   MELD_CHECK_ARG(mode == 0 ? (fb_cnt && err_flag && fb_cursor) : (fb_off && fb_cursor && fb_col && fb_val),
                  "meld_knn_radius_exact: missing output for mode %d", mode);
   const size_t lds = sizeof(double) * RB_FALL * (size_t)d;
@@ -510,6 +659,7 @@
 extern "C" int meld_knn_pair_distances(const double* X, int d, const int64_t* rows, const int64_t* cand, int64_t n, int kk, double* out,
                                        meld_stream_t stream) {
   MELD_CHECK_ARG(X && rows && cand && out && d > 0 && n >= 0 && kk > 0, "meld_knn_pair_distances: bad arguments");
+  MELD_CHECK_ARG(!rf_four_chains(d) || ((uintptr_t)X & 15) == 0, "meld_knn_pair_distances: X must be 16-byte aligned (even d <= %d)", RF_DMAX);
   if (n == 0) return MELD_OK;
   hipLaunchKernelGGL(pair_distances_kernel, dim3((unsigned)ceil_div(n * kk, 256)), dim3(256), 0, S(stream), X, d, rows, cand, n, kk, out);
   MELD_LAUNCH_CHECK("pair_distances_kernel");
diff --git a/meld_amd/graph.py b/meld_amd/graph.py
--- a/meld_amd/graph.py
+++ b/meld_amd/graph.py
@@ -11,7 +11,7 @@
 import torch
 
 from ._lib import check, get_lib, ptr
-from .knn_plan import SearchOptions, plan_knn_search, search_nprod, sphere_layout
+from .knn_plan import SearchOptions, bucket_route, plan_knn_search, search_nprod, sphere_layout
 
 __all__ = ["DeviceGraph", "build_knn_graph", "default_ksel", "EVENTS", "record_events"]
 
@@ -530,7 +530,16 @@
             raise ValueError("cross search: the queries must lie behind the n_refs references")
         a = SimpleNamespace(X=X, N=N, d=int(X.shape[1]), NR=NR, cross=n_refs is not None, q_begin=q_begin, q_count=q_count, knn=knn, decay=decay,
                             thresh=thresh, bw_scale=bw_scale, bw_fixed=bw_fixed, knn_max=knn_max, force_fallback=force_fallback,
-                            col_stats=col_stats, frame_axes=frame_axes, tm=tm or _Timer(False))
+                            col_stats=col_stats, frame_axes=frame_axes, tm=tm or _Timer(False), assemble=bool(assemble), rows_fused=True)
+        out = self._directed_kernel(a, ksel, comm, assemble, symm, count_rows_ge, anisotropy)
+        if out is None:
+            a.rows_fused = False
+            out = self._directed_kernel(a, ksel, comm, assemble, symm, count_rows_ge, anisotropy)
+            out[3]["fused_rows_recovered"] = True
+        return out
+
+    def _directed_kernel(self, a, ksel, comm, assemble, symm, count_rows_ge, anisotropy):
+        q_count, force_fallback = a.q_count, a.force_fallback
         r = self._search_and_refine(a, ksel, comm)
         retry_from = None
         if r.n_flag > max(1024, q_count // 100) and ksel < 128 and r.plan.search == "f16x3" and not force_fallback:
@@ -538,8 +547,11 @@
             r = self._search_and_refine(a, ksel, None)
         s = self._exact_sweep(a, r, count_rows_ge)
         keys, vals, assembled = self._emit(a, r, s, ksel, assemble, symm, anisotropy)
+        if r.buckets is not None and assembled is None and r.m_main + s.fb_total > 0:
+            return None
         p, c = r.plan, r.cands
         info = dict(ksel=int(ksel), KP=int(c.KP), search=p.search, nprod=p.nprod, n_flagged_rows=r.n_flag,
+                    fused_rows=p.fused_rows if p.fused_rows != "sort+emit" or getattr(c, "raw", None) is not None else "emit",
                     prune=p.prune, radius_cut=p.radius_cut, seed=p.seed != "none", seeded_bounds=p.seeded_bounds, block_order=p.block_order != "none",
                     step_lists=p.lists != "none", principal_frame=p.frame, two_phase=p.two_pass, n_rows_bandwidth_recomputed=s.n_rebandwidth,
                     n_researched_rows=r.n_flag_stage1 if p.stage2 else 0, nnz_directed=r.m_main + s.fb_total,
@@ -557,7 +569,9 @@
         nprod = search_nprod(self.nprod, a.d)
         resident = lib.meld_knn16_resident_blocks(a.d, nprod) if lib.meld_knn16_kblocks(a.d) > 0 and nprod in (1, 3) else 0
         plan = plan_knn_search(lib, a.N, a.d, a.q_begin, a.q_count, a.knn, ksel, options=self, cross=a.cross, bandwidth=a.bw_fixed is not None,
-                               world=getattr(comm, "world", 1) if comm is not None else 1, resident=resident)
+                               world=getattr(comm, "world", 1) if comm is not None else 1, resident=resident,
+                               assemble=a.assemble and a.rows_fused, free_bytes=torch.cuda.mem_get_info(dev)[0] if a.assemble and a.rows_fused else 0,
+                               x_aligned=a.X.data_ptr() % 16 == 0)
         a.tm.start()
         col_min = col_max = None
         if a.col_stats is not None:
@@ -772,7 +786,13 @@
                        torch.empty(S * q_pad, dtype=torch.int32, device=dev), torch.full((S, q_pad), float("inf"), dtype=torch.float32, device=dev))
             else:
                 out = (c.idx, c.d2, c.cnt, c.thr)
-            if step_list is not None:
+            c.raw = None
+            if step_list is not None and plan.fused_rows == "sort+emit" and S == 1:
+                check(lib.meld_knn16_topk_listed_raw(ptr(o.Q), ptr(o.Qn), ptr(o.Rt), ptr(o.scale_info), a.NR, d, q_count, ksel, ptr(step_list), ptr(step_cnt),
+                                                     o.n_tiles, ptr(c.nmax), q0, ptr(seeds), plan.knn_cut, rfac, *map(ptr, out), ptr(tiles_b), ptr(block_order),
+                                                     int(plan.partial_in_search), st), "meld_knn16_topk_listed_raw")
+                c.raw = (o.Qn, o.scale_info)
+            elif step_list is not None:
                 check(lib.meld_knn16_topk_listed_partial(ptr(o.Q), ptr(o.Qn), ptr(o.Rt), ptr(o.scale_info), a.NR, d, q_count, ksel, ptr(step_list), ptr(step_cnt),
                                                          o.n_tiles, ptr(c.nmax), q0, ptr(seeds), plan.knn_cut, rfac, *map(ptr, out), ptr(tiles_b), ptr(block_order),
                                                          S, int(plan.partial_in_search), st), "meld_knn16_topk_listed")
@@ -792,21 +812,35 @@
         r = SimpleNamespace(plan=c.plan, cands=c)
         max_rank = 0 if a.knn_max is None else int(a.knn_max) + 1
         r.bw = torch.empty(q_count, dtype=torch.float64, device=dev)
-        r.cand_val = torch.empty(q_count * ksel, dtype=torch.float64, device=dev)
         r.keep_cnt = torch.empty(q_count, dtype=torch.int32, device=dev)
         r.flag_rows = torch.empty(q_count, dtype=torch.int32, device=dev)
         n_flag = torch.zeros(1, dtype=torch.int32, device=dev)
         nmax_used = c.nmax
         if a.force_fallback:
             nmax_used = torch.full((1,), float("inf"), dtype=torch.float32, device=dev)
-        check(
-            lib.meld_knn_refine(
-                ptr(a.X), a.N, a.d, a.q_begin, q_count, ptr(c.idx), ptr(c.d2), ptr(c.cnt), ptr(c.thr), ksel, c.cap, a.knn, float(a.decay),
-                float(a.thresh), ptr(nmax_used), float(c.err_coef), ptr(c.norm2), float(c.err_lin), ptr(r.bw), ptr(r.cand_val), ptr(r.keep_cnt),
-                ptr(r.flag_rows), ptr(n_flag), None, 0, None, float(a.bw_scale), ptr(a.bw_fixed), max_rank, st,
-            ),
-            "meld_knn_refine",
-        )
+        r.buckets = r.cand_val = r.rows2 = None
+        if c.plan.fused_rows != "off":
+            B = int(lib.meld_csr_bucket_slots())
+            r.buckets = (torch.empty(q_count, dtype=torch.int32, device=dev), torch.empty(q_count * B, dtype=torch.int32, device=dev),
+                         torch.empty(q_count * B, dtype=torch.float64, device=dev))
+            raw = getattr(c, "raw", None)
+            tail = (ksel, c.cap, a.knn, float(a.decay), float(a.thresh), ptr(nmax_used), float(c.err_coef), ptr(c.norm2), float(c.err_lin), ptr(r.bw),
+                    ptr(r.keep_cnt), ptr(r.flag_rows), ptr(n_flag), float(a.bw_scale), ptr(a.bw_fixed), max_rank, *map(ptr, r.buckets), st)
+            if raw is not None:
+                check(lib.meld_knn_refine_sort_emit(ptr(a.X), a.N, a.d, ptr(c.idx), ptr(c.d2), ptr(c.cnt), ptr(raw[0]), ptr(raw[1]), ptr(c.thr), *tail),
+                      "meld_knn_refine_sort_emit")
+            else:
+                check(lib.meld_knn_refine_emit(ptr(a.X), a.N, a.d, ptr(c.idx), ptr(c.d2), ptr(c.cnt), ptr(c.thr), *tail), "meld_knn_refine_emit")
+        else:
+            r.cand_val = torch.empty(q_count * ksel, dtype=torch.float64, device=dev)
+            check(
+                lib.meld_knn_refine(
+                    ptr(a.X), a.N, a.d, a.q_begin, q_count, ptr(c.idx), ptr(c.d2), ptr(c.cnt), ptr(c.thr), ksel, c.cap, a.knn, float(a.decay),
+                    float(a.thresh), ptr(nmax_used), float(c.err_coef), ptr(c.norm2), float(c.err_lin), ptr(r.bw), ptr(r.cand_val), ptr(r.keep_cnt),
+                    ptr(r.flag_rows), ptr(n_flag), None, 0, None, float(a.bw_scale), ptr(a.bw_fixed), max_rank, st,
+                ),
+                "meld_knn_refine",
+            )
         r.n_flag = r.n_flag_stage1 = int(n_flag.item())
         a.tm.stop("refine")
         stage2 = c.research is not None and r.n_flag > 0 and not a.force_fallback
@@ -831,6 +865,9 @@
         lib, st, dev, d, cap, o = self.lib, _stream(), a.X.device, a.d, c.cap, c.research
         n_flag_h = r.n_flag
         rows2 = torch.sort(r.flag_rows[:n_flag_h]).values.contiguous()
+        if r.buckets is not None:
+            r.cand_val = torch.empty(a.q_count * ksel, dtype=torch.float64, device=dev)
+            r.rows2 = rows2
         q2_pad = ((n_flag_h + o.BQ - 1) // o.BQ) * o.BQ
         Q2 = torch.empty(q2_pad * lib.meld_knn16_query_bytes(d), dtype=torch.uint8, device=dev)
         Qn2 = torch.empty(q2_pad, dtype=torch.float32, device=dev)
@@ -930,18 +967,29 @@
         lib, st, dev, q_count, n_flag_h, c = self.lib, _stream(), a.X.device, a.q_count, r.n_flag, r.cands
         M = r.m_main + s.fb_total
         assembled = None
-        if assemble and M > 0 and a.q_begin == 0 and q_count == a.NR and not a.cross and opt("MELD_ASSEMBLE", "bucket") == "bucket" \
-                and opt("MELD_ASSEMBLE_FUSED", "1") != "0":
-            B = int(lib.meld_csr_bucket_slots())
-            if ksel <= B and q_count * B * 12 <= torch.cuda.mem_get_info(dev)[0] // 4:
-                cursor = r.keep_cnt.clone()
-                if n_flag_h > 0 and s.fb_total > 0:
-                    cursor[r.flag_rows[:n_flag_h].to(torch.int64)] = s.fb_cnt
-                tcol = torch.empty(q_count * B, dtype=torch.int32, device=dev)
-                tval = torch.empty(q_count * B, dtype=torch.float64, device=dev)
-                check(lib.meld_coo_emit_scatter(q_count, ptr(c.idx), ptr(r.cand_val), ksel, c.cap, ptr(r.keep_cnt), ptr(r.flag_rows), n_flag_h,
-                                                ptr(s.fb_off), ptr(s.fb_col), ptr(s.fb_val), s.fb_total, ptr(cursor), ptr(tcol), ptr(tval), st),
-                      "meld_coo_emit_scatter")
+        fused = getattr(r, "buckets", None) is not None
+        if fused or (M > 0 and bucket_route(lib, a.NR, a.q_begin, q_count, ksel, cross=a.cross, assemble=assemble,
+                                            free_bytes=torch.cuda.mem_get_info(dev)[0])):
+            if fused and M == 0:
+                r.buckets = None
+            else:
+                if fused:
+                    cursor, tcol, tval = r.buckets
+                    n2 = int(r.rows2.shape[0]) if r.rows2 is not None else 0
+                    if n2 > 0 or (n_flag_h > 0 and s.fb_total > 0):
+                        check(lib.meld_coo_emit_scatter_listed(ptr(r.rows2), n2, ptr(c.idx), ptr(r.cand_val), ksel, c.cap, ptr(r.keep_cnt), ptr(r.flag_rows),
+                                                               n_flag_h, ptr(s.fb_off), ptr(s.fb_col), ptr(s.fb_val), s.fb_total, ptr(cursor), ptr(tcol),
+                                                               ptr(tval), st), "meld_coo_emit_scatter_listed")
+                else:
+                    B = int(lib.meld_csr_bucket_slots())
+                    cursor = r.keep_cnt.clone()
+                    if n_flag_h > 0 and s.fb_total > 0:
+                        cursor[r.flag_rows[:n_flag_h].to(torch.int64)] = s.fb_cnt
+                    tcol = torch.empty(q_count * B, dtype=torch.int32, device=dev)
+                    tval = torch.empty(q_count * B, dtype=torch.float64, device=dev)
+                    check(lib.meld_coo_emit_scatter(q_count, ptr(c.idx), ptr(r.cand_val), ksel, c.cap, ptr(r.keep_cnt), ptr(r.flag_rows), n_flag_h,
+                                                    ptr(s.fb_off), ptr(s.fb_col), ptr(s.fb_val), s.fb_total, ptr(cursor), ptr(tcol), ptr(tval), st),
+                          "meld_coo_emit_scatter")
                 a.tm.stop("coo_emit")
                 aniso = anisotropy if opt("MELD_ASSEMBLE_FUSED_ANISO", "1") != "0" else None
                 assembled = self._finish_buckets(cursor, tcol, tval, q_count, sums_diag=1.0, symm=symm, anisotropy=aniso)
@@ -951,6 +999,8 @@
                         assembled = assembled + (self.last_degrees,)
                 a.tm.stop("symmetrize")
                 del cursor, tcol, tval
+                if fused and assembled is None:
+                    return None, None, None
         keys = vals = None
         if assembled is None:
             keys = torch.empty(2 * M, dtype=torch.int64, device=dev)
diff --git a/meld_amd/knn_plan.py b/meld_amd/knn_plan.py
--- a/meld_amd/knn_plan.py
+++ b/meld_amd/knn_plan.py
@@ -52,6 +52,7 @@
     lead_bounds: Optional[bool] = None
     partial_forced: bool = False
     fused_operands: bool = dataclasses.field(default=False, compare=False)
+    fused_rows: str = dataclasses.field(default="off", compare=False)
 
     def __post_init__(self):
         if self.lead_bounds is None:
@@ -72,7 +73,29 @@
     return int(rows.value), int(row_bytes.value)
 
 
-def plan_knn_search(lib, N, d, q_begin, q_count, knn, ksel, *, options, cross=False, bandwidth=False, world=1, resident=0):
+def bucket_route(lib, N, q_begin, q_count, ksel, *, cross, assemble, free_bytes):
+    if not assemble or cross or q_begin != 0 or q_count != N:
+        return False
+    if opt("MELD_ASSEMBLE", "bucket") != "bucket" or opt("MELD_ASSEMBLE_FUSED", "1") == "0":
+        return False
+    B = int(lib.meld_csr_bucket_slots())
+    return ksel <= B and q_count * B * 12 <= int(free_bytes) // 4
+
+
+def plan_fused_rows(lib, N, d, q_begin, q_count, ksel, *, search, cross=False, world=1, assemble=False, free_bytes=0, x_aligned=True,
+                    raw_rows=False):
+    if search != "f16x3" or world != 1 or not bucket_route(lib, N, q_begin, q_count, ksel, cross=cross, assemble=assemble, free_bytes=free_bytes):
+        return "off"
+    if d % 2 != 0 or d > 256 or not x_aligned or ksel > 128 or ksel > int(lib.meld_csr_bucket_slots()):
+        return "off"
+    want = opt("MELD_ROWS_FUSED", "b")
+    if want == "0":
+        return "off"
+    return "sort+emit" if raw_rows and want != "a" else "emit"
+
+
+def plan_knn_search(lib, N, d, q_begin, q_count, knn, ksel, *, options, cross=False, bandwidth=False, world=1, resident=0, assemble=False,
+                    free_bytes=0, x_aligned=True):
     search = options.search
     if search == "f16x3" and lib.meld_knn16_kblocks(d) < 0:
         search = "wide"
@@ -112,5 +135,7 @@
     two_pass = lists != "none" and frame and (main_slices == 1 or two == "2") and two != "0" and ee is None
     lead_bounds = lists == "direct" and frame and opt("MELD_KNN16_LEAD_BOUNDS", "1") != "0"
     fused = prune and bounds != "bounds_from_spheres" and q_begin == 0 and q_count == N and opt("MELD_KNN_FUSED_OPERANDS", "1") != "0"
+    fused_rows = plan_fused_rows(lib, N, d, q_begin, q_count, ksel, search=search, cross=cross, world=world, assemble=assemble,
+                                 free_bytes=free_bytes, x_aligned=x_aligned, raw_rows=lists != "none" and main_slices == 1)
     return KnnPlan(search, nprod, frame, radius_cut, prune, seed, 0 if seed == "bandwidth" else knn, bounds, seeded_bounds, lists,
-                   block_order, main_slices, two_pass, partial, nprod == 1, lead_bounds, ee is not None, fused)
+                   block_order, main_slices, two_pass, partial, nprod == 1, lead_bounds, ee is not None, fused, fused_rows)
```
